# haoy945/DeMF

Hardware: AMD Instinct MI355X
Metric: DeMF fusion fwd+bwd scenes/sec at 20k pts + 530x730 RGB (higher is better)
Workload: dtype f32; 1 GPU; BASELINE configs[2]: full DeMF fusion hot path fwd+loss+bwd+allreduce+AdamW, 8 scenes/GPU x (20000 pts, 800x1120 -> 4-level 256-ch pyramid), 256 queries, H=8 L=4 P=2, fp32; compute_mode=f32, scenes_per_gpu=8, parallelism=dp1, cloud=uniform

## Files before the change

### demf_amd/_ffi.py

```python
import ctypes
import os

_HERE = os.path.dirname(os.path.abspath(__file__))
LIB_PATH = os.environ.get("DEMF_LIB_PATH") or os.path.join(_HERE, "lib", "libdemf_hip.so")

_c_int = ctypes.c_int
_c_float = ctypes.c_float
_ptr = ctypes.c_void_p

SIGNATURES = {
    "demf_stream_create_cu_masked": [_ptr, _c_int, _c_int, _ptr],
    "demf_spin_us": [_c_int, _ptr],
    "demf_conv_nhwc_f32": [_c_int] * 9 + [_ptr, _ptr, _c_int, _ptr, _ptr, _c_int, _c_int, _ptr, _ptr],
    "demf_conv_stem7_nhwc4_f32": [_c_int] * 4 + [_ptr, _ptr, _c_int, _ptr, _c_int, _ptr, _ptr],
    "demf_maxpool3x3s2_nhwc_f32": [_c_int] * 4 + [_ptr, _ptr, _ptr],
    "demf_nchw3_to_nhwc4_f32": [_c_int] * 3 + [_ptr, _ptr, _ptr],
    "demf_groupnorm_nhwc_f32": [_c_int] * 4 + [_c_float, _ptr, _ptr, _ptr, _ptr, _ptr, ctypes.c_longlong, _ptr],
    "demf_fps_f32": [_c_int, _c_int, _c_int, _ptr, _ptr, _ptr, _ptr],
    "demf_fps_ws_f32": [_c_int, _c_int, _c_int, _ptr, _ptr, ctypes.c_longlong, _ptr, _ptr],
    "demf_ball_query_f32": [_c_int, _c_int, _c_int, _c_float, _c_float, _c_int, _ptr, _ptr,
                            _ptr, _ptr],
    "demf_ball_query_grid_ws": [_c_int, _c_int, _ptr, _ptr],
    "demf_ball_query_grid_f32": [_c_int, _c_int, _c_int, _c_float, _c_int] + [_ptr] * 6,
    "demf_group_points_fwd": [_c_int] * 5 + [_ptr] * 4,
    "demf_group_points_bwd": [_c_int] * 5 + [_ptr] * 4,
    "demf_gather_points_fwd": [_c_int] * 4 + [_ptr] * 4,
    "demf_gather_points_bwd": [_c_int] * 4 + [_ptr] * 4,
    "demf_three_nn_f32": [_c_int] * 3 + [_ptr] * 5,
    "demf_three_nn_weights_f32": [_c_int] * 3 + [_ptr] * 6,
    "demf_three_interpolate_fwd": [_c_int] * 4 + [_ptr] * 5,
    "demf_three_interpolate_bwd": [_c_int] * 4 + [_ptr] * 5,
    "demf_group_concat_cl_fwd": [_c_int] * 8 + [_c_float, _c_int] + [_ptr] * 6,
    "demf_group_concat_cl_bwd": [_c_int] * 8 + [_c_float, _c_int] + [_ptr] * 6,
    "demf_gather_rows_cl_fwd": [_c_int] * 4 + [_ptr] * 4,
    "demf_gather_rows_cl_bwd": [_c_int] * 4 + [_ptr] * 4,
    "demf_three_interpolate_cl_fwd": [_c_int] * 6 + [_ptr] * 5,
    "demf_three_interpolate_cl_bwd": [_c_int] * 6 + [_ptr] * 5,
    "demf_three_interpolate_cat_cl_fwd": [_c_int] * 5 + [_ptr] * 6,
    "demf_maxpool_ns_fwd": [_c_int] * 3 + [_ptr] * 4,
    "demf_maxpool_ns_bwd": [_c_int] * 3 + [_ptr] * 4,
    "demf_colsum_f32": [_c_int] * 3 + [_ptr] * 3,
    "demf_nchw_to_tokens": [_c_int] * 5 + [_ptr] * 4,
    "demf_pyramid_to_tokens": [_c_int] * 4 + [_ptr] * 5,
    "demf_pyramid_to_tokens_bf16": [_c_int] * 4 + [_ptr] * 5,
    "demf_vote_targets": [_c_int] * 4 + [_ptr] * 8,
    "demf_box_extent_count": [_c_int] * 4 + [_ptr] * 8,
    "demf_aligned_nms": [_c_int, _c_int, _c_float] + [_ptr] * 6,
    "demf_detect_decode": [_c_int] * 6 + [_ptr] * 7 + [_ptr],
    "demf_detect_pack": [_c_int] * 4 + [_c_float] + [_ptr] * 5 + [_c_int] * 3 + [_ptr] * 5 + [_ptr],
    "demf_box3d_iou": [_c_int, _c_int] + [_ptr] * 4,
    "demf_eval_match": [_c_int, _c_int, _ptr, _c_int, _c_int] + [_ptr] * 7,
    "demf_eval_ap": [_c_int, _c_int] + [_ptr] * 8,
    "demf_points_floor": [_c_int, _c_int, ctypes.c_longlong] + [_ptr] * 4,
    "demf_points_prep": [_c_int] * 3 + [ctypes.c_longlong] + [_ptr] * 8,
    "demf_image_prep": [_c_int] * 3 + [ctypes.c_longlong] + [_ptr] * 6,
    "demf_proposal_targets": [_c_int] * 4 + [_c_float] * 3 + [_ptr] * 18,
    "demf_gt_prep": [_c_int] * 3 + [_ptr] * 10,
    "demf_pad_gt": [_c_int] * 2 + [_ptr] * 8,
    "demf_query_pos_rows": [_c_int] * 2 + [_ptr] * 4,
    "demf_loss_total": [_c_int] + [_ptr] * 4,
    "demf_loss_total_bwd": [_c_int] + [_ptr] * 4,
    "demf_target_weights": [_c_int] + [_ptr] * 5,
    "demf_rows_ln_pos_f32": [_c_int] * 2 + [_ptr] * 4 + [_c_float] + [_ptr] * 4,
    "demf_rows_gemm_f32": [_c_int] * 3 + [_ptr, ctypes.c_longlong, _ptr, _c_int, _c_int, _ptr, _c_int, _ptr, _c_int, _ptr, _c_int,
                           _ptr, ctypes.c_longlong, _ptr, _ptr, _c_float, _ptr, ctypes.c_longlong, _ptr],
    "demf_msda_fwd_raw_f32": [_c_int] * 7 + [_ptr, ctypes.c_longlong, _ptr, _ptr, _ptr, ctypes.c_longlong, _c_int, _c_int,
                              _ptr, _ptr, _ptr],
    "demf_msda_fwd_raw_head_f32": [_c_int] * 4 + [_ptr, ctypes.c_longlong, _ptr, _ptr, _ptr, ctypes.c_longlong, _c_int, _c_int,
                                   _ptr, _ptr, _c_int, _c_int, _ptr],
    "demf_invert_index": [_c_int] * 3 + [_ptr] * 4,
    "demf_invert_index_ws": [_c_int] * 3 + [_ptr] * 5,
    "demf_mlp_gemm_bwd_dw_group": [_c_int, _ptr, _ptr],
    "demf_sa_index_chain": [_c_int] * 3 + [_ptr] * 4,
    "demf_split_points": [ctypes.c_longlong, _c_int] + [_ptr] * 4,
    "demf_group_concat_cl_bwd_gather": [_c_int] * 6 + [_ptr] * 5,
    "demf_group_first_fwd": [_c_int] * 5 + [_c_float, _c_int] + [_ptr] * 5 + [_c_int] + [_ptr] * 4 + [_c_float] * 2 + [_ptr] * 6 + [_ptr],
    "demf_group_first_bwd": [_c_int] * 5 + [_c_float, _c_int] + [_ptr] * 10 + [_c_int, _ptr, _c_int] + [_ptr] * 4,
    "demf_adamw_f32": [ctypes.c_longlong] + [_ptr] * 5 + [_c_float] * 7 + [_c_int, _ptr],
    "demf_multi_copy_sumsq": [_c_int, _ptr, _c_int, _ptr, _ptr],
    "demf_sumsq_f32": [ctypes.c_longlong, _ptr, _ptr, _ptr],
    "demf_adamw_state_f32": [_c_int] + [_ptr] * 9 + [_c_float] * 5 + [_ptr],
    "demf_step_meter": [_c_int, _ptr, _ptr, _c_float, _c_float, _ptr, _c_int, _ptr],
    "demf_mlp_gemm_fwd": [_c_int] * 4 + [_ptr] * 6,
    "demf_mlp_gemm_fwd_pool": [_c_int] * 4 + [_ptr] * 5 + [_c_int] + [_ptr] * 5,
    "demf_mlp_gemm_fwd_bn": [_c_int] * 4 + [_ptr] * 7 + [_c_float, _c_float] + [_ptr] * 7,
    "demf_mlp_gemm_fwd_pool_bn": [_c_int] * 4 + [_ptr] * 5 + [_c_int] + [_ptr] * 6 + [_c_float, _c_float] + [_ptr] * 7,
    "demf_mlp_gemm_fwd_bn_st": [_c_int] * 4 + [_ptr] * 7 + [_c_float, _c_float] + [_ptr] * 6 + [_c_int, _ptr],
    "demf_mlp_gemm_fwd_pool_bn_st": [_c_int] * 4 + [_ptr] * 5 + [_c_int] + [_ptr] * 4 + [_c_float, _c_float] + [_ptr] * 6 + [_c_int, _ptr],
    "demf_pool_select": [_c_int] * 2 + [_ptr] * 9,
    "demf_pool_select_slot0": [_c_int] * 2 + [_ptr] * 7,
    "demf_mlp_first_stats": [_c_int] * 2 + [_ptr] * 5 + [_c_float, _c_float] + [_ptr] * 7,
    "demf_mlp_gemm_fwd_bn_x4": [_c_int] * 2 + [_ptr] * 8 + [_c_float, _c_float] + [_ptr] * 7,
    "demf_mlp_bwd_fused_x4": [_c_int] * 3 + [_ptr] * 11,
    "demf_mlp_bwd_pool": [_c_int] * 4 + [_ptr] * 17,
    "demf_mlp_bwd_pool_ws": [_c_int, _ptr],
    "demf_bn_finalize": [_c_int, ctypes.c_longlong] + [_ptr] * 3 + [_c_float, _c_float] + [_ptr] * 7,
    "demf_l2norm_rows_fwd": [_c_int] * 2 + [_ptr] * 4,
    "demf_l2norm_rows_bwd": [_c_int] * 2 + [_ptr] * 5,
    "demf_vote_combine_fwd": [_c_int] * 2 + [_ptr] * 7,
    "demf_vote_combine_bwd": [_c_int] * 2 + [_ptr] * 7,
    "demf_bnrelu_maxpool_fwd": [_c_int] * 3 + [_ptr] * 5,
    "demf_bn_bwd_reduce": [_c_int] * 3 + [_ptr] * 9,
    "demf_bn_bwd_vectors": [_c_int, ctypes.c_longlong] + [_ptr] * 8,
    "demf_mlp_gemm_bwd_dx": [_c_int] * 4 + [_ptr] * 3 + [_c_int] + [_ptr] * 5,
    "demf_mlp_gemm_bwd_dx_first": [_c_int] * 3 + [_ptr] * 10,
    "demf_mlp_first_finish": [_c_int, ctypes.c_longlong] + [_ptr] * 7,
    "demf_mlp_gemm_bwd_dx_red": [_c_int] * 4 + [_ptr] * 3 + [_c_int] + [_ptr] * 9,
    "demf_mlp_gemm_bwd_dx_w": [_c_int] * 4 + [_ptr] * 3 + [_c_int] + [_ptr] * 5,
    "demf_mlp_bwd_fused": [_c_int] * 3 + [_ptr] * 3 + [_c_int] + [_ptr] * 15 + [_c_int, _ptr],
    "demf_mlp_bwd_fused_cols": [_c_int] * 5 + [_ptr] * 3 + [_c_int] + [_ptr] * 14,
    "demf_mlp_gemm_bwd_dx_red_v": [_c_int] * 4 + [_ptr] * 3 + [_c_int] + [_ptr] * 13,
    "demf_bn_bwd_reduce_vectors": [_c_int] * 3 + [_ptr] * 11 + [_c_int, _ptr],
    "demf_mlp_gemm_bwd_dw": [_c_int] * 4 + [_ptr] * 3 + [_c_int] + [_ptr] * 6,
    "demf_mlp_gemm_bwd_dw_ld": [_c_int] * 4 + [_ptr] * 3 + [_c_int] + [_ptr] * 5 + [_c_int, _ptr],
    "demf_head_loss_fwd": [_c_int] * 3 + [_ptr] * 14,
    "demf_head_loss_bwd": [_c_int] * 3 + [_ptr] * 17,
    "demf_vote_loss": [_c_int] * 4 + [_c_float] + [_ptr] * 10,
    "demf_vote_loss_fwd": [_c_int] * 4 + [_c_float] + [_ptr] * 8,
    "demf_msda_fwd_f32": [_c_int] * 7 + [_ptr] * 7,
    "demf_msda_bwd_f32": [_c_int] * 7 + [_ptr] * 10,
    "demf_msda_fwd_bf16": [_c_int] * 7 + [_ptr] * 7,
    "demf_msda_bwd_bf16": [_c_int] * 7 + [_ptr] * 10,
    "demf_gemm_f32": [_ptr, _ptr],
    "demf_gemm_group_f32": [_ptr, _c_int, _ptr],
    "demf_set_compute_dtype": [_c_int],
    "demf_set_f16_terms": [_c_int],
    "demf_get_compute_dtype": [],
    "demf_ctx_push": [_ptr],
    "demf_ctx_pop": [],
    "demf_gemm_f32_ctx": [_ptr] * 3,
    "demf_gemm_group_f32_ctx": [_ptr, _ptr, _c_int, _ptr],
    "demf_mlp_gemm_fwd_ctx": [_ptr] + [_c_int] * 4 + [_ptr] * 6,
    "demf_multi_copy": [_c_int, _ptr, _c_int, _ptr],
    "demf_zero_f32": [ctypes.c_longlong, _ptr, _ptr],
    "demf_add_dropout_ln_fwd": [_c_int] * 2 + [_ptr] * 4 + [_c_float] * 2 + [_ptr, _c_int] + [_ptr] * 4,
    "demf_add_dropout_ln_bwd": [_c_int] * 2 + [_ptr] * 5 + [_c_float, _ptr, _c_int, _ptr, _c_int] + [_ptr] * 4,
    "demf_attn_core_fwd": [_c_int] * 4 + [_ptr, _c_float, _c_float, _ptr, _c_int] + [_ptr] * 5,
    "demf_attn_core_bwd": [_c_int] * 4 + [_ptr] * 4 + [_c_float, _c_float, _ptr, _c_int] + [_ptr] * 2,
    "demf_softmax_dropout_fwd": [_c_int] * 2 + [_ptr, _c_float, _ptr, _c_int] + [_ptr] * 3,
    "demf_softmax_dropout_bwd": [_c_int] * 2 + [_ptr, _c_float, _ptr, _c_int] + [_ptr] * 2,
    "demf_msda_prep_fwd": [_c_int] * 5 + [_ptr] * 10,
    "demf_msda_prep_bwd": [_c_int] * 5 + [_ptr] * 14,
    "demf_rng_advance": [_ptr, _ptr],
    "demf_rng_next": [_ptr, _ptr, _ptr],
    "demf_dropout_mask": [ctypes.c_longlong, _c_float, _ptr, _c_int, _ptr, _ptr],
}


class DwJob(ctypes.Structure):
    _fields_ = [("R", _c_int), ("N", _c_int), ("K", _c_int), ("ldx", _c_int), ("G", _ptr), ("dP", _ptr), ("arg", _ptr),
                ("ns", _c_int), ("Y", _ptr), ("vec6", _ptr), ("Xprev", _ptr), ("prev_scale_shift", _ptr), ("dW", _ptr),
                ("lddw", _c_int)]


class DetectLayer(ctypes.Structure):
    _fields_ = [("K", _c_int), ("res_scale", _c_float)] + [
        f for name in ("center", "center_base", "size", "dir_class", "dir_res", "obj", "sem")
        for f in ((name, _ptr), ((name if name != "center_base" else "base") + "_sb", _c_int),
                  ((name if name != "center_base" else "base") + "_sk", _c_int))]


class GemmDesc(ctypes.Structure):
    _ll = ctypes.c_longlong
    _fields_ = [
        ("M", _c_int), ("N", _c_int), ("K", _c_int), ("batch", _c_int), ("zdiv", _c_int),
        ("splitk", _c_int),
        ("A", _ptr), ("sam", _ll), ("sak", _ll), ("sab", _ll), ("sab2", _ll),
        ("A2", _ptr), ("a2_cols", _c_int),
        ("B", _ptr), ("sbn", _ll), ("sbk", _ll), ("sbb", _ll), ("sbb2", _ll),
        ("B2", _ptr), ("b2_rows", _c_int),
        ("C", _ptr), ("scm", _ll), ("scb", _ll), ("scb2", _ll),
        ("C2", _ptr),
        ("bias", _ptr), ("sbias_b", _ll),
        ("rowscale", _ptr), ("srs_m", _ll), ("srs_b", _ll),
        ("alpha", _c_float),
        ("flags", _c_int),
        ("gate", _ptr), ("sgm", _ll), ("sgb", _ll),
        ("gate_scale", _c_float),
        ("drop_p", _c_float),
        ("rng", _ptr),
        ("op_id", _c_int),
        ("asum", _ptr),
    ]

_lib = None


def load():
    global _lib
    if _lib is not None:
        return _lib
    if not os.path.exists(LIB_PATH):
        raise RuntimeError(
            f"{LIB_PATH} not found: build it with `python -c 'import __graft_entry__ as g; "
            "g.build()'` (hipcc --offload-arch=gfx950). demf_amd has no CPU fallback.")
    import torch
    lib = ctypes.CDLL(LIB_PATH)
    lib.demf_version.restype = _c_int
    lib.demf_version.argtypes = []
    lib.demf_last_error.restype = ctypes.c_char_p
    lib.demf_last_error.argtypes = []
    for name, argtypes in SIGNATURES.items():
        fn = getattr(lib, name)
        fn.restype = _c_int
        fn.argtypes = argtypes
    _lib = lib
    return lib


def call(name, *args):
    lib = load()
    rc = getattr(lib, name)(*args)
    if rc != 0:
        msg = lib.demf_last_error().decode("utf-8", "replace")
        raise RuntimeError(f"{name} failed (code {rc}): {msg}")
```

### demf_amd/csrc/dense.hip

```cpp
#include "common.h"
#include <stdlib.h>
#include <type_traits>
#include "rng.h"

namespace demf {

using f32x16 = float __attribute__((ext_vector_type(16)));
using bf16x8 = __bf16 __attribute__((ext_vector_type(8)));
using bf16x4 = __bf16 __attribute__((ext_vector_type(4)));

enum {
  GEMM_RELU = DEMF_GEMM_RELU, GEMM_DROPOUT = DEMF_GEMM_DROPOUT, GEMM_GATE = DEMF_GEMM_GATE,
  GEMM_ACCUM = DEMF_GEMM_ACCUM, GEMM_ROWBIAS = DEMF_GEMM_ROWBIAS, GEMM_ACCUM2 = DEMF_GEMM_ACCUM2,
  GEMM_FP32 = DEMF_GEMM_FP32,
};
using GemmArgs = demf_gemm_desc;

constexpr int G_BM = 64, G_BN = 64, G_BK = 64, G_LD = G_BK + 4;

struct GemmRegs {
  float4 v[4], w[4];
};

template <int mode, bool ADD2>
__device__ __forceinline__ void gemm_fetch(GemmRegs& g, float (&sc)[16], const float* __restrict__ P,
                                           const float* __restrict__ P2, long long sr, long long sk,
                                           int r0, int R, int k0, int K1) {
  const int t = threadIdx.x;
  if constexpr (mode == 1) {
#pragma unroll
    for (int i = 0; i < 4; ++i) {
      const int row = (t >> 4) + 16 * i, kq = (t & 15) * 4;
      g.v[i] = make_float4(0.f, 0.f, 0.f, 0.f);
      if constexpr (ADD2) g.w[i] = g.v[i];
      if (r0 + row < R && k0 + kq < K1) {
        const size_t o = (size_t)(r0 + row) * sr + k0 + kq;
        g.v[i] = *reinterpret_cast<const float4*>(P + o);
        if constexpr (ADD2) g.w[i] = *reinterpret_cast<const float4*>(P2 + o);
      }
    }
  } else if constexpr (mode == 2) {
#pragma unroll
    for (int i = 0; i < 4; ++i) {
      const int k = (t >> 4) + 16 * i, rq = (t & 15) * 4;
      g.v[i] = make_float4(0.f, 0.f, 0.f, 0.f);
      if constexpr (ADD2) g.w[i] = g.v[i];
      if (k0 + k < K1 && r0 + rq < R) {
        const size_t o = (size_t)(k0 + k) * sk + r0 + rq;
        g.v[i] = *reinterpret_cast<const float4*>(P + o);
        if constexpr (ADD2) g.w[i] = *reinterpret_cast<const float4*>(P2 + o);
      }
    }
  } else {
#pragma unroll
    for (int i = 0; i < 16; ++i) {
      const int e = t + 256 * i, row = e >> 6, k = e & 63;
      float v = 0.f;
      if (r0 + row < R && k0 + k < K1) {
        const size_t o = (size_t)(r0 + row) * sr + (size_t)(k0 + k) * sk;
        v = P[o];
        if constexpr (ADD2) v += P2[o];
      }
      sc[i] = v;
    }
  }
}

constexpr int G_LDB = 2 * (G_BK + 8);

__device__ __forceinline__ float4 add4(float4 v, const float4& w) {
  v.x += w.x; v.y += w.y; v.z += w.z; v.w += w.w;
  return v;
}

template <int mode, bool ADD2>
__device__ __forceinline__ void gemm_commit_bf16(char* __restrict__ s, const GemmRegs& g, const float (&sc)[16]) {
  const int t = threadIdx.x;
  if constexpr (mode == 1) {
#pragma unroll
    for (int i = 0; i < 4; ++i) {
      const float4 v = ADD2 ? add4(g.v[i], g.w[i]) : g.v[i];
      bf16x4 b;
      b[0] = (__bf16)v.x; b[1] = (__bf16)v.y; b[2] = (__bf16)v.z; b[3] = (__bf16)v.w;
      *reinterpret_cast<bf16x4*>(s + ((t >> 4) + 16 * i) * G_LDB + 2 * (t & 15) * 4) = b;
    }
  } else if constexpr (mode == 2) {
#pragma unroll
    for (int i = 0; i < 4; ++i) {
      const float4 v = ADD2 ? add4(g.v[i], g.w[i]) : g.v[i];
      char* d = s + (t & 15) * 4 * G_LDB + 2 * ((t >> 4) + 16 * i);
      *reinterpret_cast<__bf16*>(d) = (__bf16)v.x;
      *reinterpret_cast<__bf16*>(d + G_LDB) = (__bf16)v.y;
      *reinterpret_cast<__bf16*>(d + 2 * G_LDB) = (__bf16)v.z;
      *reinterpret_cast<__bf16*>(d + 3 * G_LDB) = (__bf16)v.w;
    }
  } else {
#pragma unroll
    for (int i = 0; i < 16; ++i) {
      const int e = t + 256 * i;
      *reinterpret_cast<__bf16*>(s + (e >> 6) * G_LDB + 2 * (e & 63)) = (__bf16)sc[i];
    }
  }
}

template <int mode, bool ADD2>
__device__ __forceinline__ void gemm_commit(float* __restrict__ s, const GemmRegs& g, const float (&sc)[16]) {
  const int t = threadIdx.x;
  if constexpr (mode == 1) {
#pragma unroll
    for (int i = 0; i < 4; ++i) {
      float4 v = g.v[i];
      if constexpr (ADD2) { v.x += g.w[i].x; v.y += g.w[i].y; v.z += g.w[i].z; v.w += g.w[i].w; }
      *reinterpret_cast<float4*>(s + ((t >> 4) + 16 * i) * G_LD + (t & 15) * 4) = v;
    }
  } else if constexpr (mode == 2) {
#pragma unroll
    for (int i = 0; i < 4; ++i) {
      float4 v = g.v[i];
      if constexpr (ADD2) { v.x += g.w[i].x; v.y += g.w[i].y; v.z += g.w[i].z; v.w += g.w[i].w; }
      float* d = s + (t & 15) * 4 * G_LD + (t >> 4) + 16 * i;
      d[0] = v.x; d[G_LD] = v.y; d[2 * G_LD] = v.z; d[3 * G_LD] = v.w;
    }
  } else {
#pragma unroll
    for (int i = 0; i < 16; ++i) {
      const int e = t + 256 * i;
      s[(e >> 6) * G_LD + (e & 63)] = sc[i];
    }
  }
}

__device__ __forceinline__ void gemm_store(const GemmArgs& p, int z, size_t oc, int sp, int m, int n,
                                           float bias, float accv) {
  float v = p.alpha * accv;
  if (p.flags & GEMM_ROWBIAS) {
    if (sp == 0) v = __builtin_fmaf(bias, p.rowscale[(size_t)m * p.srs_m + (size_t)z * p.srs_b], v);
  } else {
    v += bias;
  }
  if (p.flags & GEMM_RELU) v = fmaxf(v, 0.f);
  if (p.flags & GEMM_DROPOUT) {
    const unsigned long long idx = ((unsigned long long)z * p.M + m) * p.N + n;
    v = dropout_keep((const unsigned long long*)p.rng, (unsigned)p.op_id, idx, p.drop_p)
            ? v * (1.0f / (1.0f - p.drop_p)) : 0.f;
  }
  if (p.flags & GEMM_GATE)
    v = p.gate[(size_t)z * p.sgb + (size_t)m * p.sgm + n] != 0.f ? v * p.gate_scale : 0.f;
  float* dst = p.C + oc + (size_t)m * p.scm + n;
  if (p.splitk > 1) atomicAdd(dst, v);
  else if (p.flags & GEMM_ACCUM) *dst += v;
  else *dst = v;
  if (p.C2 != nullptr) {
    float* d2 = p.C2 + oc + (size_t)m * p.scm + n;
    if (p.splitk > 1) atomicAdd(d2, v);
    else if (p.flags & GEMM_ACCUM2) *d2 += v;
    else *d2 = v;
  }
}

__device__ __forceinline__ void xcd_rows(int& bx, int& by, int gx, int gy) {
  if ((gy & 7) == 0) {
    const int L = bx + gx * by;
    by = (L & 7) + 8 * (L / (8 * gx));
    bx = (L >> 3) % gx;
  }
}

template <int MA, int MB, bool ADD, bool BF16>
__global__ __launch_bounds__(256, 2) void gemm_kernel(GemmArgs p) {
  __shared__ __attribute__((aligned(16))) float s_a[G_BM * G_LD];
  __shared__ __attribute__((aligned(16))) float s_b[G_BN * G_LD];
  const int lane = threadIdx.x & 63, wave = threadIdx.x >> 6;
  const int lr = lane & 31, lh = lane >> 5;
  const int wm = wave & 1, wn = wave >> 1;
  int bx = blockIdx.x, by = blockIdx.y;
  xcd_rows(bx, by, gridDim.x, gridDim.y);
  const int m0 = by * G_BM, n0 = bx * G_BN;
  const int z = blockIdx.z / p.splitk, sp = blockIdx.z - z * p.splitk;
  const int kchunk = ((p.K + p.splitk - 1) / p.splitk + G_BK - 1) / G_BK * G_BK;
  const int kbeg = sp * kchunk, kend = min(p.K, kbeg + kchunk);
  const int zo = z / p.zdiv, zi = z - zo * p.zdiv;
  const size_t oa = (size_t)zo * p.sab + (size_t)zi * p.sab2, ob = (size_t)zo * p.sbb + (size_t)zi * p.sbb2;
  const float* A = p.A + oa;
  const float* A2 = (p.A2 != nullptr && n0 < p.a2_cols) ? p.A2 + oa : nullptr;
  const float* B = p.B + ob;
  const float* B2 = (p.B2 != nullptr && m0 < p.b2_rows) ? p.B2 + ob : nullptr;
  f32x16 acc;
#pragma unroll
  for (int r = 0; r < 16; ++r) acc[r] = 0.f;
  constexpr int NS = ADD ? 2 : 3;
  GemmRegs ga[NS], gb[NS];
  float sa16[NS][16], sb16[NS][16];
  auto fetch = [&](auto stage, int k0) {
    constexpr int S = decltype(stage)::value;
    if (ADD && A2 != nullptr) gemm_fetch<MA, ADD>(ga[S], sa16[S], A, A2, p.sam, p.sak, m0, p.M, k0, kend);
    else gemm_fetch<MA, false>(ga[S], sa16[S], A, nullptr, p.sam, p.sak, m0, p.M, k0, kend);
    if (ADD && B2 != nullptr) gemm_fetch<MB, ADD>(gb[S], sb16[S], B, B2, p.sbn, p.sbk, n0, p.N, k0, kend);
    else gemm_fetch<MB, false>(gb[S], sb16[S], B, nullptr, p.sbn, p.sbk, n0, p.N, k0, kend);
  };
  auto step = [&](auto stage, int k0) {
    constexpr int S = decltype(stage)::value;
    lds_barrier();
    if constexpr (BF16) {
      char* ca = reinterpret_cast<char*>(s_a);
      char* cb = reinterpret_cast<char*>(s_b);
      if (ADD && A2 != nullptr) gemm_commit_bf16<MA, ADD>(ca, ga[S], sa16[S]); else gemm_commit_bf16<MA, false>(ca, ga[S], sa16[S]);
      if (ADD && B2 != nullptr) gemm_commit_bf16<MB, ADD>(cb, gb[S], sb16[S]); else gemm_commit_bf16<MB, false>(cb, gb[S], sb16[S]);
      lds_barrier();
      if (k0 + NS * G_BK < kend) fetch(stage, k0 + NS * G_BK);
#pragma unroll
      for (int c16 = 0; c16 < G_BK / 16; ++c16) {
        const bf16x8 a8 = *reinterpret_cast<const bf16x8*>(ca + (wm * 32 + lr) * G_LDB + 2 * (c16 * 16 + 8 * lh));
        const bf16x8 b8 = *reinterpret_cast<const bf16x8*>(cb + (wn * 32 + lr) * G_LDB + 2 * (c16 * 16 + 8 * lh));
        acc = __builtin_amdgcn_mfma_f32_32x32x16_bf16(a8, b8, acc, 0, 0, 0);
      }
    } else {
      if (ADD && A2 != nullptr) gemm_commit<MA, ADD>(s_a, ga[S], sa16[S]); else gemm_commit<MA, false>(s_a, ga[S], sa16[S]);
      if (ADD && B2 != nullptr) gemm_commit<MB, ADD>(s_b, gb[S], sb16[S]); else gemm_commit<MB, false>(s_b, gb[S], sb16[S]);
      lds_barrier();
      if (k0 + NS * G_BK < kend) fetch(stage, k0 + NS * G_BK);
#pragma unroll
      for (int c8 = 0; c8 < G_BK / 8; ++c8) {
        const float4 a4 = *reinterpret_cast<const float4*>(s_a + (wm * 32 + lr) * G_LD + c8 * 8 + 4 * lh);
        const float4 b4 = *reinterpret_cast<const float4*>(s_b + (wn * 32 + lr) * G_LD + c8 * 8 + 4 * lh);
        acc = __builtin_amdgcn_mfma_f32_32x32x2f32(a4.x, b4.x, acc, 0, 0, 0);
        acc = __builtin_amdgcn_mfma_f32_32x32x2f32(a4.y, b4.y, acc, 0, 0, 0);
        acc = __builtin_amdgcn_mfma_f32_32x32x2f32(a4.z, b4.z, acc, 0, 0, 0);
        acc = __builtin_amdgcn_mfma_f32_32x32x2f32(a4.w, b4.w, acc, 0, 0, 0);
      }
    }
  };
  using S0 = std::integral_constant<int, 0>;
  using S1 = std::integral_constant<int, 1>;
  using S2 = std::integral_constant<int, NS - 1>;
  if (kbeg < kend) fetch(S0{}, kbeg);
  if (kbeg + G_BK < kend) fetch(S1{}, kbeg + G_BK);
  if constexpr (NS == 3) {
    if (kbeg + 2 * G_BK < kend) fetch(S2{}, kbeg + 2 * G_BK);
  }
  for (int k0 = kbeg; k0 < kend; k0 += NS * G_BK) {
    step(S0{}, k0);
    if (k0 + G_BK < kend) step(S1{}, k0 + G_BK);
    if constexpr (NS == 3) {
      if (k0 + 2 * G_BK < kend) step(S2{}, k0 + 2 * G_BK);
    }
  }
  const int n = n0 + wn * 32 + lr;
  if (n >= p.N) return;
  float bias = 0.f;
  if (p.bias != nullptr && sp == 0) bias = p.bias[(size_t)z * p.sbias_b + n];
  const size_t oc = (size_t)zo * p.scb + (size_t)zi * p.scb2;
#pragma unroll
  for (int r = 0; r < 16; ++r) {
    const int m = m0 + wm * 32 + (r & 3) + 8 * (r >> 2) + 4 * lh;
    if (m < p.M) gemm_store(p, z, oc, sp, m, n, bias, acc[r]);
  }
}

struct GemmRegsS {
  float4 v[2], w[2];
};

template <int mode, bool ADD2>
__device__ __forceinline__ void gemm_fetch_s(GemmRegsS& g, float (&sc)[8], const float* __restrict__ P,
                                             const float* __restrict__ P2, long long sr, long long sk,
                                             int r0, int R, int k0, int K1) {
  const int t = threadIdx.x;
  if constexpr (mode == 1) {
#pragma unroll
    for (int i = 0; i < 2; ++i) {
      const int row = (t >> 4) + 16 * i, kq = (t & 15) * 4;
      g.v[i] = make_float4(0.f, 0.f, 0.f, 0.f);
      if constexpr (ADD2) g.w[i] = g.v[i];
      if (r0 + row < R && k0 + kq < K1) {
        const size_t o = (size_t)(r0 + row) * sr + k0 + kq;
        g.v[i] = *reinterpret_cast<const float4*>(P + o);
        if constexpr (ADD2) g.w[i] = *reinterpret_cast<const float4*>(P2 + o);
      }
    }
  } else if constexpr (mode == 2) {
#pragma unroll
    for (int i = 0; i < 2; ++i) {
      const int k = (t >> 3) + 32 * i, rq = (t & 7) * 4;
      g.v[i] = make_float4(0.f, 0.f, 0.f, 0.f);
      if constexpr (ADD2) g.w[i] = g.v[i];
      if (k0 + k < K1 && r0 + rq < R) {
        const size_t o = (size_t)(k0 + k) * sk + r0 + rq;
        g.v[i] = *reinterpret_cast<const float4*>(P + o);
        if constexpr (ADD2) g.w[i] = *reinterpret_cast<const float4*>(P2 + o);
      }
    }
  } else {
#pragma unroll
    for (int i = 0; i < 8; ++i) {
      const int e = t + 256 * i, row = e >> 6, k = e & 63;
      float v = 0.f;
      if (r0 + row < R && k0 + k < K1) {
        const size_t o = (size_t)(r0 + row) * sr + (size_t)(k0 + k) * sk;
        v = P[o];
        if constexpr (ADD2) v += P2[o];
      }
      sc[i] = v;
    }
  }
}

template <int mode, bool ADD2, bool BF16>
__device__ __forceinline__ void gemm_commit_s(float* __restrict__ s, const GemmRegsS& g, const float (&sc)[8]) {
  const int t = threadIdx.x;
  char* sb = reinterpret_cast<char*>(s);
  if constexpr (mode == 1) {
#pragma unroll
    for (int i = 0; i < 2; ++i) {
      const float4 v = ADD2 ? add4(g.v[i], g.w[i]) : g.v[i];
      const int row = (t >> 4) + 16 * i, kq = (t & 15) * 4;
      if constexpr (BF16) {
        bf16x4 b;
        b[0] = (__bf16)v.x; b[1] = (__bf16)v.y; b[2] = (__bf16)v.z; b[3] = (__bf16)v.w;
        *reinterpret_cast<bf16x4*>(sb + row * G_LDB + 2 * kq) = b;
      } else {
        *reinterpret_cast<float4*>(s + row * G_LD + kq) = v;
      }
    }
  } else if constexpr (mode == 2) {
#pragma unroll
    for (int i = 0; i < 2; ++i) {
      const float4 v = ADD2 ? add4(g.v[i], g.w[i]) : g.v[i];
      const int k = (t >> 3) + 32 * i, rq = (t & 7) * 4;
      if constexpr (BF16) {
        char* d = sb + rq * G_LDB + 2 * k;
        *reinterpret_cast<__bf16*>(d) = (__bf16)v.x;
        *reinterpret_cast<__bf16*>(d + G_LDB) = (__bf16)v.y;
        *reinterpret_cast<__bf16*>(d + 2 * G_LDB) = (__bf16)v.z;
        *reinterpret_cast<__bf16*>(d + 3 * G_LDB) = (__bf16)v.w;
      } else {
        float* d = s + rq * G_LD + k;
        d[0] = v.x; d[G_LD] = v.y; d[2 * G_LD] = v.z; d[3 * G_LD] = v.w;
      }
    }
  } else {
#pragma unroll
    for (int i = 0; i < 8; ++i) {
      const int e = t + 256 * i;
      if constexpr (BF16) *reinterpret_cast<__bf16*>(sb + (e >> 6) * G_LDB + 2 * (e & 63)) = (__bf16)sc[i];
      else s[(e >> 6) * G_LD + (e & 63)] = sc[i];
    }
  }
}

template <int MA, int MB, bool ADD, bool BF16>
__device__ __forceinline__ void gemm_ks_body(const GemmArgs& p, int bx, int by, int bz, float* __restrict__ s_a,
                                             float* __restrict__ s_b, float (*s_red)[16][64]) {
  const int lane = threadIdx.x & 63, wave = threadIdx.x >> 6;
  const int lr = lane & 31, lh = lane >> 5;
  const int m0 = by * 32, n0 = bx * 32;
  const int z = bz / p.splitk, sp = bz - z * p.splitk;
  const bool do_asum = MA == 2 && p.asum != nullptr && bx == 0;
  float4 rs4 = make_float4(0.f, 0.f, 0.f, 0.f);
  const int kchunk = ((p.K + p.splitk - 1) / p.splitk + G_BK - 1) / G_BK * G_BK;
  const int kbeg = sp * kchunk, kend = min(p.K, kbeg + kchunk);
  const int zo = z / p.zdiv, zi = z - zo * p.zdiv;
  const size_t oa = (size_t)zo * p.sab + (size_t)zi * p.sab2, ob = (size_t)zo * p.sbb + (size_t)zi * p.sbb2;
  const float* A = p.A + oa;
  const float* A2 = (p.A2 != nullptr && n0 < p.a2_cols) ? p.A2 + oa : nullptr;
  const float* B = p.B + ob;
  const float* B2 = (p.B2 != nullptr && m0 < p.b2_rows) ? p.B2 + ob : nullptr;
  f32x16 acc;
#pragma unroll
  for (int r = 0; r < 16; ++r) acc[r] = 0.f;
  constexpr int NS = 3;
  GemmRegsS ga[NS], gb[NS];
  float sa8[NS][8], sb8[NS][8];
// ... 3 lines not shown
    else gemm_fetch_s<MA, false>(ga[S], sa8[S], A, nullptr, p.sam, p.sak, m0, p.M, k0, kend);
    if (ADD && B2 != nullptr) gemm_fetch_s<MB, ADD>(gb[S], sb8[S], B, B2, p.sbn, p.sbk, n0, p.N, k0, kend);
    else gemm_fetch_s<MB, false>(gb[S], sb8[S], B, nullptr, p.sbn, p.sbk, n0, p.N, k0, kend);
  };
  auto step = [&](auto stage, int k0) {
    constexpr int S = decltype(stage)::value;
    lds_barrier();
    if (ADD && A2 != nullptr) gemm_commit_s<MA, ADD, BF16>(s_a, ga[S], sa8[S]); else gemm_commit_s<MA, false, BF16>(s_a, ga[S], sa8[S]);
    if constexpr (MA == 2) {
      if (do_asum) {
        rs4 = add4(rs4, add4(ga[S].v[0], ga[S].v[1]));
      }
    }
    if (ADD && B2 != nullptr) gemm_commit_s<MB, ADD, BF16>(s_b, gb[S], sb8[S]); else gemm_commit_s<MB, false, BF16>(s_b, gb[S], sb8[S]);
    lds_barrier();
    if (k0 + NS * G_BK < kend) fetch(stage, k0 + NS * G_BK);
    if constexpr (BF16) {
      const char* ca = reinterpret_cast<const char*>(s_a);
      const char* cb = reinterpret_cast<const char*>(s_b);
      const bf16x8 a8 = *reinterpret_cast<const bf16x8*>(ca + lr * G_LDB + 2 * (wave * 16 + 8 * lh));
      const bf16x8 b8 = *reinterpret_cast<const bf16x8*>(cb + lr * G_LDB + 2 * (wave * 16 + 8 * lh));
      acc = __builtin_amdgcn_mfma_f32_32x32x16_bf16(a8, b8, acc, 0, 0, 0);
    } else {
#pragma unroll
      for (int c8 = 0; c8 < 2; ++c8) {
        const float4 a4 = *reinterpret_cast<const float4*>(s_a + lr * G_LD + wave * 16 + c8 * 8 + 4 * lh);
        const float4 b4 = *reinterpret_cast<const float4*>(s_b + lr * G_LD + wave * 16 + c8 * 8 + 4 * lh);
        acc = __builtin_amdgcn_mfma_f32_32x32x2f32(a4.x, b4.x, acc, 0, 0, 0);
        acc = __builtin_amdgcn_mfma_f32_32x32x2f32(a4.y, b4.y, acc, 0, 0, 0);
        acc = __builtin_amdgcn_mfma_f32_32x32x2f32(a4.z, b4.z, acc, 0, 0, 0);
        acc = __builtin_amdgcn_mfma_f32_32x32x2f32(a4.w, b4.w, acc, 0, 0, 0);
      }
    }
  };
  using S0 = std::integral_constant<int, 0>;
  using S1 = std::integral_constant<int, 1>;
  using S2 = std::integral_constant<int, 2>;
  if (kbeg < kend) fetch(S0{}, kbeg);
  if (kbeg + G_BK < kend) fetch(S1{}, kbeg + G_BK);
  if (kbeg + 2 * G_BK < kend) fetch(S2{}, kbeg + 2 * G_BK);
  for (int k0 = kbeg; k0 < kend; k0 += NS * G_BK) {
    step(S0{}, k0);
    if (k0 + G_BK < kend) step(S1{}, k0 + G_BK);
    if (k0 + 2 * G_BK < kend) step(S2{}, k0 + 2 * G_BK);
  }
#pragma unroll
  for (int r = 0; r < 16; ++r) s_red[wave][r][lane] = acc[r];
  lds_barrier();
  const int n = n0 + lr;
  if (n < p.N) {
    float bias = 0.f;
    if (p.bias != nullptr && sp == 0) bias = p.bias[(size_t)z * p.sbias_b + n];
    const size_t oc = (size_t)zo * p.scb + (size_t)zi * p.scb2;
#pragma unroll
    for (int q = 0; q < 4; ++q) {
      const int r = 4 * wave + q;
      const int m = m0 + q + 8 * wave + 4 * lh;
      const float v = (s_red[0][r][lane] + s_red[1][r][lane]) + (s_red[2][r][lane] + s_red[3][r][lane]);
      if (m < p.M) gemm_store(p, z, oc, sp, m, n, bias, v);
    }
  }
  if constexpr (MA == 2) {
    if (do_asum) {
      lds_barrier();
      float4* q4 = reinterpret_cast<float4*>(&s_red[0][0][0]);
      q4[threadIdx.x] = rs4;
      lds_barrier();
      if (threadIdx.x < 32 && m0 + (int)threadIdx.x < p.M) {
        const int rq = threadIdx.x >> 2, c = threadIdx.x & 3;
        const float* f = &s_red[0][0][0];
        float t = 0.f;
        for (int j = 0; j < 32; ++j) t += f[(8 * j + rq) * 4 + c];
        atomicAdd(p.asum + (size_t)z * p.M + m0 + threadIdx.x, t);
      }
    }
  }
}

template <int MA, int MB, bool ADD, bool BF16>
__global__ __launch_bounds__(256, ADD ? 2 : 4) void gemm_ks_kernel(GemmArgs p) {
  __shared__ __attribute__((aligned(16))) float s_a[32 * G_LD];
  __shared__ __attribute__((aligned(16))) float s_b[32 * G_LD];
  __shared__ float s_red[4][16][64];
  int bx = blockIdx.x, by = blockIdx.y;
  xcd_rows(bx, by, gridDim.x, gridDim.y);
  gemm_ks_body<MA, MB, ADD, BF16>(p, bx, by, blockIdx.z, s_a, s_b, s_red);
}

constexpr int GEMM_GROUP_MAX = 12;
struct GemmGroup {
  GemmArgs p[GEMM_GROUP_MAX];
  int start[GEMM_GROUP_MAX + 1];
  int n;
  int dbg;
};
template <int MA, int MB, bool ADD, bool BF16>
__global__ __launch_bounds__(256, ADD ? 2 : 4) void gemm_ks_group_kernel(GemmGroup g) {
  __shared__ __attribute__((aligned(16))) float s_a[32 * G_LD];
  __shared__ __attribute__((aligned(16))) float s_b[32 * G_LD];
  __shared__ float s_red[4][16][64];
  const int b = blockIdx.x;
  int i = 0;
  while (i + 1 < g.n && b >= g.start[i + 1]) ++i;
  const GemmArgs& p = g.p[i];
  const int local = b - g.start[i];
  const int gx = (p.N + 31) / 32, gy = (p.M + 31) / 32;
  const int sp = local % p.splitk, rest = local / p.splitk;
  const int bx = rest % gx, by = (rest / gx) % gy, bz = (rest / (gx * gy)) * p.splitk + sp;
  gemm_ks_body<MA, MB, ADD, BF16>(p, bx, by, bz, s_a, s_b, s_red);
}

using f32x2 = float __attribute__((ext_vector_type(2)));
using bf16x2 = __bf16 __attribute__((ext_vector_type(2)));
template <int P>
__device__ __forceinline__ void split_pair(float a, float b, unsigned (&o)[P]) {
  const f32x2 x = {a, b};
  const bf16x2 h = __builtin_convertvector(x, bf16x2);
  o[0] = __builtin_bit_cast(unsigned, h);
  if constexpr (P == 3) {
    const f32x2 r = x - __builtin_convertvector(h, f32x2);
    const bf16x2 m = __builtin_convertvector(r, bf16x2);
    o[1] = __builtin_bit_cast(unsigned, m);
    const f32x2 l = r - __builtin_convertvector(m, f32x2);
    o[2] = __builtin_bit_cast(unsigned, __builtin_convertvector(l, bf16x2));
  }
}
__device__ __forceinline__ int tn_swz(int col, int chunk) { return col * 64 + ((chunk ^ ((col >> 2) & 3)) << 4); }

template <int P>
__global__ __launch_bounds__(256, 3) void gemm_tn_group_kernel(GemmGroup g) {
  __shared__ __attribute__((aligned(16))) char s_pl[2][2][P][4096];
  __shared__ float4 s_rs[128];
  const int b = blockIdx.x;
  const int li = threadIdx.x & 63;
  const int gi = __builtin_amdgcn_readfirstlane(
      __popcll(__ballot(li + 1 < g.n && b >= g.start[li + 1 < GEMM_GROUP_MAX ? li + 1 : GEMM_GROUP_MAX])));
  const GemmArgs& p = g.p[gi];
  const int local = b - g.start[gi];
  const int gx = (p.N + 63) / 64, gy = (p.M + 63) / 64;
  const int sp = local % p.splitk, rest = local / p.splitk;
  const int bx = rest % gx, by = (rest / gx) % gy, z = rest / (gx * gy);
  const int m0 = by * 64, n0 = bx * 64;
  const int t = threadIdx.x, lane = t & 63, wave = t >> 6;
  const int lc = lane & 31, lh = lane >> 5, wm = wave & 1, wn = wave >> 1;
  const int kchunk = ((p.K + p.splitk - 1) / p.splitk + 31) / 32 * 32;
  const int kbeg = sp * kchunk, kend = min(p.K, kbeg + kchunk);
  const int zo = z / p.zdiv, zi = z - zo * p.zdiv;
  const size_t ob = (size_t)zo * p.sbb + (size_t)zi * p.sbb2;
  const int opd = t >> 7, u = t & 127, rg = u >> 4, sc = (u & 15) * 4;
  const float* src = opd == 0 ? p.A + (size_t)zo * p.sab + (size_t)zi * p.sab2 + m0 + sc : p.B + ob + n0 + sc;
  const float* src2 = (opd == 1 && p.B2 != nullptr && m0 < p.b2_rows) ? p.B2 + ob + n0 + sc : nullptr;
  const long long sk = opd == 0 ? p.sak : p.sbk;
  const bool col_ok = opd == 0 ? m0 + sc < p.M : n0 + sc < p.N;
  const bool do_asum = p.asum != nullptr && bx == 0 && opd == 0;
  float4 rv[2][4], rw[2][4], rs4 = make_float4(0.f, 0.f, 0.f, 0.f);
  auto fetch = [&](auto stage, int k0) {
    constexpr int S = decltype(stage)::value;
#pragma unroll
    for (int j = 0; j < 4; ++j) {
      const int k = k0 + 4 * rg + j;
      rv[S][j] = rw[S][j] = make_float4(0.f, 0.f, 0.f, 0.f);
      if (col_ok && k < kend && !(g.dbg & 8)) {
        rv[S][j] = *reinterpret_cast<const float4*>(src + (size_t)k * sk);
        if (src2 != nullptr) rw[S][j] = *reinterpret_cast<const float4*>(src2 + (size_t)k * sk);
      }
    }
// ... 11 lines not shown
      unsigned lo[P], hi[P];
      split_pair<P>(f[c], f[4 + c], lo);
      split_pair<P>(f[8 + c], f[12 + c], hi);
      const int off = tn_swz(sc + c, rg >> 1) + 8 * (rg & 1);
#pragma unroll
      for (int q = 0; q < P; ++q) *reinterpret_cast<uint2*>(&s_pl[buf][opd][q][off]) = make_uint2(lo[q], hi[q]);
    }
  };
  f32x16 acc, acc1;
#pragma unroll
  for (int r = 0; r < 16; ++r) acc[r] = acc1[r] = 0.f;
  auto step = [&](auto stage, int k0, int buf) {
    if (!(g.dbg & 4)) commit(stage, buf);
    lds_barrier();
    if (k0 + 64 < kend) fetch(stage, k0 + 64);
    if (g.dbg & 2) return;
#pragma unroll
    for (int c = 0; c < 2; ++c) {
      bf16x8 pa[P], pb[P];
#pragma unroll
      for (int q = 0; q < P; ++q) {
        pa[q] = *reinterpret_cast<const bf16x8*>(&s_pl[buf][0][q][tn_swz(32 * wm + lc, 2 * c + lh)]);
        pb[q] = *reinterpret_cast<const bf16x8*>(&s_pl[buf][1][q][tn_swz(32 * wn + lc, 2 * c + lh)]);
      }
      f32x16& ac = c == 0 ? acc : acc1;
      if constexpr (P == 3) {
        ac = __builtin_amdgcn_mfma_f32_32x32x16_bf16(pa[2], pb[0], ac, 0, 0, 0);
        ac = __builtin_amdgcn_mfma_f32_32x32x16_bf16(pa[0], pb[2], ac, 0, 0, 0);
        ac = __builtin_amdgcn_mfma_f32_32x32x16_bf16(pa[1], pb[1], ac, 0, 0, 0);
        ac = __builtin_amdgcn_mfma_f32_32x32x16_bf16(pa[1], pb[0], ac, 0, 0, 0);
        ac = __builtin_amdgcn_mfma_f32_32x32x16_bf16(pa[0], pb[1], ac, 0, 0, 0);
      }
      ac = __builtin_amdgcn_mfma_f32_32x32x16_bf16(pa[0], pb[0], ac, 0, 0, 0);
    }
  };
  using S0 = std::integral_constant<int, 0>;
  using S1 = std::integral_constant<int, 1>;
  if (kbeg < kend) fetch(S0{}, kbeg);
  if (kbeg + 32 < kend) fetch(S1{}, kbeg + 32);
  for (int k0 = kbeg; k0 < kend; k0 += 64) {
    step(S0{}, k0, 0);
    if (k0 + 32 < kend) step(S1{}, k0 + 32, 1);
  }
#pragma unroll
  for (int r = 0; r < 16; ++r) acc[r] += acc1[r];
  const int n = n0 + 32 * wn + lc;
  if (n < p.N && !(g.dbg & 16)) {
    float* C = p.C + (size_t)zo * p.scb + (size_t)zi * p.scb2;
#pragma unroll
    for (int r = 0; r < 16; ++r) {
      const int m = m0 + 32 * wm + (r & 3) + 8 * (r >> 2) + 4 * lh;
      if (m < p.M) {
        float* dst = C + (size_t)m * p.scm + n;
        const float v = p.alpha * acc[r];
        if (g.dbg & 1) *dst = v;
        else if (p.splitk > 1) atomicAdd(dst, v);
        else if (p.flags & GEMM_ACCUM) *dst += v;
        else *dst = v;
      }
    }
  }
  if (p.asum != nullptr && bx == 0) {
    if (opd == 0) s_rs[u] = rs4;
    lds_barrier();
    if (t < 64 && m0 + t < p.M) {
      const float* f = reinterpret_cast<const float*>(s_rs);
      float v = 0.f;
      for (int j = 0; j < 8; ++j) v += f[(16 * j + (t >> 2)) * 4 + (t & 3)];
      atomicAdd(p.asum + (size_t)z * p.M + m0 + t, v);
    }
  }
}

static int env_tiles() {
  static const int v = getenv("DEMF_GEMM_SMALL_TILES") ? atoi(getenv("DEMF_GEMM_SMALL_TILES")) : 1024;
  return v;
}

static int stage_mode(long long sr, long long sk, int R, int K) {
  if (sk == 1 && K % 4 == 0) return 1;
  if (sr == 1 && R % 4 == 0) return 2;
  return 0;
}

template <int VPL>
__global__ __launch_bounds__(256) void add_dropout_ln_fwd_k(int R, const float* __restrict__ x,
                                                            const float* __restrict__ identity,
                                                            const float* __restrict__ gamma,
                                                            const float* __restrict__ beta, float eps,
                                                            float p, const unsigned long long* __restrict__ rng,
                                                            unsigned op, float* __restrict__ s_out,
                                                            float* __restrict__ y,
                                                            float* __restrict__ stats) {
  constexpr int C = 64 * VPL;
  const int row = blockIdx.x * 4 + (threadIdx.x >> 6), lane = threadIdx.x & 63;
  if (row >= R) return;
  const float inv_keep = p > 0.f ? 1.0f / (1.0f - p) : 1.0f;
  float v[VPL];
  float sum = 0.f;
#pragma unroll
  for (int i = 0; i < VPL; ++i) {
    const int c = lane + 64 * i;
    float xv = x[(size_t)row * C + c];
    if (p > 0.f) xv = dropout_keep(rng, op, (unsigned long long)row * C + c, p) ? xv * inv_keep : 0.f;
    v[i] = (identity != nullptr ? identity[(size_t)row * C + c] : 0.f) + xv;
    sum += v[i];
  }
  const float mean = group_allsum<64>(sum) * (1.0f / C);
  float sq = 0.f;
#pragma unroll
  for (int i = 0; i < VPL; ++i) sq = __builtin_fmaf(v[i] - mean, v[i] - mean, sq);
  const float rstd = 1.0f / sqrtf(group_allsum<64>(sq) * (1.0f / C) + eps);
#pragma unroll
  for (int i = 0; i < VPL; ++i) {
    const int c = lane + 64 * i;
    if (s_out != nullptr) s_out[(size_t)row * C + c] = v[i];
    y[(size_t)row * C + c] = __builtin_fmaf((v[i] - mean) * rstd, gamma[c], beta[c]);
  }
  if (lane == 0 && stats != nullptr) { stats[2 * row] = mean; stats[2 * row + 1] = rstd; }
}

template <int VPL>
__global__ __launch_bounds__(256) void add_dropout_ln_bwd_k(int R, int rows_per_wave,
                                                            const float* __restrict__ dy,
                                                            const float* __restrict__ dy2,
                                                            const float* __restrict__ s,
                                                            const float* __restrict__ stats,
                                                            const float* __restrict__ gamma, float p,
                                                            const unsigned long long* __restrict__ rng,
                                                            unsigned op, float* __restrict__ ds_out,
                                                            int ds_accum, float* __restrict__ dx_out,
                                                            float* __restrict__ dgamma,
                                                            float* __restrict__ dbeta) {
  constexpr int C = 64 * VPL;
  __shared__ float s_red[4][2][C];
  const int wave = threadIdx.x >> 6, lane = threadIdx.x & 63;
  const float inv_keep = p > 0.f ? 1.0f / (1.0f - p) : 1.0f;
  float ag[VPL], ab[VPL], gm[VPL];
#pragma unroll
  for (int i = 0; i < VPL; ++i) { ag[i] = ab[i] = 0.f; gm[i] = gamma[lane + 64 * i]; }
  const int row0 = (blockIdx.x * 4 + wave) * rows_per_wave;
  for (int row = row0; row < min(R, row0 + rows_per_wave); ++row) {
    const float mean = stats[2 * row], rstd = stats[2 * row + 1];
    float d[VPL], xh[VPL];
    float m1 = 0.f, m2 = 0.f;
#pragma unroll
    for (int i = 0; i < VPL; ++i) {
      const size_t o = (size_t)row * C + lane + 64 * i;
      d[i] = dy[o] + (dy2 != nullptr ? dy2[o] : 0.f);
      xh[i] = (s[o] - mean) * rstd;
      ag[i] = __builtin_fmaf(d[i], xh[i], ag[i]);
      ab[i] += d[i];
      const float g = d[i] * gm[i];
      m1 += g;
      m2 = __builtin_fmaf(g, xh[i], m2);
    }
    m1 = group_allsum<64>(m1) * (1.0f / C);
    m2 = group_allsum<64>(m2) * (1.0f / C);
#pragma unroll
    for (int i = 0; i < VPL; ++i) {
      const int c = lane + 64 * i;
      const size_t o = (size_t)row * C + c;
      const float v = rstd * (d[i] * gm[i] - m1 - xh[i] * m2);
      if (ds_out != nullptr) ds_out[o] = ds_accum ? ds_out[o] + v : v;
      if (dx_out != nullptr) {
        float xv = v;
// ... 154 lines not shown
    if (h != 0) return;
    for (int hh = 0; hh < H; ++hh)
      for (int l = 0; l < L; ++l) {
        const float vx = vr[(b * L + l) * 2], vy = vr[(b * L + l) * 2 + 1];
        for (int q = 0; q < P; ++q) {
          const size_t o = ((size_t)row * H + hh) * LP + l * P + q;
          du = __builtin_fmaf(DL(2 * o), vx, du);
          dv = __builtin_fmaf(DL(2 * o + 1), vy, dv);
        }
      }
  }
  const float u0 = uvw[4 * row], v0 = uvw[4 * row + 1], xw = uvw[4 * row + 2], yw = uvw[4 * row + 3];
  if (!(u0 >= 0.f && u0 <= 1.f)) du = 0.f;
  if (!(v0 >= 0.f && v0 <= 1.f)) dv = 0.f;
  const float x = pts[3 * row], y = pts[3 * row + 1], zc = pts[3 * row + 2];
  const float* m = M + 16 * b;
  const float pw = m[8] * x + m[9] * y + m[10] * zc + m[11];
  const float gx = du * ab[4 * b] / pw, gy = dv * ab[4 * b + 2] / pw;
  const float gw = -(gx * xw + gy * yw);
  dpts[3 * row] = gx * m[0] + gy * m[4] + gw * m[8];
  dpts[3 * row + 1] = gx * m[1] + gy * m[5] + gw * m[9];
  dpts[3 * row + 2] = gx * m[2] + gy * m[6] + gw * m[10];
}

template <int VPL>
__global__ __launch_bounds__(256) void l2norm_fwd_k(int R, const float* __restrict__ x,
                                                    float* __restrict__ y, float* __restrict__ norm) {
  constexpr int C = 64 * VPL;
  const int row = blockIdx.x * 4 + (threadIdx.x >> 6), lane = threadIdx.x & 63;
  if (row >= R) return;
  float v[VPL], sq = 0.f;
#pragma unroll
  for (int i = 0; i < VPL; ++i) { v[i] = x[(size_t)row * C + lane + 64 * i]; sq = __builtin_fmaf(v[i], v[i], sq); }
  const float n = sqrtf(group_allsum<64>(sq));
#pragma unroll
  for (int i = 0; i < VPL; ++i) y[(size_t)row * C + lane + 64 * i] = v[i] / n;
  if (lane == 0) norm[row] = n;
}

template <int VPL>
__global__ __launch_bounds__(256) void l2norm_bwd_k(int R, const float* __restrict__ y,
                                                    const float* __restrict__ norm,
                                                    const float* __restrict__ dy, float* __restrict__ dx) {
  constexpr int C = 64 * VPL;
  const int row = blockIdx.x * 4 + (threadIdx.x >> 6), lane = threadIdx.x & 63;
  if (row >= R) return;
  float yv[VPL], g[VPL], dot = 0.f;
#pragma unroll
  for (int i = 0; i < VPL; ++i) {
    yv[i] = y[(size_t)row * C + lane + 64 * i];
    g[i] = dy[(size_t)row * C + lane + 64 * i];
    dot = __builtin_fmaf(yv[i], g[i], dot);
  }
  dot = group_allsum<64>(dot);
  const float inv = 1.0f / norm[row];
#pragma unroll
  for (int i = 0; i < VPL; ++i) dx[(size_t)row * C + lane + 64 * i] = (g[i] - yv[i] * dot) * inv;
}

template <int VPL>
__global__ __launch_bounds__(256) void vote_combine_fwd_k(int R, const float* __restrict__ rows,
                                                          const float* __restrict__ votes,
                                                          const float* __restrict__ seed_xyz,
                                                          float* __restrict__ vote_xyz,
                                                          float* __restrict__ y, float* __restrict__ norm) {
  constexpr int C = 64 * VPL;
  const int row = blockIdx.x * 4 + (threadIdx.x >> 6), lane = threadIdx.x & 63;
  if (row >= R) return;
  const float* vr = votes + (size_t)row * (C + 3);
  float v[VPL], sq = 0.f;
#pragma unroll
  for (int i = 0; i < VPL; ++i) {
    v[i] = rows[(size_t)row * C + lane + 64 * i] + vr[3 + lane + 64 * i];
    sq = __builtin_fmaf(v[i], v[i], sq);
  }
  const float n = sqrtf(group_allsum<64>(sq));
#pragma unroll
  for (int i = 0; i < VPL; ++i) y[(size_t)row * C + lane + 64 * i] = v[i] / n;
  if (lane == 0) norm[row] = n;
  if (lane < 3) vote_xyz[(size_t)row * 3 + lane] = seed_xyz[(size_t)row * 3 + lane] + vr[lane];
}

template <int VPL>
__global__ __launch_bounds__(256) void vote_combine_bwd_k(int R, const float* __restrict__ y,
                                                          const float* __restrict__ norm,
                                                          const float* __restrict__ dy,
                                                          const float* __restrict__ dxyz,
                                                          float* __restrict__ dvotes,
                                                          float* __restrict__ drows) {
  constexpr int C = 64 * VPL;
  const int row = blockIdx.x * 4 + (threadIdx.x >> 6), lane = threadIdx.x & 63;
  if (row >= R) return;
  float yv[VPL], g[VPL], dot = 0.f;
#pragma unroll
  for (int i = 0; i < VPL; ++i) {
    yv[i] = y[(size_t)row * C + lane + 64 * i];
    g[i] = dy != nullptr ? dy[(size_t)row * C + lane + 64 * i] : 0.f;
    dot = __builtin_fmaf(yv[i], g[i], dot);
  }
  dot = group_allsum<64>(dot);
  const float inv = 1.0f / norm[row];
  float* dv = dvotes + (size_t)row * (C + 3);
#pragma unroll
  for (int i = 0; i < VPL; ++i) {
    const float d = (g[i] - yv[i] * dot) * inv;
    dv[3 + lane + 64 * i] = d;
    drows[(size_t)row * C + lane + 64 * i] = d;
  }
  if (lane < 3) dv[lane] = dxyz != nullptr ? dxyz[(size_t)row * 3 + lane] : 0.f;
}

__global__ void rng_advance_k(unsigned long long* rng) { rng[1] += 1; }
__global__ void rng_next_k(unsigned long long* rng, unsigned long long* snap) {
  const unsigned long long s = rng[1] + 1;
  rng[1] = s;
  snap[0] = rng[0];
  snap[1] = s;
}

__global__ void dropout_mask_k(long long n, float p, const unsigned long long* __restrict__ rng,
                               unsigned op, float* __restrict__ out) {
  const long long i = (long long)blockIdx.x * blockDim.x + threadIdx.x;
  if (i < n) out[i] = dropout_keep(rng, op, (unsigned long long)i, p) ? 1.0f / (1.0f - p) : 0.f;
}

}

using namespace demf;

static int gemm_validate(const GemmArgs& p) {
  DEMF_REQUIRE(p.M > 0 && p.N > 0 && p.K > 0 && p.batch > 0 && p.splitk > 0 && p.zdiv > 0,
               "gemm: bad sizes %d %d %d %d %d %d", p.M, p.N, p.K, p.batch, p.splitk, p.zdiv);
  DEMF_REQUIRE(p.A && p.B && p.C, "gemm: null operand");
  DEMF_REQUIRE(!(p.flags & GEMM_DROPOUT) || p.rng, "gemm: dropout needs the rng state");
  DEMF_REQUIRE(!(p.flags & GEMM_GATE) || p.gate, "gemm: gate flag without a gate tensor");
  DEMF_REQUIRE(!(p.flags & GEMM_ROWBIAS) || (p.rowscale && p.bias), "gemm: rowbias needs bias and rowscale");
  DEMF_REQUIRE(p.splitk == 1 || !(p.flags & (GEMM_RELU | GEMM_DROPOUT | GEMM_GATE)),
               "gemm: split-K cannot carry a non-linear epilogue");
  DEMF_REQUIRE((long long)p.batch * p.splitk <= 65535, "gemm: batch*splitk too large");
  return DEMF_OK;
}

static bool gemm_is_small(const GemmArgs& p) {
  const long long tiles = (long long)cdiv(p.N, G_BN) * cdiv(p.M, G_BM) * p.batch * p.splitk;
  return tiles <= env_tiles() || p.N <= 32;
}

extern "C" int demf_gemm_f32(const demf_gemm_desc* d, demf_stream_t stream) {
  DEMF_REQUIRE(d != nullptr, "gemm: null descriptor");
  GemmArgs p = *d;
  if (int e = gemm_validate(p)) return e;
  const int modeA = stage_mode(p.sam, p.sak, p.M, p.K);
  const int modeB = stage_mode(p.sbn, p.sbk, p.N, p.K);
  dim3 grid(cdiv(p.N, G_BN), cdiv(p.M, G_BM), p.batch * p.splitk);
  const bool add = p.A2 != nullptr || p.B2 != nullptr;
  const bool bf = compute_bf16() && !(p.flags & GEMM_FP32);
  const bool small = gemm_is_small(p);
  if (p.asum != nullptr && !(small && modeA == 2 && p.A2 == nullptr)) {
    DEMF_REQUIRE(p.sam == 1 && p.A2 == nullptr,
                 "gemm: asum needs A contiguous along M (sam == 1) and no A2");
    float* asum = p.asum;
    p.asum = nullptr;
    if (int e = demf_gemm_f32(&p, stream)) return e;
    for (int z = 0; z < p.batch; ++z) {
      const int zo = z / p.zdiv, zi = z - zo * p.zdiv;
      const float* a = p.A + (size_t)zo * p.sab + (size_t)zi * p.sab2;
      if (int e = demf_colsum_f32(p.K, p.M, (int)p.sak, a, asum + (size_t)z * p.M, stream)) return e;
    }
    return DEMF_OK;
  }
  if (small) {
    grid = dim3(cdiv(p.N, 32), cdiv(p.M, 32), p.batch * p.splitk);
#define GEMM_LAUNCH_S(MA_, MB_)                                                                        \
  do {                                                                                                 \
    if (bf) {                                                                                          \
      if (add) hipLaunchKernelGGL((gemm_ks_kernel<MA_, MB_, true, true>), grid, dim3(256), 0, (hipStream_t)stream, p);   \
      else hipLaunchKernelGGL((gemm_ks_kernel<MA_, MB_, false, true>), grid, dim3(256), 0, (hipStream_t)stream, p);      \
    } else {                                                                                           \
      if (add) hipLaunchKernelGGL((gemm_ks_kernel<MA_, MB_, true, false>), grid, dim3(256), 0, (hipStream_t)stream, p);  \
      else hipLaunchKernelGGL((gemm_ks_kernel<MA_, MB_, false, false>), grid, dim3(256), 0, (hipStream_t)stream, p);     \
    }                                                                                                  \
  } while (0)
    switch (modeA * 3 + modeB) {
      case 0: GEMM_LAUNCH_S(0, 0); break;
      case 1: GEMM_LAUNCH_S(0, 1); break;
      case 2: GEMM_LAUNCH_S(0, 2); break;
      case 3: GEMM_LAUNCH_S(1, 0); break;
      case 4: GEMM_LAUNCH_S(1, 1); break;
      case 5: GEMM_LAUNCH_S(1, 2); break;
      case 6: GEMM_LAUNCH_S(2, 0); break;
      case 7: GEMM_LAUNCH_S(2, 1); break;
      default: GEMM_LAUNCH_S(2, 2); break;
    }
#undef GEMM_LAUNCH_S
    return check_launch("gemm_ks_kernel");
  }
#define GEMM_LAUNCH(MA_, MB_)                                                                          \
  do {                                                                                                 \
    if (bf) {                                                                                          \
      if (add) hipLaunchKernelGGL((gemm_kernel<MA_, MB_, true, true>), grid, dim3(256), 0, (hipStream_t)stream, p);   \
      else hipLaunchKernelGGL((gemm_kernel<MA_, MB_, false, true>), grid, dim3(256), 0, (hipStream_t)stream, p);      \
    } else {                                                                                           \
      if (add) hipLaunchKernelGGL((gemm_kernel<MA_, MB_, true, false>), grid, dim3(256), 0, (hipStream_t)stream, p);  \
      else hipLaunchKernelGGL((gemm_kernel<MA_, MB_, false, false>), grid, dim3(256), 0, (hipStream_t)stream, p);     \
    }                                                                                                  \
  } while (0)
  switch (modeA * 3 + modeB) {
    case 0: GEMM_LAUNCH(0, 0); break;
    case 1: GEMM_LAUNCH(0, 1); break;
    case 2: GEMM_LAUNCH(0, 2); break;
    case 3: GEMM_LAUNCH(1, 0); break;
    case 4: GEMM_LAUNCH(1, 1); break;
    case 5: GEMM_LAUNCH(1, 2); break;
    case 6: GEMM_LAUNCH(2, 0); break;
    case 7: GEMM_LAUNCH(2, 1); break;
    default: GEMM_LAUNCH(2, 2); break;
  }
#undef GEMM_LAUNCH
  return check_launch("gemm_kernel");
}

extern "C" int demf_gemm_group_f32(const demf_gemm_desc* descs, int n, demf_stream_t stream) {
  DEMF_REQUIRE(descs != nullptr && n >= 1, "gemm_group: no descriptors");
  const bool bf = compute_bf16();
  static const bool tn_off = getenv("DEMF_GEMM_TN3") && atoi(getenv("DEMF_GEMM_TN3")) == 0;
  const bool tn3 = compute_mode() != 0 && !tn_off;
  static const int tn_split = getenv("DEMF_GEMM_TN_SPLIT") ? atoi(getenv("DEMF_GEMM_TN_SPLIT")) : 0;
  int i0 = 0;
  while (i0 < n) {
    GemmGroup g{};
    int cnt = 0, tiles = 0;
    while (i0 + cnt < n && cnt < GEMM_GROUP_MAX) {
      const GemmArgs& p = descs[i0 + cnt];
      if (int e = gemm_validate(p)) return e;
      const bool ok = gemm_is_small(p) && stage_mode(p.sam, p.sak, p.M, p.K) == 2 &&
                      stage_mode(p.sbn, p.sbk, p.N, p.K) == 2 && !(p.flags & GEMM_FP32) && p.A2 == nullptr &&
                      (!tn3 || ((p.flags & ~GEMM_ACCUM) == 0 && p.bias == nullptr && p.C2 == nullptr &&
                                (p.B2 == nullptr || p.b2_rows % 64 == 0 || p.b2_rows >= p.M)));
      if (!ok) break;
      g.p[cnt] = p;
      g.start[cnt] = tiles;
      tiles += (tn3 ? cdiv(p.N, 64) * cdiv(p.M, 64) : cdiv(p.N, 32) * cdiv(p.M, 32)) * p.batch * g.p[cnt].splitk;
      ++cnt;
    }
    if (cnt == 0) {
      if (int e = demf_gemm_f32(descs + i0, stream)) return e;
      ++i0;
      continue;
    }
    if (tn3) {
      int base = 0;
      for (int i = 0; i < cnt; ++i) base += cdiv(g.p[i].N, 64) * cdiv(g.p[i].M, 64) * g.p[i].batch;
      const int want = tn_split > 0 ? tn_split : (768 + base / 2) / base;
      tiles = 0;
      for (int i = 0; i < cnt; ++i) {
        GemmArgs& q = g.p[i];
        if (q.splitk > 1) q.splitk = want < 2 ? 2 : (want < q.splitk ? want : q.splitk);
        g.start[i] = tiles;
        tiles += cdiv(q.N, 64) * cdiv(q.M, 64) * q.batch * q.splitk;
      }
    }
    g.start[cnt] = tiles;
    g.n = cnt;
    static const int tn_dbg = getenv("DEMF_TN_DBG") ? atoi(getenv("DEMF_TN_DBG")) : 0;
    g.dbg = tn_dbg;
    if (tn3) {
      if (bf) hipLaunchKernelGGL((gemm_tn_group_kernel<1>), dim3(tiles), dim3(256), 0, (hipStream_t)stream, g);
      else hipLaunchKernelGGL((gemm_tn_group_kernel<3>), dim3(tiles), dim3(256), 0, (hipStream_t)stream, g);
      if (int e = check_launch("gemm_tn_group_kernel")) return e;
      i0 += cnt;
      continue;
    }
    if (bf) hipLaunchKernelGGL((gemm_ks_group_kernel<2, 2, true, true>), dim3(tiles), dim3(256), 0, (hipStream_t)stream, g);
    else hipLaunchKernelGGL((gemm_ks_group_kernel<2, 2, true, false>), dim3(tiles), dim3(256), 0, (hipStream_t)stream, g);
    if (int e = check_launch("gemm_ks_group_kernel")) return e;
    i0 += cnt;
  }
  return DEMF_OK;
}

#define LN_DISPATCH(C, CALL)                       \
  switch ((C) / 64) {                              \
    case 1: CALL(1); break;                        \
    case 2: CALL(2); break;                        \
    case 4: CALL(4); break;                        \
    case 8: CALL(8); break;                        \
    case 16: CALL(16); break;                      \
    default:                                       \
      demf::set_error("row kernel: %d channels unsupported (64/128/256/512/1024)", (C)); \
      return DEMF_EUNSUPPORTED;                    \
  }

#define SM_DISPATCH(S, CALL)                       \
  if ((S) <= 0 || (S) > 1024) {                    \
    demf::set_error("softmax: %d keys unsupported (1..1024)", (S)); \
    return DEMF_EUNSUPPORTED;                      \
  } else if ((S) <= 64) { CALL(1); }               \
  else if ((S) <= 128) { CALL(2); }                \
  else if ((S) <= 256) { CALL(4); }                \
  else if ((S) <= 512) { CALL(8); }                \
  else { CALL(16); }

extern "C" int demf_add_dropout_ln_fwd(int R, int C, const float* x, const float* identity,
                                       const float* gamma, const float* beta, float eps, float p,
                                       const void* rng, int op_id, float* s_out, float* y,
                                       float* stats, demf_stream_t stream) {
  DEMF_REQUIRE(R > 0 && x && gamma && beta && y, "add_dropout_ln_fwd: bad arguments");
  DEMF_REQUIRE(p == 0.f || rng, "add_dropout_ln_fwd: dropout needs the rng state");
#define CALL(V) hipLaunchKernelGGL(add_dropout_ln_fwd_k<V>, dim3(cdiv(R, 4)), dim3(256), 0, (hipStream_t)stream, \
                                   R, x, identity, gamma, beta, eps, p, (const unsigned long long*)rng,        \
                                   (unsigned)op_id, s_out, y, stats)
  LN_DISPATCH(C, CALL)
#undef CALL
  return check_launch("add_dropout_ln_fwd_k");
}

extern "C" int demf_add_dropout_ln_bwd(int R, int C, const float* dy, const float* dy2, const float* s,
                                       const float* stats, const float* gamma, float p, const void* rng,
// ... 10 lines not shown
  LN_DISPATCH(C, CALL)
#undef CALL
  return check_launch("add_dropout_ln_bwd_k");
}

extern "C" int demf_softmax_dropout_fwd(int R, int S, const float* scores, float p, const void* rng,
                                        int op_id, float* prob, float* out, demf_stream_t stream) {
  DEMF_REQUIRE(R > 0 && scores && prob && out, "softmax_dropout_fwd: bad arguments");
  DEMF_REQUIRE(p == 0.f || rng, "softmax_dropout_fwd: dropout needs the rng state");
#define CALL(V) hipLaunchKernelGGL(softmax_dropout_fwd_k<V>, dim3(cdiv(R, 4)), dim3(256), 0, (hipStream_t)stream, \
                                   R, S, scores, p, (const unsigned long long*)rng, (unsigned)op_id, prob, out)
  SM_DISPATCH(S, CALL)
#undef CALL
  return check_launch("softmax_dropout_fwd_k");
}

extern "C" int demf_softmax_dropout_bwd(int R, int S, const float* prob, float p, const void* rng,
                                        int op_id, float* dio, demf_stream_t stream) {
  DEMF_REQUIRE(R > 0 && prob && dio, "softmax_dropout_bwd: bad arguments");
  DEMF_REQUIRE(p == 0.f || rng, "softmax_dropout_bwd: dropout needs the rng state");
#define CALL(V) hipLaunchKernelGGL(softmax_dropout_bwd_k<V>, dim3(cdiv(R, 4)), dim3(256), 0, (hipStream_t)stream, \
                                   R, S, prob, p, (const unsigned long long*)rng, (unsigned)op_id, dio)
  SM_DISPATCH(S, CALL)
#undef CALL
  return check_launch("softmax_dropout_bwd_k");
}

extern "C" int demf_msda_prep_fwd(int R, int Q, int H, int L, int P, const float* pts, const float* M,
                                  const float* ab, const float* valid_ratios, const int64_t* shapes,
                                  const float* raw, float* loc, float* w, float* uvw,
                                  demf_stream_t stream) {
  DEMF_REQUIRE(R > 0 && Q > 0 && R % Q == 0 && H > 0 && L > 0 && P > 0 && L * P <= 16,
               "msda_prep_fwd: bad sizes (L*P <= 16)");
  DEMF_REQUIRE(pts && M && ab && valid_ratios && shapes && raw && loc && w && uvw, "msda_prep_fwd: null pointer");
  hipLaunchKernelGGL(msda_prep_fwd_k, dim3(cdiv(R * H, 256)), dim3(256), 0, (hipStream_t)stream, R, Q, H, L,
                     P, pts, M, ab, valid_ratios, (const long long*)shapes, raw, loc, w, uvw);
  return check_launch("msda_prep_fwd_k");
}

extern "C" int demf_msda_prep_bwd(int R, int Q, int H, int L, int P, const float* pts, const float* M,
                                  const float* ab, const float* valid_ratios, const int64_t* shapes,
                                  const float* w, const float* uvw, const float* dloc, const float* dloc2,
                                  const float* dw, const float* dw2, float* draw, float* dpts,
                                  demf_stream_t stream) {
  DEMF_REQUIRE(R > 0 && Q > 0 && R % Q == 0 && H > 0 && L > 0 && P > 0 && L * P <= 16,
               "msda_prep_bwd: bad sizes (L*P <= 16)");
  DEMF_REQUIRE(pts && M && ab && valid_ratios && shapes && w && uvw && dloc && dw && draw, "msda_prep_bwd: null pointer");
  hipLaunchKernelGGL(msda_prep_bwd_k, dim3(cdiv(R * H, 256)), dim3(256), 0, (hipStream_t)stream, R, Q, H, L,
                     P, pts, M, ab, valid_ratios, (const long long*)shapes, w, uvw, dloc, dloc2, dw, dw2, draw, dpts);
  return check_launch("msda_prep_bwd_k");
}

extern "C" int demf_l2norm_rows_fwd(int R, int C, const float* x, float* y, float* norm,
                                    demf_stream_t stream) {
  DEMF_REQUIRE(R > 0 && x && y && norm, "l2norm_rows_fwd: bad arguments");
#define CALL(V) hipLaunchKernelGGL(l2norm_fwd_k<V>, dim3(cdiv(R, 4)), dim3(256), 0, (hipStream_t)stream, R, x, y, norm)
  LN_DISPATCH(C, CALL)
#undef CALL
  return check_launch("l2norm_fwd_k");
}

extern "C" int demf_l2norm_rows_bwd(int R, int C, const float* y, const float* norm, const float* dy,
                                    float* dx, demf_stream_t stream) {
  DEMF_REQUIRE(R > 0 && y && norm && dy && dx, "l2norm_rows_bwd: bad arguments");
#define CALL(V) hipLaunchKernelGGL(l2norm_bwd_k<V>, dim3(cdiv(R, 4)), dim3(256), 0, (hipStream_t)stream, R, y, norm, dy, dx)
  LN_DISPATCH(C, CALL)
#undef CALL
  return check_launch("l2norm_bwd_k");
}

extern "C" int demf_vote_combine_fwd(int R, int C, const float* rows, const float* votes,
                                     const float* seed_xyz, float* vote_xyz, float* vote_feats,
                                     float* norm, demf_stream_t stream) {
  DEMF_REQUIRE(R > 0 && rows && votes && seed_xyz && vote_xyz && vote_feats && norm,
               "vote_combine_fwd: bad arguments");
#define CALL(V) hipLaunchKernelGGL(vote_combine_fwd_k<V>, dim3(cdiv(R, 4)), dim3(256), 0, (hipStream_t)stream, R, rows, votes, seed_xyz, vote_xyz, vote_feats, norm)
  LN_DISPATCH(C, CALL)
#undef CALL
  return check_launch("vote_combine_fwd_k");
}

extern "C" int demf_vote_combine_bwd(int R, int C, const float* vote_feats, const float* norm,
                                     const float* d_vote_feats, const float* d_vote_xyz,
                                     float* d_votes, float* d_rows, demf_stream_t stream) {
  DEMF_REQUIRE(R > 0 && vote_feats && norm && d_votes && d_rows, "vote_combine_bwd: bad arguments");
#define CALL(V) hipLaunchKernelGGL(vote_combine_bwd_k<V>, dim3(cdiv(R, 4)), dim3(256), 0, (hipStream_t)stream, R, vote_feats, norm, d_vote_feats, d_vote_xyz, d_votes, d_rows)
  LN_DISPATCH(C, CALL)
#undef CALL
  return check_launch("vote_combine_bwd_k");
}

extern "C" int demf_rng_advance(void* rng, demf_stream_t stream) {
  DEMF_REQUIRE(rng, "rng_advance: null state");
  hipLaunchKernelGGL(rng_advance_k, dim3(1), dim3(1), 0, (hipStream_t)stream, (unsigned long long*)rng);
  return check_launch("rng_advance_k");
}

extern "C" int demf_rng_next(void* rng, void* snapshot, demf_stream_t stream) {
  DEMF_REQUIRE(rng && snapshot, "rng_next: null state");
  hipLaunchKernelGGL(rng_next_k, dim3(1), dim3(1), 0, (hipStream_t)stream, (unsigned long long*)rng,
                     (unsigned long long*)snapshot);
  return check_launch("rng_next_k");
}

extern "C" int demf_dropout_mask(long long n, float p, const void* rng, int op_id, float* out,
                                 demf_stream_t stream) {
  DEMF_REQUIRE(n > 0 && rng && out && p >= 0.f && p < 1.f, "dropout_mask: bad arguments");
  hipLaunchKernelGGL(dropout_mask_k, dim3((unsigned)((n + 255) / 256)), dim3(256), 0, (hipStream_t)stream, n, p,
                     (const unsigned long long*)rng, (unsigned)op_id, out);
  return check_launch("dropout_mask_k");
}
```

### demf_amd/csrc/loss.hip

```cpp
#include "common.h"

namespace demf {

struct HeadLossCfg {
  int R, ncls, nreg, nbins, nsem;
  float cw0, cw1;
  float w_obj, w_dircls, w_dirres, w_size, w_center, w_sem, w_iou;
  float beta_dirres, beta_size, beta_center;
};

constexpr int NLOSS = 7;

__device__ __forceinline__ float smooth_l1(float d, float beta) {
  const float a = fabsf(d);
  return a < beta ? 0.5f * a * a / beta : a - 0.5f * beta;
}
__device__ __forceinline__ float smooth_l1_grad(float d, float beta) {
  const float a = fabsf(d);
  return a < beta ? d / beta : (d > 0.f ? 1.f : (d < 0.f ? -1.f : 0.f));
}

template <int MAXN>
__device__ __forceinline__ float ce(const float* p, int n, int t, float* grad , float gscale) {
  float m = p[0];
// ... 347 lines not shown
                          float* __restrict__ dir_res, unsigned char* __restrict__ valid,
                          long long* __restrict__ lab, float* __restrict__ center) {
  const int i = blockIdx.x * blockDim.x + threadIdx.x;
  if (i >= n) return;
  const float* t = gt + (size_t)i * 7;
  const float yaw = t[6];
  cs[i] = cosf(-yaw);
  sn[i] = sinf(-yaw);
  const float two_pi = (float)(2.0 * 3.14159265358979323846);
  const float per = (float)(2.0 * 3.14159265358979323846 / (double)nbins);
  const float half = (float)(2.0 * 3.14159265358979323846 / (double)nbins / 2.0);
  const float ang = torch_remainder(yaw, two_pi);
  const float shifted = torch_remainder(ang + half, two_pi);
  const float c = torch_floor_divide(shifted, per);
  dir_cls[i] = (long long)c;
  dir_res[i] = shifted - (c * per + half);
  const long long l = labels[i];
  valid[i] = l >= 0 ? 1 : 0;
  lab[i] = l < 0 ? 0 : l;
  center[(size_t)i * 3] = t[0];
  center[(size_t)i * 3 + 1] = t[1];
  center[(size_t)i * 3 + 2] = t[2] + t[5] * 0.5f;
}

constexpr int PAD_GT_MAX_B = 32;
struct PadGtArgs {
  const float* boxes[PAD_GT_MAX_B];
  const long long* labels[PAD_GT_MAX_B];
  int count[PAD_GT_MAX_B];
  int box_dim[PAD_GT_MAX_B];
  int B, G;
};
__global__ void pad_gt_k(PadGtArgs a, float* __restrict__ gt, long long* __restrict__ lab,
                         unsigned char* __restrict__ valid) {
  const int i = blockIdx.x * blockDim.x + threadIdx.x;
  if (i >= a.B * a.G) return;
  const int b = i / a.G, g = i - b * a.G;
  const int n = a.count[b];
  float* o = gt + (size_t)i * 7;
  if (g < n) {
    const float* t = a.boxes[b] + (size_t)g * a.box_dim[b];
#pragma unroll
    for (int c = 0; c < 7; ++c) o[c] = t[c];
    lab[i] = a.labels[b][g];
  } else {
#pragma unroll
    for (int c = 0; c < 7; ++c) o[c] = 0.f;
    lab[i] = (n == 0 && g == 0) ? 0 : -1;
  }
  if (valid != nullptr) valid[i] = g < (n > 1 ? n : 1) ? 1 : 0;
}

__global__ void query_pos_rows_k(int R, int nreg, const float* __restrict__ reg, const float* __restrict__ base,
                                 float* __restrict__ out) {
  const int r = blockIdx.x * blockDim.x + threadIdx.x;
  if (r >= R) return;
  const float* g = reg + (size_t)r * nreg;
  const float* b = base + (size_t)r * 3;
  float4* o = reinterpret_cast<float4*>(out + (size_t)r * 8);
  o[0] = make_float4(b[0] + g[0], b[1] + g[1], b[2] + g[2], g[3]);
  o[1] = make_float4(g[4], g[5], 0.f, 0.f);
}

__global__ __launch_bounds__(1024) void target_weights_k(int R, const float* __restrict__ obj_mask,
                                                         const long long* __restrict__ obj_t,
                                                         float* __restrict__ obj_w,
                                                         float* __restrict__ box_w) {
  __shared__ float s_m[16], s_o[16];
  float m = 0.f, o = 0.f;
  for (int i = threadIdx.x; i < R; i += 1024) { m += obj_mask[i]; o += (float)obj_t[i]; }
  for (int d = 32; d >= 1; d >>= 1) { m += __shfl_xor(m, d); o += __shfl_xor(o, d); }
  if ((threadIdx.x & 63) == 0) { s_m[threadIdx.x >> 6] = m; s_o[threadIdx.x >> 6] = o; }
  __syncthreads();
  m = 0.f; o = 0.f;
  for (int w = 0; w < 16; ++w) { m += s_m[w]; o += s_o[w]; }
  const float im = m + 1e-6f, io = o + 1e-6f;
  for (int i = threadIdx.x; i < R; i += 1024) {
    obj_w[i] = obj_mask[i] / im;
    box_w[i] = (float)obj_t[i] / io;
  }
}

struct LossTotalArgs { const float* v[4]; };
__global__ void loss_total_k(int n, LossTotalArgs a, const float* __restrict__ vote, float* __restrict__ out8) {
  if (threadIdx.x != 0 || blockIdx.x != 0) return;
  float tot = 0.f;
  for (int i = 0; i < 7; ++i) {
    float m = a.v[0][i];
    for (int j = 1; j < n; ++j) m = m + a.v[j][i];
    m = m / (float)n;
    out8[i] = m;
    tot = i == 0 ? m : tot + m;
  }
  out8[7] = tot + (vote ? vote[0] : 0.f);
}
__global__ void loss_total_bwd_k(int n, const float* __restrict__ g8, float* __restrict__ gv, float* __restrict__ gvote) {
  const int t = threadIdx.x;
  if (t < 7) {
    const float g = (g8[t] + g8[7]) / (float)n;
    for (int j = 0; j < n; ++j) gv[7 * j + t] = g;
  }
  if (t == 7 && gvote) gvote[0] = g8[7];
}

}


using namespace demf;

static HeadLossCfg make_cfg(int R, const float* hp) {
  HeadLossCfg c;
  c.R = R; c.ncls = 12; c.nreg = 30; c.nbins = 12; c.nsem = 10;
  c.cw0 = hp[0]; c.cw1 = hp[1];
  c.w_obj = hp[2]; c.w_dircls = hp[3]; c.w_dirres = hp[4]; c.w_size = hp[5]; c.w_center = hp[6];
  c.w_sem = hp[7]; c.w_iou = hp[8];
  c.beta_dirres = hp[9]; c.beta_size = hp[10]; c.beta_center = hp[11];
  return c;
}

extern "C" int demf_head_loss_fwd(int R, int num_dir_bins, int num_classes, const float* hyper12,
                                  const float* cls, const float* reg, const float* base_xyz,
                                  const float* center_t, const float* size_t_,
                                  const int64_t* dir_class_t, const float* dir_res_t,
                                  const int64_t* sem_t, const int64_t* obj_t, const float* obj_w,
                                  const float* box_w, float* out7, demf_stream_t stream) {
  DEMF_REQUIRE(R >= 0 && num_dir_bins == 12 && num_classes == 10,
               "head_loss: only the reference layout (12 direction bins, 10 classes) is built");
  if (R == 0) return DEMF_OK;
  DEMF_REQUIRE(hyper12 && cls && reg && base_xyz && center_t && size_t_ && dir_class_t && dir_res_t &&
                   sem_t && obj_t && obj_w && box_w && out7, "head_loss_fwd: null pointer");
  hipLaunchKernelGGL(head_loss_fwd_k, dim3(cdiv(R, 256)), dim3(256), 0, (hipStream_t)stream,
                     make_cfg(R, hyper12), cls, reg, base_xyz, center_t, size_t_,
                     (const long long*)dir_class_t, dir_res_t, (const long long*)sem_t,
                     (const long long*)obj_t, obj_w, box_w, out7);
  return check_launch("head_loss_fwd");
}

extern "C" int demf_head_loss_bwd(int R, int num_dir_bins, int num_classes, const float* hyper12,
                                  const float* cls, const float* reg, const float* base_xyz,
                                  const float* center_t, const float* size_t_,
                                  const int64_t* dir_class_t, const float* dir_res_t,
                                  const int64_t* sem_t, const int64_t* obj_t, const float* obj_w,
                                  const float* box_w, const float* grad_out7, float* grad_cls,
                                  float* grad_reg, float* grad_base, demf_stream_t stream) {
  DEMF_REQUIRE(R >= 0 && num_dir_bins == 12 && num_classes == 10,
               "head_loss: only the reference layout (12 direction bins, 10 classes) is built");
  if (R == 0) return DEMF_OK;
  DEMF_REQUIRE(hyper12 && cls && reg && base_xyz && center_t && size_t_ && dir_class_t && dir_res_t &&
                   sem_t && obj_t && obj_w && box_w && grad_out7 && grad_cls && grad_reg && grad_base,
               "head_loss_bwd: null pointer");
  hipLaunchKernelGGL(head_loss_bwd_k, dim3(cdiv(R, 256)), dim3(256), 0, (hipStream_t)stream,
                     make_cfg(R, hyper12), cls, reg, base_xyz, center_t, size_t_,
                     (const long long*)dir_class_t, dir_res_t, (const long long*)sem_t,
                     (const long long*)obj_t, obj_w, box_w, grad_out7, grad_cls, grad_reg, grad_base);
  return check_launch("head_loss_bwd");
}

extern "C" int demf_vote_loss(int B, int S, int N, int gt_per_seed, float dst_weight,
                              const float* seed_points, const float* vote_points,
                              const int64_t* seed_indices, const int64_t* vote_target_masks,
                              const float* vote_targets, const float* mask_sum,
                              const float* grad_out, float* out, float* grad_vote,
                              demf_stream_t stream) {
  DEMF_REQUIRE(B >= 0 && S >= 0 && N >= 1 && gt_per_seed >= 1, "vote_loss: bad sizes");
  if (B * S == 0) return DEMF_OK;
  DEMF_REQUIRE(seed_points && vote_points && seed_indices && vote_target_masks && vote_targets &&
                   mask_sum && (grad_out ? grad_vote != nullptr : out != nullptr),
               "vote_loss: null pointer");
  hipLaunchKernelGGL(vote_loss_k<false>, dim3(cdiv(B * S, 256)), dim3(256), 0, (hipStream_t)stream, B, S, N,
                     3 * gt_per_seed, dst_weight, seed_points, vote_points,
                     (const long long*)seed_indices, (const long long*)vote_target_masks,
                     vote_targets, mask_sum, grad_out, out, grad_vote, (float*)nullptr);
  return check_launch("vote_loss");
}

extern "C" int demf_vote_loss_fwd(int B, int S, int N, int gt_per_seed, float dst_weight,
                                  const float* seed_points, const float* vote_points,
                                  const int64_t* seed_indices, const int64_t* vote_target_masks,
                                  const float* vote_targets, float* mask_sum_out, float* out,
                                  demf_stream_t stream) {
  DEMF_REQUIRE(B >= 0 && S >= 0 && N >= 1 && gt_per_seed >= 1, "vote_loss_fwd: bad sizes");
  DEMF_REQUIRE(mask_sum_out && out, "vote_loss_fwd: null pointer");
  if (B * S == 0) return DEMF_OK;
  DEMF_REQUIRE(seed_points && vote_points && seed_indices && vote_target_masks && vote_targets,
               "vote_loss_fwd: null pointer");
// ... 32 lines not shown
                                     int64_t* mask_targets, float* distance_targets,
                                     int64_t* objectness_targets, float* objectness_masks,
                                     demf_stream_t stream) {
  DEMF_REQUIRE(B >= 0 && Q >= 0 && G >= 1 && res_scale > 0.f, "proposal_targets: bad sizes");
  if (B * Q == 0) return DEMF_OK;
  DEMF_REQUIRE(aggregated_points && gt_boxes && cos_neg_yaw && sin_neg_yaw && gt_dir_class &&
                   gt_dir_res && gt_labels && valid && center_targets && size_targets &&
                   dir_class_targets && dir_res_targets && dir_targets && mask_targets &&
                   distance_targets && objectness_targets && objectness_masks,
               "proposal_targets: null pointer");
  PropTargetArgs a;
  a.Q = Q; a.G = G; a.with_rot = with_rot; a.pos_thr = pos_thr; a.neg_thr = neg_thr;
  a.res_scale = res_scale; a.agg = aggregated_points; a.gt = gt_boxes; a.cs = cos_neg_yaw;
  a.sn = sin_neg_yaw; a.dir_res = gt_dir_res; a.dir_cls = (const long long*)gt_dir_class;
  a.lab = (const long long*)gt_labels; a.valid = valid; a.center_t = center_targets;
  a.size_t_ = size_targets; a.dir_res_t = dir_res_targets; a.dir_t = dir_targets;
  a.dist_t = distance_targets; a.obj_mask = objectness_masks;
  a.dir_cls_t = (long long*)dir_class_targets; a.mask_t = (long long*)mask_targets;
  a.obj_t = (long long*)objectness_targets;
  hipLaunchKernelGGL(proposal_targets_k, dim3(cdiv(Q, 256), B), dim3(256), 0, (hipStream_t)stream, a);
  return check_launch("proposal_targets");
}

extern "C" int demf_gt_prep(int B, int G, int num_dir_bins, const float* gt_boxes,
                            const int64_t* labels_padded, float* cos_neg_yaw, float* sin_neg_yaw,
                            int64_t* gt_dir_class, float* gt_dir_res, unsigned char* valid,
                            int64_t* labels_clamped, float* gravity_center, demf_stream_t stream) {
  DEMF_REQUIRE(B >= 0 && G >= 1 && num_dir_bins >= 1, "gt_prep: bad sizes B=%d G=%d", B, G);
  if (B == 0) return DEMF_OK;
  DEMF_REQUIRE(gt_boxes && labels_padded && cos_neg_yaw && sin_neg_yaw && gt_dir_class && gt_dir_res &&
                   valid && labels_clamped && gravity_center, "gt_prep: null pointer");
  const int n = B * G;
  hipLaunchKernelGGL(gt_prep_k, dim3(cdiv(n, 256)), dim3(256), 0, (hipStream_t)stream, n, num_dir_bins,
                     gt_boxes, (const long long*)labels_padded, cos_neg_yaw, sin_neg_yaw,
                     (long long*)gt_dir_class, gt_dir_res, valid, (long long*)labels_clamped,
                     gravity_center);
  return check_launch("gt_prep");
}

extern "C" int demf_pad_gt(int B, int G, const int* counts, const int* box_dims, const void* const* boxes,
                           const void* const* labels, float* gt_padded, int64_t* labels_padded,
                           unsigned char* valid, demf_stream_t stream) {
  DEMF_REQUIRE(B >= 0 && B <= PAD_GT_MAX_B && G >= 1, "pad_gt: bad sizes B=%d (max %d) G=%d", B, PAD_GT_MAX_B, G);
  if (B == 0) return DEMF_OK;
  DEMF_REQUIRE(counts && box_dims && boxes && labels && gt_padded && labels_padded, "pad_gt: null pointer");
  PadGtArgs a{};
  a.B = B; a.G = G;
  for (int b = 0; b < B; ++b) {
    DEMF_REQUIRE(counts[b] >= 0 && counts[b] <= G, "pad_gt: scene %d has %d boxes, the padded form holds %d", b, counts[b], G);
    DEMF_REQUIRE(counts[b] == 0 || (boxes[b] && labels[b] && box_dims[b] >= 7), "pad_gt: scene %d: null list / box_dim < 7", b);
    a.boxes[b] = (const float*)boxes[b];
    a.labels[b] = (const long long*)labels[b];
    a.count[b] = counts[b];
    a.box_dim[b] = box_dims[b];
  }
  const int n = B * G;
  hipLaunchKernelGGL(pad_gt_k, dim3(cdiv(n, 256)), dim3(256), 0, (hipStream_t)stream, a, gt_padded,
                     (long long*)labels_padded, valid);
  return check_launch("pad_gt");
}

extern "C" int demf_query_pos_rows(int R, int nreg, const float* reg_rows, const float* base_xyz,
                                   float* out8, demf_stream_t stream) {
  DEMF_REQUIRE(R >= 0 && nreg >= 6, "query_pos_rows: bad sizes R=%d nreg=%d", R, nreg);
  if (R == 0) return DEMF_OK;
  DEMF_REQUIRE(reg_rows && base_xyz && out8, "query_pos_rows: null pointer");
  hipLaunchKernelGGL(query_pos_rows_k, dim3(cdiv(R, 256)), dim3(256), 0, (hipStream_t)stream, R, nreg, reg_rows,
                     base_xyz, out8);
  return check_launch("query_pos_rows");
}

extern "C" int demf_target_weights(int R, const float* objectness_masks,
                                   const int64_t* objectness_targets, float* objectness_weights,
                                   float* box_loss_weights, demf_stream_t stream) {
  DEMF_REQUIRE(R >= 0, "target_weights: bad size");
  if (R == 0) return DEMF_OK;
  DEMF_REQUIRE(objectness_masks && objectness_targets && objectness_weights && box_loss_weights,
               "target_weights: null pointer");
  hipLaunchKernelGGL(target_weights_k, dim3(1), dim3(1024), 0, (hipStream_t)stream, R, objectness_masks,
                     (const long long*)objectness_targets, objectness_weights, box_loss_weights);
  return check_launch("target_weights");
}

extern "C" int demf_loss_total(int n, const float* const* vecs, const float* vote, float* out8, demf_stream_t stream) {
  DEMF_REQUIRE(n >= 1 && n <= 4 && vecs && out8, "loss_total: 1..4 seven-vectors");
  LossTotalArgs a{};
  for (int i = 0; i < n; ++i) {
    DEMF_REQUIRE(vecs[i], "loss_total: null vector %d", i);
    a.v[i] = vecs[i];
  }
  hipLaunchKernelGGL(loss_total_k, dim3(1), dim3(64), 0, (hipStream_t)stream, n, a, vote, out8);
  return check_launch("loss_total");
}

extern "C" int demf_loss_total_bwd(int n, const float* g8, float* gvecs, float* gvote, demf_stream_t stream) {
  DEMF_REQUIRE(n >= 1 && n <= 4 && g8 && gvecs, "loss_total_bwd: 1..4 seven-vectors");
  hipLaunchKernelGGL(loss_total_bwd_k, dim3(1), dim3(64), 0, (hipStream_t)stream, n, g8, gvecs, gvote);
  return check_launch("loss_total_bwd");
}
```

### demf_amd/engine.py

```python
import contextlib
import os

import torch
import torch.distributed as dist


def init_distributed():
    world = int(os.environ.get("WORLD_SIZE", "1"))
    rank = int(os.environ.get("RANK", "0"))
    local = int(os.environ.get("LOCAL_RANK", "0"))
    if os.environ.get("DEMF_SHARE_DEVICE"):
        local = 0
    if world > 1 and not dist.is_initialized():
        os.environ.setdefault("MASTER_ADDR", "127.0.0.1")
        os.environ.setdefault("MASTER_PORT", "29500")
        backend = os.environ.get("DEMF_DIST_BACKEND") or \
            ("nccl" if torch.cuda.is_available() else "gloo")
        if torch.cuda.is_available():
            torch.cuda.set_device(local)
        dist.init_process_group(backend=backend, rank=rank, world_size=world)
    elif torch.cuda.is_available():
        torch.cuda.set_device(local)
    return rank, local, world


def cu_masked_streams(side_cus):
    import ctypes
    from . import _ffi
    arr = (ctypes.c_int * len(side_cus))(*side_cus)
    out = []
    for invert in (1, 0):
        h = ctypes.c_void_p()
        _ffi.call("demf_stream_create_cu_masked", ctypes.cast(arr, ctypes.c_void_p), len(side_cus),
                  invert, ctypes.cast(ctypes.byref(h), ctypes.c_void_p))
        out.append(torch.cuda.ExternalStream(h.value))
    return out[0], out[1]


_REJECTED_STREAMS = []


def concurrent_stream(main=None, tries=8, spin_us=300):
    from . import _ffi
    main = main if main is not None else torch.cuda.current_stream()
    if torch.cuda.is_current_stream_capturing():
        return torch.cuda.Stream()
    last = None
    for _ in range(tries):
        cand = torch.cuda.Stream()
        last = cand
        cand.wait_stream(main)
        e0, e1 = torch.cuda.Event(enable_timing=True), torch.cuda.Event(enable_timing=True)
        e0.record(main)
        _ffi.call("demf_spin_us", spin_us, main.cuda_stream)
        with torch.cuda.stream(cand):
            _ffi.call("demf_spin_us", spin_us, cand.cuda_stream)
        main.wait_stream(cand)
        e1.record(main)
        e1.synchronize()
        if e0.elapsed_time(e1) * 1e3 < 1.5 * spin_us:
            return cand
        _REJECTED_STREAMS.append(cand)
    return last


class FlatGrads:

    def __init__(self, params):
        self.params = [p for p in params if p.requires_grad]
        n = sum(p.numel() for p in self.params)
        dev, dt = self.params[0].device, self.params[0].dtype
        self.flat = torch.zeros(n, dtype=dt, device=dev)
        self.views = []
        self._pending_tables, self._tables = [], []
        self.captured_pack = False
        self.sumsq_state = None
        self._reserved_table = None
        off = 0
        for p in self.params:
            k = p.numel()
            p.grad = self.flat[off:off + k].view_as(p)
            self.views.append(p.grad)
            off += k

    def backward_into(self, loss):
        if self.flat.is_cuda:
            from . import ops
            with ops.deferred_weight_grads():
                grads = torch.autograd.grad(loss, self.params, allow_unused=True)
        else:
            grads = torch.autograd.grad(loss, self.params, allow_unused=True)
        dst = [v for v, g in zip(self.views, grads) if g is not None]
        src = [g for g in grads if g is not None]
        if len(src) != len(grads):
            self.flat.zero_()
        if self.captured_pack and self.flat.is_cuda and torch.cuda.is_current_stream_capturing() and src:
            from . import _ffi
            src = [g if g.is_contiguous() else g.contiguous() for g in src]
            tab = [[g.data_ptr() for g in src], [d.data_ptr() for d in dst],
                   [d.numel() for d in dst]]
            table = self._reserved_table.view(-1)[:3 * len(src)].view(3, len(src))
            blocks = max(1, min(64, max(tab[2]) // 4096))
            if self.sumsq_state is not None:
                _ffi.call("demf_multi_copy_sumsq", len(src), table.data_ptr(), blocks,
                          self.sumsq_state.data_ptr(), torch.cuda.current_stream().cuda_stream)
            else:
                _ffi.call("demf_multi_copy", len(src), table.data_ptr(), blocks,
                          torch.cuda.current_stream().cuda_stream)
            self._pending_tables.append((table, tab))
            return
        torch._foreach_copy_(dst, src)

    def reserve_table(self):
        self._reserved_table = torch.empty((3, len(self.params)), dtype=torch.int64,
                                           device=self.flat.device)

    def finish_capture(self):
        for table, tab in self._pending_tables:
            table.copy_(torch.tensor(tab, dtype=torch.int64))
            self._tables.append(table)
        self._reserved_table = None
        self._pending_tables = []

    def zero_(self):
        self.flat.zero_()

    def all_reduce_mean(self):
        if dist.is_initialized() and dist.get_world_size() > 1:
            dist.all_reduce(self.flat, op=dist.ReduceOp.SUM)
            self.flat.div_(dist.get_world_size())

    def clip_(self, max_norm):
        norm = torch.linalg.vector_norm(self.flat)
        self.flat.mul_(torch.clamp(max_norm / (norm + 1e-6), max=1.0))
        return norm


class FlatAdamW:

    def __init__(self, groups, flat_grads, betas=(0.9, 0.999), eps=1e-8):
        import ctypes
        params = flat_grads.params
        assert [id(p) for g in groups for p in g["params"] if p.requires_grad] == [id(p) for p in params]
        self.grads = flat_grads.flat
        self.flat = torch.empty_like(self.grads)
        off, self.segments = 0, []
        for g in groups:
            start = off
            for p in g["params"]:
                if not p.requires_grad:
                    continue
                k = p.numel()
                self.flat[off:off + k].copy_(p.data.reshape(-1))
                p.data = self.flat[off:off + k].view_as(p)
                off += k
            if off > start:
                self.segments.append((start, off - start, float(g["lr"]), float(g["weight_decay"])))
        if not 1 <= len(self.segments) <= 4:
            raise ValueError("FlatAdamW: %d parameter groups (demf_adamw_state_f32 takes 1..4)" % len(self.segments))
        n = len(self.segments)
        self._seg = ((ctypes.c_longlong * n)(*[s[0] for s in self.segments]),
                     (ctypes.c_longlong * n)(*[s[1] for s in self.segments]),
                     (ctypes.c_float * n)(*[s[2] for s in self.segments]),
                     (ctypes.c_float * n)(*[s[3] for s in self.segments]))
        self.params = params
        self.exp_avg = torch.zeros_like(self.flat)
        self.exp_avg_sq = torch.zeros_like(self.flat)
        self.betas, self.eps = betas, eps
        self.state = torch.zeros(64, dtype=torch.uint8, device=self.flat.device)
        self._lr_factor = 1.0
        self.state.view(torch.float32)[5] = 1.0

# ... 689 lines not shown
```

### demf_amd/fused.py

```python
import ctypes
import math

import torch
from torch.autograd import Function
from torch.autograd.function import once_differentiable

from . import _ffi

RELU, DROPOUT, GATE, ACCUM, ROWBIAS, ACCUM2 = 1, 2, 4, 8, 16, 32

OP_ATTN, OP_LN1, OP_LN2, OP_FFN, OP_LN3 = 1, 2, 3, 4, 5

_RNG = {}
ATTN_CORE = True
_DEBUG = None


def rng_state(device, seed=None):
    device = torch.device(device)
    if device.index is None:
        device = torch.device(device.type, torch.cuda.current_device())
    key = str(device)
    if key not in _RNG or seed is not None:
        s = torch.initial_seed() if seed is None else int(seed)
        t = torch.tensor([s & 0x7FFFFFFFFFFFFFFF, 0], dtype=torch.int64, device=device)
        if key in _RNG:
            _RNG[key].copy_(t)
        else:
            _RNG[key] = t
    return _RNG[key]


def advance_rng(device):
    _ffi.call("demf_rng_advance", rng_state(device).data_ptr(), torch.cuda.current_stream().cuda_stream)


def next_rng(device):
    state = rng_state(device)
    snap = torch.empty_like(state)
    _ffi.call("demf_rng_next", state.data_ptr(), snap.data_ptr(), torch.cuda.current_stream().cuda_stream)
    return snap


def peek_next_rng(device):
    snap = rng_state(device).clone()
    snap[1] += 1
    return snap


def get_rng_state(device):
    return [int(v) for v in rng_state(device).tolist()]


def set_rng_state(device, seed_step):
    rng_state(device).copy_(torch.tensor([int(seed_step[0]), int(seed_step[1])], dtype=torch.int64))


def dropout_mask(numel, p, op_id, device, state=None):
    out = torch.empty(numel, dtype=torch.float32, device=device)
    st = rng_state(device) if state is None else state
    _ffi.call("demf_dropout_mask", numel, float(p), st.data_ptr(), int(op_id),
              out.data_ptr(), torch.cuda.current_stream().cuda_stream)
    return out


def _st():
    return torch.cuda.current_stream().cuda_stream


def _p(t, off=0):
    return None if t is None else t.data_ptr() + 4 * off


def gemm(M, N, K, A, sa, B, sb, C, scm, *, batch=1, zdiv=1, sab=(0, 0), sbb=(0, 0), scb=(0, 0),
         A2=None, a2_cols=0, B2=None, b2_rows=0, C2=None, bias=None, sbias_b=0, rowscale=None,
         srs=(0, 0), alpha=1.0, flags=0, gate=None, sg=(0, 0), gate_scale=1.0, drop_p=0.0, rng=None,
         op_id=0, splitk=1, asum=None, group=None):
    d = _ffi.GemmDesc()
    d.M, d.N, d.K, d.batch, d.zdiv, d.splitk = M, N, K, batch, zdiv, splitk
    d.A, d.sam, d.sak, d.sab, d.sab2 = A, sa[0], sa[1], sab[0], sab[1]
    d.A2, d.a2_cols = A2, a2_cols
    d.B, d.sbn, d.sbk, d.sbb, d.sbb2 = B, sb[0], sb[1], sbb[0], sbb[1]
    d.B2, d.b2_rows = B2, b2_rows
    d.C, d.scm, d.scb, d.scb2 = C, scm, scb[0], scb[1]
    d.C2 = C2
    d.bias, d.sbias_b = bias, sbias_b
    d.rowscale, d.srs_m, d.srs_b = rowscale, srs[0], srs[1]
    d.alpha, d.flags = alpha, flags
    d.gate, d.sgm, d.sgb, d.gate_scale = gate, sg[0], sg[1], gate_scale
    d.drop_p, d.rng, d.op_id = drop_p, rng, op_id
    d.asum = asum
    if group is not None:
        group.append(d)
        return
    _ffi.call("demf_gemm_f32", ctypes.addressof(d), _st())


def gemm_group(descs):
    if not descs:
        return
    arr = (_ffi.GemmDesc * len(descs))(*descs)
    _ffi.call("demf_gemm_group_f32", ctypes.addressof(arr), len(descs), _st())


def _splitk(K):
    return max(1, min(16, K // 256))


def linear_fwd(x, w, b, out=None, **kw):
    R, K = x.shape
    N = w.shape[0]
    if out is None:
        out = torch.empty((R, N), dtype=torch.float32, device=x.device)
    gemm(R, N, K, _p(x), (K, 1), _p(w), (K, 1), _p(out), N, bias=_p(b), **kw)
    return out


def weight_grad(dy, x, dw, db=None, x2=None, dy_cols=None, dy_off=0, x2_rows=0, group=None):
    R = dy.shape[0]
    N, K = dw.shape
    ldy = dy.shape[1]
    fused_bias = db is not None and N % 4 == 0
    gemm(N, K, R, _p(dy, dy_off), (1, ldy), _p(x), (1, x.shape[1]), _p(dw), K,
         B2=_p(x2), b2_rows=x2_rows if x2 is not None else 0, splitk=_splitk(R),
         asum=_p(db) if fused_bias else None, group=group)
    if db is not None and not fused_bias:
        _ffi.call("demf_colsum_f32", R, N, ldy, _p(dy, dy_off), _p(db), _st())


class FusedDecoderLayer(Function):

    @staticmethod
    def forward(ctx, x, pos, pts, tokens, keep4, shapes, lsi, M, ab, vr, dims, training,
                in_w, in_b, out_w, out_b, g1, b1, off_w, off_b, aw_w, aw_b, vp_w, vp_b, op_w, op_b,
                g2, b2, f0_w, f0_b, f1_w, f1_b, g3, b3):
        B, Q, H, L, P, p_attn, p_ffn, eps = dims[:8]
        salt = 8 * (int(dims[8]) if len(dims) > 8 else 0)
        if not training:
            p_attn = p_ffn = 0.0
        dev = x.device
        R, E = x.shape
        Dh, F, Ct, S = E // H, f0_w.shape[0], tokens.shape[2], tokens.shape[1]
        HLP = H * L * P
        assert R == B * Q and x.is_contiguous() and pos.is_contiguous() and pts.is_contiguous()
        snap = next_rng(dev) if (p_attn > 0.0 or p_ffn > 0.0) else rng_state(dev)
        rng = snap.data_ptr()
        OP_ATTN, OP_LN1, OP_LN2, OP_FFN, OP_LN3 = (salt + o for o in (1, 2, 3, 4, 5))
        new = lambda *s: torch.empty(s, dtype=torch.float32, device=dev)
        st = _st()
        qkv = new(R, 3 * E)
        gemm(R, 3 * E, E, _p(x), (E, 1), _p(in_w), (E, 1), _p(qkv), 3 * E, A2=_p(pos), a2_cols=2 * E,
             bias=_p(in_b))
        att = new(R, E)
        core = ATTN_CORE and Q == 256 and Dh == 32
        if core:
            prob = pd = new(0)
            ast = new(B * H * Q, 2)
            dbg = _DEBUG is not None
            if dbg:
                prob, pd = new(B * H, Q, Q), new(B * H, Q, Q)
            _ffi.call("demf_attn_core_fwd", B, H, Q, Dh, _p(qkv), 1.0 / math.sqrt(Dh), p_attn, rng, OP_ATTN,
                      _p(att), _p(ast), _p(prob) if dbg else None, _p(pd) if dbg else None, st)
        else:
            ast = new(0)
            sc = new(B * H, Q, Q)
            zb = (Q * 3 * E, Dh)
            gemm(Q, Q, Dh, _p(qkv), (3 * E, 1), _p(qkv, E), (3 * E, 1), _p(sc), Q, batch=B * H, zdiv=H,
                 sab=zb, sbb=zb, scb=(H * Q * Q, Q * Q), alpha=1.0 / math.sqrt(Dh))
            prob, pd = new(B * H, Q, Q), sc
            _ffi.call("demf_softmax_dropout_fwd", B * H * Q, Q, _p(sc), p_attn, rng, OP_ATTN, _p(prob),
                      _p(pd), st)
            gemm(Q, Dh, Q, _p(pd), (Q, 1), _p(qkv, 2 * E), (1, 3 * E), _p(att), E, batch=B * H, zdiv=H,
                 sab=(H * Q * Q, Q * Q), sbb=zb, scb=(Q * E, Dh))
        s1 = linear_fwd(att, out_w, out_b)
        x1, st1 = new(R, E), new(R, 2)
        _ffi.call("demf_add_dropout_ln_fwd", R, E, _p(s1), _p(x), _p(g1), _p(b1), eps, p_attn, rng,
                  OP_LN1, _p(s1), _p(x1), _p(st1), st)
        raw = new(R, 3 * HLP)
        gemm(R, 2 * HLP, E, _p(x1), (E, 1), _p(off_w), (E, 1), _p(raw), 3 * HLP, A2=_p(pos),
             a2_cols=2 * HLP, bias=_p(off_b))
        gemm(R, HLP, E, _p(x1), (E, 1), _p(aw_w), (E, 1), _p(raw, 2 * HLP), 3 * HLP, A2=_p(pos),
             a2_cols=HLP, bias=_p(aw_b))
        loc, w, uvw = new(R, H, L, P, 2), new(R, H, L, P), new(R, 4)
        _ffi.call("demf_msda_prep_fwd", R, Q, H, L, P, _p(pts), _p(M), _p(ab), _p(vr), shapes.data_ptr(),
                  _p(raw), _p(loc), _p(w), _p(uvw), st)
        z, ks4 = new(R * H, Ct), new(R * H, 4)
        _ffi.call("demf_msda_fwd_bf16" if tokens.dtype == torch.bfloat16 else "demf_msda_fwd_f32", B, S, 1, Ct, L,
                  Q * H, P, _p(tokens), shapes.data_ptr(), lsi.data_ptr(), _p(loc), _p(w), _p(z), st)
        _ffi.call("demf_msda_fwd_f32", B, S, 1, 4, L, Q * H, P, _p(keep4), shapes.data_ptr(),
                  lsi.data_ptr(), _p(loc), _p(w), _p(ks4), st)
        mo = new(R, E)
        gemm(R, Dh, Ct, _p(z), (H * Ct, 1), _p(vp_w), (Ct, 1), _p(mo), E, batch=H, sab=(Ct, 0),
             sbb=(Dh * Ct, 0), scb=(Dh, 0), bias=_p(vp_b), sbias_b=Dh, rowscale=_p(ks4), srs=(4 * H, 4),
             flags=ROWBIAS)
        s2 = linear_fwd(mo, op_w, op_b)
        x2, st2 = new(R, E), new(R, 2)
        _ffi.call("demf_add_dropout_ln_fwd", R, E, _p(s2), _p(x1), _p(g2), _p(b2), eps, p_attn, rng,
                  OP_LN2, _p(s2), _p(x2), _p(st2), st)
        hid = new(R, F)
        gemm(R, F, E, _p(x2), (E, 1), _p(f0_w), (E, 1), _p(hid), F, bias=_p(f0_b),
             flags=RELU | (DROPOUT if p_ffn > 0 else 0), drop_p=p_ffn, rng=rng, op_id=OP_FFN)
        s3 = linear_fwd(hid, f1_w, f1_b)
        x3, st3 = new(R, E), new(R, 2)
        _ffi.call("demf_add_dropout_ln_fwd", R, E, _p(s3), _p(x2), _p(g3), _p(b3), eps, p_ffn, rng,
                  OP_LN3, _p(s3), _p(x3), _p(st3), st)
        ctx.dims = (B, Q, H, L, P, p_attn, p_ffn, eps, salt)
        ctx.core = core
        ctx.save_for_backward(snap, x, pos, pts, tokens, keep4, shapes, lsi, M, ab, vr, qkv, prob, pd, att, ast,
                              s1, st1, x1, w, loc, uvw, z, ks4, mo, s2, st2, x2, hid, s3, st3,
                              in_w, out_w, g1, off_w, aw_w, vp_w, vp_b, op_w, g2, f0_w, f1_w, g3)
        return x3

    @staticmethod
    @once_differentiable
    def backward(ctx, dx3):
        (snap, x, pos, pts, tokens, keep4, shapes, lsi, M, ab, vr, qkv, prob, pd, att, ast, s1, st1, x1, w, loc,
         uvw, z, ks4, mo, s2, st2, x2, hid, s3, st3, in_w, out_w, g1, off_w, aw_w, vp_w, vp_b, op_w,
         g2, f0_w, f1_w, g3) = ctx.saved_tensors
        B, Q, H, L, P, p_attn, p_ffn, eps, salt = ctx.dims
        OP_ATTN, OP_LN1, OP_LN2, OP_FFN, OP_LN3 = (salt + o for o in (1, 2, 3, 4, 5))
        dev = x.device
        R, E = x.shape
        Dh, F, Ct, S = E // H, f0_w.shape[0], tokens.shape[2], tokens.shape[1]
        HLP = H * L * P
        rng = snap.data_ptr()
        st = _st()
        new = lambda *s: torch.empty(s, dtype=torch.float32, device=dev)
        dx3 = dx3.contiguous()
        wg = []
        shp = [(3 * E, E), (3 * E,), (E, E), (E,), (E,), (E,), (2 * HLP, E), (2 * HLP,), (HLP, E), (HLP,),
               (E, Ct), (E,), (E, E), (E,), (E,), (E,), (F, E), (F,), (E, F), (E,), (E,), (E,)]
        sizes = [math.prod(s) for s in shp]
        from . import ops
        ws = ops.zeros(sum(sizes), dev)
        gr, o = [], 0
# ... 82 lines not shown
```

### demf_amd/modules/head.py

```python
import numpy as np
import torch
import torch.nn as nn
import torch.nn.functional as F

from .. import ops
from ..geometry import DepthBoxes, level_masks, rotation_3d_in_axis_z
from . import losses as L
from .coder import DeMFClassAgnosticBBoxCoder
from .pointnet2 import build_sa_module
from .transformer import DeMFTransformerDecoderLayer
from .vote import BaseConvBboxHead, VoteModule


BF16_TOKENS = True


def compose_projection(img_meta):
    A = np.eye(3)
    t = np.zeros(3)
    rot = np.asarray(img_meta.get("pcd_rotation", np.eye(3)), np.float64)
    scale = float(img_meta.get("pcd_scale_factor", 1.0))
    trans = np.asarray(img_meta.get("pcd_trans", np.zeros(3)), np.float64)
    for op in list(img_meta.get("transformation_3d_flow", []))[::-1]:
        if op == "T":
# ... 277 lines not shown
        p = torch.cat([seeds_3d_batch, ones], dim=-1) @ M.transpose(1, 2)
        uv = p[..., :2] / p[..., 2:3]
        uv = uv * ab[:, None, 0::2] + ab[:, None, 1::2]
        return torch.clamp(uv, 0, 1)

    def _sample_first(self, on_gpu, C0, S):
        att = self.decoder[0].layer.attentions[1]
        samples = self.num_proposal * att.num_levels * att.num_points * 4
        return bool(on_gpu and samples < S and C0 % 4 == 0 and C0 <= 256)

    def pyramid_tokens(self, mlvl_feats, img_metas, out=None):
        feats = list(mlvl_feats)
        on_gpu = feats[0].is_cuda and not any(f.requires_grad for f in feats) and all(f.is_contiguous() for f in feats)
        spatial = [tuple(f.shape[-2:]) for f in feats]
        S = sum(h * w for h, w in spatial)
        if not self._sample_first(on_gpu, feats[0].shape[1], S) or feats[0].dtype != torch.float32:
            return None
        mt = self._meta_tensors(img_metas, spatial, feats[0].device, feats[0].dtype)
        bf16 = BF16_TOKENS and ops.get_compute_dtype() == "bf16"
        if out is not None and list(out["spatial"]) != spatial:
            raise ValueError("pyramid_tokens: `out` holds levels %s, the pyramid has %s" % (out["spatial"], spatial))
        tokens = ops.pyramid_to_tokens(feats, mt["mask_u8"], bf16=bf16, out=None if out is None else out["tokens"])
        return out if out is not None else dict(tokens=tokens, spatial=spatial, padding_zeroed=True)

    def prepare_image_inputs(self, mlvl_feats, img_metas):
        prepared = False
        if isinstance(mlvl_feats, dict):
            spatial, feat_flatten = list(mlvl_feats["spatial"]), mlvl_feats["tokens"]
            on_gpu, C0 = feat_flatten.is_cuda and not feat_flatten.requires_grad, feat_flatten.shape[2]
            prepared = bool(mlvl_feats.get("padding_zeroed"))
        else:
            spatial = [tuple(f.shape[-2:]) for f in mlvl_feats]
            feat_flatten = None
            on_gpu = mlvl_feats[0].is_cuda and not any(f.requires_grad for f in mlvl_feats) and \
                all(f.is_contiguous() for f in mlvl_feats)
            C0 = mlvl_feats[0].shape[1]
        dev = mlvl_feats["tokens"].device if isinstance(mlvl_feats, dict) else mlvl_feats[0].device
        dt = mlvl_feats["tokens"].dtype if isinstance(mlvl_feats, dict) else mlvl_feats[0].dtype
        if dt == torch.bfloat16:
            dt = torch.float32
        mt = self._meta_tensors(img_metas, spatial, dev, dt)
        mask_flatten, valid_ratios = mt["mask_flatten"], mt["valid_ratios"]
        S = mask_flatten.shape[1]
        sample_first = self._sample_first(on_gpu, C0, S)
        if prepared and not sample_first:
            raise ValueError("tokens with zeroed padding rows serve the sample-then-project attention only")
        if feat_flatten is None:
            if on_gpu:
                feat_flatten = ops.pyramid_to_tokens(mlvl_feats, mt["mask_u8"] if sample_first else None,
                                                     bf16=sample_first and BF16_TOKENS and
                                                     ops.get_compute_dtype() == "bf16")
            else:
                feat_flatten = torch.cat([f.flatten(2).transpose(1, 2) for f in mlvl_feats], 1)
        elif sample_first and not prepared:
            feat_flatten = feat_flatten.masked_fill(mask_flatten.unsqueeze(-1), 0.0)
        value_tokens = (feat_flatten, mt["keep4"]) if sample_first else None
        value_projected = None
        feat_flatten = feat_flatten.permute(1, 0, 2)
        if value_tokens is None:
            value_projected = [layer.layer.attentions[1].project_value(feat_flatten, mask_flatten)
                               for layer in self.decoder]
        return dict(feat_flatten=feat_flatten, mask_flatten=mask_flatten, spatial=spatial,
                    spatial_shapes=mt["spatial_shapes"], level_start_index=mt["level_start_index"],
                    valid_ratios=valid_ratios, value_projected=value_projected,
                    value_tokens=value_tokens)

    def prepare_decoder_inputs(self, seeds_3d, mlvl_feats, img_metas):
        ii = self.prepare_image_inputs(mlvl_feats, img_metas)
        reference_points = self.get_reference_points(seeds_3d, img_metas, ii["spatial"])
        return ii["feat_flatten"], ii["mask_flatten"], reference_points, ii["spatial_shapes"], \
            ii["level_start_index"], ii["valid_ratios"]

    def loss(self, bbox_preds, points, gt_bboxes_3d, gt_labels_3d, pts_semantic_mask=None,
             pts_instance_mask=None, img_metas=None, gt_bboxes_ignore=None, vote_pack=None):
        bbox_preds = dict(bbox_preds)
        decode_res_all = bbox_preds.pop("decode_res_all")
        targets = self.get_targets(points, gt_bboxes_3d, gt_labels_3d, bbox_preds, vote_pack)
        assert self.num_fusion_layers + 1 == len(decode_res_all)
        if all(self._fusable(d) for d in decode_res_all):
            vecs, vote = zip(*[self._loss_fused(bbox_preds, targets, d["_rows"],
                                                 with_vote=(i == 0))
                               for i, d in enumerate(decode_res_all)])
            if vecs[0].is_cuda and len(vecs) <= 4:
                out8 = ops.loss_total(list(vecs), vote[0])
                mean7, total = out8[:7], out8[7]
            else:
                mean7 = vecs[0]
                for v in vecs[1:]:
                    mean7 = mean7 + v
                mean7 = mean7 / len(vecs)
                total = mean7.sum() + vote[0]
            losses = dict(vote_loss=vote[0])
            for i, name in enumerate(ops.HEAD_LOSS_NAMES):
                losses[name] = mean7[i]
            losses["_total"] = total
            return losses
        losses_all = [self._loss({**bbox_preds, **d}, targets) for d in decode_res_all]
        return {k: sum(l[k] for l in losses_all) / (self.num_fusion_layers + 1)
                for k in losses_all[0]}

    def _fusable(self, decode_res):
        rows = decode_res.get("_rows")
        c = self.loss_cfg
        return rows is not None and rows[0].is_cuda and rows[0].shape[-1] == 12 and \
            rows[1].shape[-1] == 30 and c["semantic"] is not None and bool(c["iou"])

    def _loss(self, bbox_preds, targets):
        (vote_targets, vote_target_masks, dir_class_targets, dir_res_targets, mask_targets,
         objectness_targets, objectness_weights, box_loss_weights, distance_targets,
         dir_targets, size_targets, center_targets) = targets
        c = self.loss_cfg
        if self._fusable(bbox_preds):
            seven, vote = self._loss_fused(bbox_preds, targets, bbox_preds["_rows"])
            losses = dict(vote_loss=vote)
            for i, name in enumerate(ops.HEAD_LOSS_NAMES):
                losses[name] = seven[i]
            return losses
        vote_loss = self.vote_module.get_loss(bbox_preds["seed_points"], bbox_preds["vote_points"],
                                              bbox_preds["seed_indices"], vote_target_masks,
                                              vote_targets)
        ocw = c["objectness"].get("class_weight")
        if ocw is not None:
            dev = bbox_preds["obj_scores"].device
            cw = self.__dict__.setdefault("_ocw", {})
            if str(dev) not in cw:
                cw[str(dev)] = torch.tensor(ocw, dtype=torch.float32, device=dev)
            ocw = cw[str(dev)]
        objectness_loss = L.cross_entropy_sum(bbox_preds["obj_scores"].transpose(2, 1),
                                              objectness_targets, objectness_weights, ocw,
                                              c["objectness"].get("loss_weight", 1.0))
        w3 = box_loss_weights.unsqueeze(-1).repeat(1, 1, 3)
        size_reg_loss = L.smooth_l1_sum(bbox_preds["size"], size_targets, w3,
                                        c["size_res"].get("beta", 1.0),
                                        c["size_res"].get("loss_weight", 1.0))
        center_loss = L.smooth_l1_sum(bbox_preds["center"], center_targets, w3,
                                      c["center"].get("beta", 1.0),
                                      c["center"].get("loss_weight", 1.0))
        dir_class_loss = L.cross_entropy_sum(bbox_preds["dir_class"].transpose(2, 1),
                                             dir_class_targets, box_loss_weights, None,
                                             c["dir_class"].get("loss_weight", 1.0))
        one_hot = F.one_hot(dir_class_targets, self.num_dir_bins).to(vote_targets.dtype)
        dir_res_norm = torch.sum(bbox_preds["dir_res_norm"] * one_hot, -1)
        dir_res_loss = L.smooth_l1_sum(dir_res_norm, dir_res_targets, box_loss_weights,
                                       c["dir_res"].get("beta", 1.0),
                                       c["dir_res"].get("loss_weight", 1.0))
        losses = dict(vote_loss=vote_loss, objectness_loss=objectness_loss,
                      dir_class_loss=dir_class_loss, dir_res_loss=dir_res_loss,
                      size_res_loss=size_reg_loss, center_loss=center_loss)
        if c["semantic"] is not None:
            losses["semantic_loss"] = L.cross_entropy_sum(
                bbox_preds["sem_scores"].transpose(2, 1), mask_targets, box_loss_weights, None,
                c["semantic"].get("loss_weight", 1.0))
        if c["iou"]:
            corners_pred = self.bbox_coder.decode_corners(bbox_preds["center"], bbox_preds["size"])
            corners_target = self.bbox_coder.decode_corners(center_targets, size_targets)
            losses["iou_loss"] = L.axis_aligned_iou_loss_sum(corners_pred, corners_target,
                                                             box_loss_weights,
                                                             c["iou"].get("loss_weight", 1.0))
        return losses

    def _loss_fused(self, bbox_preds, targets, rows, with_vote=True):
        (vote_targets, vote_target_masks, dir_class_targets, dir_res_targets, mask_targets,
         objectness_targets, objectness_weights, box_loss_weights, distance_targets,
         dir_targets, size_targets, center_targets) = targets
        c = self.loss_cfg
        cw = c["objectness"].get("class_weight") or [1.0, 1.0]
        hyper = (cw[0], cw[1], c["objectness"].get("loss_weight", 1.0),
                 c["dir_class"].get("loss_weight", 1.0), c["dir_res"].get("loss_weight", 1.0),
# ... 219 lines not shown
```

### demf_amd/ops.py

```python
import ctypes
import os

import torch
from torch.autograd import Function
from torch.autograd.function import once_differentiable

from . import _ffi

__all__ = [
    "set_compute_dtype", "get_compute_dtype", "gt_prep", "target_weights", "vote_combine", "furthest_point_sample", "ball_query", "grouping_operation", "gather_points",
    "three_nn", "three_nn_weights", "three_interpolate", "three_interpolate_cat_cl", "MultiScaleDeformableAttnFunction",
    "group_concat_cl", "gather_rows_cl", "three_interpolate_cl", "maxpool_ns", "shared_mlp_pool",
]


def _stream():
    return torch.cuda.current_stream().cuda_stream


LIBRARY_FALLBACK = bool(int(os.environ.get("DEMF_ALLOW_LIBRARY_FALLBACK", "0") or 0))


def library_fallback(what):
    if not LIBRARY_FALLBACK:
# ... 586 lines not shown
    return _ThreeInterpolateCatCL.apply(feat, idx, weight, skip)


def three_interpolate_cl(feat, idx, weight):
    return _ThreeInterpolateCL.apply(feat, idx, weight)


class _MaxPoolNS(Function):
    @staticmethod
    def forward(ctx, x):
        _chk(x, "x")
        R, ns, C = x.shape
        out = torch.empty((R, C), dtype=x.dtype, device=x.device)
        arg = torch.empty((R, C), dtype=torch.int32, device=x.device)
        _ffi.call("demf_maxpool_ns_fwd", R, ns, C, _p(x), _p(out), _p(arg), _stream())
        ctx.save_for_backward(arg)
        ctx.ns = ns
        return out

    @staticmethod
    @once_differentiable
    def backward(ctx, grad_out):
        (arg,) = ctx.saved_tensors
        grad_out = grad_out.contiguous()
        R, C = grad_out.shape
        gx = torch.empty((R, ctx.ns, C), dtype=grad_out.dtype, device=grad_out.device)
        _ffi.call("demf_maxpool_ns_bwd", R, ctx.ns, C, _p(grad_out), _p(arg), _p(gx), _stream())
        return gx


def maxpool_ns(x):
    return _MaxPoolNS.apply(x)


_IDENTITY_DY = {}


def _identity_dy_vectors(n, device):
    key = (n, str(device))
    if key not in _IDENTITY_DY:
        v = torch.zeros(5, n, dtype=torch.float32, device=device)
        v[1] = 1.0
        v[2] = 1.0
        _IDENTITY_DY[key] = v.reshape(-1).contiguous()
    return _IDENTITY_DY[key]


class _LinearRows(Function):

    @staticmethod
    def _rows_ok(R, K, N, x):
        return R > _OWN_GEMM_ROWS and K % 32 == 0 and N % 128 == 0 and x.stride(1) == 1 and x.stride(0) % 4 == 0

    @staticmethod
    def forward(ctx, x, weight, bias, row_mask):
        from . import fused
        ctx.has_bias = bias is not None
        R, K = x.shape
        N = weight.shape[0]
        if x.stride(1) != 1:
            x = x.contiguous()
        if bias is not None and not bias.is_contiguous():
            bias = bias.contiguous()
        y = torch.empty((R, N), dtype=torch.float32, device=x.device)
        planes = 1 if get_compute_dtype() == "bf16" else 3
        if _LinearRows._rows_ok(R, K, N, x):
            rows_gemm(x, split_planes(weight, planes), bias.detach() if bias is not None else None, y,
                      row_mask=row_mask, mask_col0=0)
        else:
            fused.gemm(R, N, K, _p(x), (x.stride(0), 1), _p(weight), weight.stride(), _p(y), N, bias=_p(bias))
            if row_mask is not None:
                y.masked_fill_(row_mask.unsqueeze(-1), 0.0)
        if row_mask is not None:
            ctx.save_for_backward(x, weight, row_mask)
        else:
            ctx.save_for_backward(x, weight)
        return y

    @staticmethod
    @once_differentiable
    def backward(ctx, g):
        from . import fused
        x, weight = ctx.saved_tensors[:2]
        g = g.contiguous()
        R, K = x.shape
        N = weight.shape[0]
        if len(ctx.saved_tensors) == 3:
            g.masked_fill_(ctx.saved_tensors[2].unsqueeze(-1), 0.0)
        gx = gw = gb = None
        Np, gq, wq = N, g, weight
        if N % 4 != 0 and R >= 4096 and len(ctx.saved_tensors) == 2:
            Np = (N + 3) // 4 * 4
            gq = zeros((R, Np), g.device)
            gq[:, :N].copy_(g)
            wq = zeros((Np, K), g.device)
            wq[:N].copy_(weight)
        if ctx.needs_input_grad[0]:
            gx = torch.empty((R, K), dtype=torch.float32, device=g.device)
            if Np != N:
                fused.gemm(R, K, Np, _p(gq), (Np, 1), _p(wq), (1, K), _p(gx), K)
            elif _LinearRows._rows_ok(R, N, K, g):
                planes = 1 if get_compute_dtype() == "bf16" else 3
                rows_gemm(g, split_planes(weight.detach().t().contiguous(), planes), None, gx)
            else:
                fused.gemm(R, K, N, _p(g), (N, 1), _p(weight), (weight.stride(1), weight.stride(0)), _p(gx), K)
        want_b = ctx.has_bias and ctx.needs_input_grad[2]
        if ctx.needs_input_grad[1] or want_b:
            ws = zeros(Np * K + Np, g.device)
            gw = ws[:Np * K].view(Np, K)
            gb = ws[Np * K:] if ctx.has_bias else None
            in_gemm = False
            if Np != N:
                in_gemm = gb is not None
                fused.gemm(Np, K, R, _p(gq), (1, Np), _p(x), (1, x.stride(0)), _p(gw), K,
                           splitk=fused._splitk(R), asum=_p(gb) if in_gemm else None)
                if gb is not None and not in_gemm:
                    _ffi.call("demf_colsum_f32", R, Np, Np, _p(gq), _p(gb), _stream())
                return gx, gw[:N], (gb[:N] if gb is not None else None), None
            if R >= 32768 and N % 4 == 0 and K % 4 == 0 and x.is_contiguous():
                _ffi.call("demf_mlp_gemm_bwd_dw", R, N, K, K, _p(g), None, None, 1, _p(g),
                          _p(_identity_dy_vectors(N, g.device)), _p(x), None, _p(gw), _stream())
            else:
                in_gemm = gb is not None and N % 4 == 0 and N >= 4
                fused.gemm(N, K, R, _p(g), (1, N), _p(x), (1, x.stride(0)), _p(gw), K,
                           splitk=fused._splitk(R), asum=_p(gb) if in_gemm else None)
            if gb is not None and not in_gemm:
                _ffi.call("demf_colsum_f32", R, N, N, _p(g), _p(gb), _stream())
        return gx, gw, gb, None


def linear(x, weight, bias=None, row_mask=None):
    if not x.is_cuda:
        raise RuntimeError("x must be a GPU (HIP) tensor: demf_amd operators have no CPU path")
    lead = x.shape[:-1]
    y = _LinearRows.apply(x.reshape(-1, x.shape[-1]), weight, bias,
                          None if row_mask is None else row_mask.reshape(-1))
    return y.view(*lead, weight.shape[0])


def split_planes(w, planes=3):
    w = w.detach().float().contiguous()
    h = w.to(torch.bfloat16)
    if planes == 1:
        return h.unsqueeze(0).contiguous()
    r = w - h.float()
    m = r.to(torch.bfloat16)
    low = (r - m.float()).to(torch.bfloat16)
    return torch.stack([h, m, low]).contiguous()


def rows_gemm(x, w_planes, bias, out, a2=None, a2_cols=0, relu=False, ln=None, row_mask=None, mask_col0=0,
              a2_replace=False):
    R, K = x.shape
    planes, N, Kw = w_planes.shape
    if not (x.is_cuda and out.is_cuda and w_planes.is_cuda):
        raise RuntimeError("rows_gemm: operands must be GPU (HIP) tensors: demf_amd operators have no CPU path")
    assert x.dtype == torch.float32 and out.dtype == torch.float32, "rows_gemm: fp32 rows in, fp32 rows out"
    assert Kw == K and out.shape == (R, N) and x.stride(1) == 1 and out.stride(1) == 1
    assert w_planes.dtype == torch.bfloat16 and w_planes.is_contiguous()
    mode = 2 if ln is not None else (1 if relu else 0)
    res, g, b, eps = ln if ln is not None else (None, None, None, 0.0)
    if a2 is not None:
        assert a2.shape == x.shape and a2.stride() == x.stride() and a2.is_cuda and a2.dtype == torch.float32
    if row_mask is not None:
        assert row_mask.dtype == torch.bool and row_mask.numel() == R and row_mask.is_contiguous() and row_mask.is_cuda
    for name, v, n in (("bias", bias, N), ("gamma", g, N), ("beta", b, N)):
        assert v is None or (v.is_cuda and v.dtype == torch.float32 and v.is_contiguous() and v.numel() == n), \
            "rows_gemm: %s must be a contiguous fp32 GPU vector of %d elements" % (name, n)
    if res is not None:
        assert res.is_cuda and res.dtype == torch.float32 and tuple(res.shape) == (R, N) and res.stride(1) == 1 and \
            res.stride(0) % 4 == 0 and out.stride(0) % 4 == 0, "rows_gemm: residual must be fp32 (R,N) rows"
    _ffi.call("demf_rows_gemm_f32", R, N, K, _p(x), x.stride(0), _p(a2), int(a2_cols), int(bool(a2_replace)),
              _p(w_planes), planes,
              _p(bias), mode, _p(row_mask), int(mask_col0), _p(res), res.stride(0) if res is not None else 0,
              _p(g), _p(b), float(eps), _p(out), out.stride(0), _stream())
    return out


def _gpu_f32(name, *ts):
    for t in ts:
        if t is None:
            continue
        if not t.is_cuda:
            raise RuntimeError(name + ": operands must be GPU (HIP) tensors: demf_amd operators have no CPU path")
        if t.dtype != torch.float32 or not t.is_contiguous():
            raise ValueError(name + ": contiguous fp32 tensors required")


def conv_weight_planes(weight, planes=3, scale=None):
    w = weight.detach().float()
    if scale is not None:
        w = w * scale.detach().float().view(-1, 1, 1, 1)
    return split_planes(w.permute(0, 2, 3, 1).reshape(w.shape[0], -1), planes)


def stem_weight_planes(weight, planes=3, scale=None):
    w = weight.detach().float()
    assert tuple(w.shape[1:]) == (3, 7, 7)
    if scale is not None:
        w = w * scale.detach().float().view(-1, 1, 1, 1)
    full = w.new_zeros(w.shape[0], 7, 8, 4)
    full[:, :, :7, :3] = w.permute(0, 2, 3, 1)
    return split_planes(full.reshape(w.shape[0], 224), planes)


def conv_nhwc(x, w_planes, bias, KH, KW, stride=1, pad=0, resid=None, relu=False, out=None, ksplit=None):
    B, H, W, Cin = x.shape
    planes, Cout, K = w_planes.shape
    _gpu_f32("conv_nhwc", x, bias, resid, out)
    assert K == KH * KW * Cin and w_planes.dtype == torch.bfloat16 and w_planes.is_contiguous() and w_planes.is_cuda
# ... 518 lines not shown
                                  _p(Ys[l - 1]), _p(sss[l - 1]), _p(mis[l - 1]), _p(g12p), st)
                        g12_pending = g12p
                elif K % 4 == 0:
                    _ffi.call("demf_mlp_gemm_bwd_dx_w", R, N, K, K, _p(G), _p(dP if sparse else None),
                              _p(arg if sparse else None), ns, _p(Ys[l]), _p(vec6), _p(W), _p(dX), st)
                else:
                    Wtt = W.t().contiguous()
                    _ffi.call("demf_mlp_gemm_bwd_dx", R, N, K, K, _p(G), _p(dP if sparse else None),
                              _p(arg if sparse else None), ns, _p(Ys[l]), _p(vec6), _p(Wtt), _p(dX),
                              st)
                if l > 0:
                    G = dX
                else:
                    dx = dX
        return (dx, None, None, None, None, None,
                dxyz if ctx.needs_input_grad[6] else None,
                dcenter if ctx.needs_input_grad[7] else None, *grads)


def shared_mlp_pool(x, ns, layers, training=True, eps=1e-5, momentum=0.1, geo=None):
    flat = []
    for layer in layers:
        W, gamma, beta, rmean, rvar = layer[:5]
        bias = layer[5] if len(layer) > 5 else None
        nbt = layer[6] if len(layer) > 6 and training else None
        if not training and bias is not None:
            rmean = rmean - bias.detach()
        flat += [W, gamma, beta, rmean, rvar, bias, nbt]
    gx = gc = None
    if geo is not None and torch.is_grad_enabled():
        gx = geo[0] if geo[0].requires_grad else None
        gc = geo[1] if geo[1].requires_grad else None
    return _SharedMLPPool.apply(x, ns, training, eps, momentum, geo, gx, gc, *flat)


class _L2NormRows(Function):
    @staticmethod
    def forward(ctx, x):
        _chk(x, "x")
        R, C = x.shape
        y = torch.empty_like(x)
        norm = torch.empty(R, dtype=torch.float32, device=x.device)
        _ffi.call("demf_l2norm_rows_fwd", R, C, _p(x), _p(y), _p(norm), _stream())
        ctx.save_for_backward(y, norm)
        return y

    @staticmethod
    @once_differentiable
    def backward(ctx, dy):
        y, norm = ctx.saved_tensors
        dy = dy.contiguous()
        dx = torch.empty_like(y)
        _ffi.call("demf_l2norm_rows_bwd", y.shape[0], y.shape[1], _p(y), _p(norm), _p(dy), _p(dx), _stream())
        return dx


def l2norm_rows(x):
    return _L2NormRows.apply(x)


class _VoteCombine(Function):
    @staticmethod
    def forward(ctx, rows, votes, seed_xyz):
        _chk(rows, "rows")
        _chk(votes, "votes")
        _chk(seed_xyz, "seed_xyz")
        R, C = rows.shape
        assert votes.shape == (R, C + 3) and seed_xyz.numel() == 3 * R
        vote_xyz = torch.empty_like(seed_xyz)
        y = torch.empty_like(rows)
        norm = torch.empty(R, dtype=torch.float32, device=rows.device)
        _ffi.call("demf_vote_combine_fwd", R, C, _p(rows), _p(votes), _p(seed_xyz), _p(vote_xyz), _p(y),
                  _p(norm), _stream())
        ctx.save_for_backward(y, norm)
        return vote_xyz, y

    @staticmethod
    @once_differentiable
    def backward(ctx, dxyz, dy):
        y, norm = ctx.saved_tensors
        R, C = y.shape
        dxyz = None if dxyz is None else dxyz.contiguous()
        dy = None if dy is None else dy.contiguous()
        dvotes = torch.empty((R, C + 3), dtype=torch.float32, device=y.device)
        drows = torch.empty_like(y)
        _ffi.call("demf_vote_combine_bwd", R, C, _p(y), _p(norm), _p(dy), _p(dxyz), _p(dvotes),
                  _p(drows), _stream())
        return drows, dvotes, (dxyz if ctx.needs_input_grad[2] else None)


def vote_combine(rows, votes, seed_xyz):
    return _VoteCombine.apply(rows.contiguous(), votes.contiguous(), seed_xyz.contiguous())


import ctypes as _ct

HEAD_LOSS_NAMES = ("objectness_loss", "dir_class_loss", "dir_res_loss", "size_res_loss",
                   "center_loss", "semantic_loss", "iou_loss")


class _HeadLoss(Function):
    @staticmethod
    def forward(ctx, cls_rows, reg_rows, base, hyper, center_t, size_t, dir_class_t, dir_res_t,
                sem_t, obj_t, obj_w, box_w):
        for t, n in ((cls_rows, "cls"), (reg_rows, "reg"), (base, "base"), (center_t, "center_t"),
                     (size_t, "size_t"), (dir_res_t, "dir_res_t"), (obj_w, "obj_w"), (box_w, "box_w")):
            _chk(t, n)
        for t, n in ((dir_class_t, "dir_class_t"), (sem_t, "sem_t"), (obj_t, "obj_t")):
            _chk(t, n, torch.int64)
        R = cls_rows.shape[0]
        assert cls_rows.shape[1] == 12 and reg_rows.shape[1] == 30
        hp = (_ct.c_float * 12)(*hyper)
        out = zeros(7, cls_rows.device)
        _ffi.call("demf_head_loss_fwd", R, 12, 10, hp, _p(cls_rows), _p(reg_rows), _p(base),
                  _p(center_t), _p(size_t), _p(dir_class_t), _p(dir_res_t), _p(sem_t), _p(obj_t),
                  _p(obj_w), _p(box_w), _p(out), _stream())
        ctx.save_for_backward(cls_rows, reg_rows, base, center_t, size_t, dir_class_t, dir_res_t,
                              sem_t, obj_t, obj_w, box_w)
        ctx.hyper = tuple(hyper)
        return out

    @staticmethod
    @once_differentiable
    def backward(ctx, grad_out):
        cls_rows, reg_rows, base = ctx.saved_tensors[:3]
        rest = ctx.saved_tensors[3:]
        R = cls_rows.shape[0]
        hp = (_ct.c_float * 12)(*ctx.hyper)
        gout = grad_out.contiguous()
        gc, gr, gb = torch.empty_like(cls_rows), torch.empty_like(reg_rows), torch.empty_like(base)
        _ffi.call("demf_head_loss_bwd", R, 12, 10, hp, _p(cls_rows), _p(reg_rows), _p(base),
                  *[_p(t) for t in rest], _p(gout), _p(gc), _p(gr), _p(gb), _stream())
        return (gc, gr, gb) + (None,) * 9


def head_loss(cls_rows, reg_rows, base_xyz, hyper12, center_t, size_t, dir_class_t, dir_res_t,
              sem_t, obj_t, obj_w, box_w):
    return _HeadLoss.apply(cls_rows, reg_rows, base_xyz, hyper12, center_t, size_t, dir_class_t,
                           dir_res_t, sem_t, obj_t, obj_w, box_w)


class _VoteLoss(Function):
    @staticmethod
    def forward(ctx, vote_points, seed_points, seed_indices, masks, vote_targets, gt_per_seed,
                dst_weight):
        _chk(vote_points, "vote_points")
        _chk(seed_points, "seed_points")
        _chk(seed_indices, "seed_indices", torch.int64)
        _chk(masks, "vote_target_masks", torch.int64)
        _chk(vote_targets, "vote_targets")
        B, S, _ = seed_points.shape
        N = masks.shape[1]
        msum = torch.empty(1, dtype=torch.float32, device=vote_points.device)
        out = zeros(1, vote_points.device)
        _ffi.call("demf_vote_loss_fwd", B, S, N, int(gt_per_seed), float(dst_weight), _p(seed_points),
                  _p(vote_points), _p(seed_indices), _p(masks), _p(vote_targets), _p(msum),
                  _p(out), _stream())
        ctx.save_for_backward(vote_points, seed_points, seed_indices, masks, vote_targets, msum)
        ctx.meta = (B, S, N, int(gt_per_seed), float(dst_weight))
        return out[0]

    @staticmethod
    @once_differentiable
    def backward(ctx, grad_out):
        vote_points, seed_points, seed_indices, masks, vote_targets, msum = ctx.saved_tensors
        B, S, N, gps, w = ctx.meta
        g = grad_out.reshape(1).contiguous()
        gv = torch.empty_like(vote_points)
        _ffi.call("demf_vote_loss", B, S, N, gps, w, _p(seed_points), _p(vote_points),
                  _p(seed_indices), _p(masks), _p(vote_targets), _p(msum), _p(g), None, _p(gv),
                  _stream())
        return gv, None, None, None, None, None, None


def vote_loss(vote_points, seed_points, seed_indices, vote_target_masks, vote_targets, gt_per_seed,
              dst_weight):
    return _VoteLoss.apply(vote_points.contiguous(), seed_points.contiguous(), seed_indices.contiguous(),
                           vote_target_masks.contiguous(), vote_targets.contiguous(), gt_per_seed,
                           dst_weight)


def gt_prep(gt, labels_padded, num_dir_bins):
    _chk(gt, "gt")
    _chk(labels_padded, "labels", torch.int64)
    B, G = gt.shape[:2]
    dev = gt.device
    f = lambda *sh: torch.empty(sh, dtype=torch.float32, device=dev)
    out = dict(cs=f(B, G), sn=f(B, G), dir_class=torch.empty((B, G), dtype=torch.int64, device=dev),
               dir_res=f(B, G), valid_u8=torch.empty((B, G), dtype=torch.uint8, device=dev),
               lab=torch.empty((B, G), dtype=torch.int64, device=dev), center=f(B, G, 3))
    _ffi.call("demf_gt_prep", B, G, int(num_dir_bins), _p(gt), _p(labels_padded), _p(out["cs"]),
              _p(out["sn"]), _p(out["dir_class"]), _p(out["dir_res"]), _p(out["valid_u8"]),
              _p(out["lab"]), _p(out["center"]), _stream())
    out["valid"] = out["valid_u8"].view(torch.bool)
    return out


def pad_gt_lists(boxes, labels, G, out=None):
    B = len(boxes)
    dev = boxes[0].device
    keep = []
    for i in range(B):
        b, l = boxes[i], labels[i]
        if b.dtype != torch.float32 or not b.is_contiguous():
            b = b.float().contiguous()
        if l.dtype != torch.int64 or not l.is_contiguous():
            l = l.long().contiguous()
        keep.append((b, l))
    counts = (ctypes.c_int * B)(*[int(b.shape[0]) for b, _ in keep])
    dims = (ctypes.c_int * B)(*[int(b.shape[1]) if b.dim() == 2 else 7 for b, _ in keep])
    bp = (ctypes.c_void_p * B)(*[b.data_ptr() if b.numel() else None for b, _ in keep])
    lp = (ctypes.c_void_p * B)(*[l.data_ptr() if l.numel() else None for _, l in keep])
    if out is not None:
        gt, lab = out
        assert tuple(gt.shape) == (B, G, 7) and tuple(lab.shape) == (B, G) and gt.is_contiguous() and \
            lab.is_contiguous() and gt.dtype == torch.float32 and lab.dtype == torch.int64
    else:
        gt = torch.empty((B, G, 7), dtype=torch.float32, device=dev)
        lab = torch.empty((B, G), dtype=torch.int64, device=dev)
    valid = torch.empty((B, G), dtype=torch.uint8, device=dev)
    _ffi.call("demf_pad_gt", B, int(G), ctypes.addressof(counts), ctypes.addressof(dims), ctypes.addressof(bp),
              ctypes.addressof(lp), _p(gt), _p(lab), _p(valid), _stream())
    return gt, lab, valid.view(torch.bool)


@torch.no_grad()
def query_pos_rows(reg_rows, base_xyz):
    _chk(base_xyz, "base_xyz")
    B, Q, nreg = reg_rows.shape
    reg = reg_rows if reg_rows.is_contiguous() else reg_rows.contiguous()
    _chk(reg, "reg_rows")
    out = torch.empty((B * Q, 8), dtype=torch.float32, device=reg.device)
    _ffi.call("demf_query_pos_rows", B * Q, nreg, _p(reg), _p(base_xyz), _p(out), _stream())
    return out


class _LossTotal(Function):
    @staticmethod
    def forward(ctx, vote, *vecs):
        n = len(vecs)
        vecs = [v.contiguous() for v in vecs]
        out = torch.empty(8, dtype=torch.float32, device=vecs[0].device)
        tab = (ctypes.c_void_p * n)(*[v.data_ptr() for v in vecs])
        _ffi.call("demf_loss_total", n, ctypes.addressof(tab), _p(vote), _p(out), _stream())
        ctx.n, ctx.has_vote = n, vote is not None
        return out

    @staticmethod
    def backward(ctx, g8):
        g8 = g8.contiguous()
        gv = torch.empty((ctx.n, 7), dtype=torch.float32, device=g8.device)
        gvote = torch.empty(1, dtype=torch.float32, device=g8.device) if ctx.has_vote else None
        _ffi.call("demf_loss_total_bwd", ctx.n, _p(g8), _p(gv), _p(gvote), _stream())
        return (gvote,) + tuple(gv[i] for i in range(ctx.n))


def loss_total(vecs, vote=None):
    assert 1 <= len(vecs) <= 4
    for v in vecs:
        _chk(v, "loss vector")
    return _LossTotal.apply(None if vote is None else vote.reshape(1), *vecs)


def target_weights(objectness_masks, objectness_targets):
    _chk(objectness_masks, "objectness_masks")
    _chk(objectness_targets, "objectness_targets", torch.int64)
    ow = torch.empty_like(objectness_masks)
    bw = torch.empty_like(objectness_masks)
    _ffi.call("demf_target_weights", objectness_masks.numel(), _p(objectness_masks),
              _p(objectness_targets), _p(ow), _p(bw), _stream())
    return ow, bw


def vote_targets(points, gt, valid, prep=None):
    _chk(points, "points")
    _chk(gt, "gt")
    B, N, stride = points.shape
    G = gt.shape[1]
    if prep is not None:
        cs, sn, v = prep["cs"], prep["sn"], prep["valid_u8"]
    else:
        yaw = gt[..., 6]
        cs, sn = torch.cos(-yaw).contiguous(), torch.sin(-yaw).contiguous()
        v = valid.to(torch.uint8).contiguous()
    vt = torch.empty((B, N, 9), dtype=torch.float32, device=points.device)
    mask = torch.empty((B, N), dtype=torch.int64, device=points.device)
    _ffi.call("demf_vote_targets", B, N, stride, G, _p(points), _p(gt), _p(cs), _p(sn), _p(v),
              _p(vt), _p(mask), _stream())
    return vt, mask


def proposal_targets(agg, gt, lab, valid, dir_class, dir_res, with_rot, pos_thr, neg_thr, res_scale,
                     prep=None):
    _chk(agg, "agg")
    _chk(gt, "gt")
    B, Q, _ = agg.shape
    G = gt.shape[1]
    dev = agg.device
    if prep is not None:
        cs, sn, valid_u8 = prep["cs"], prep["sn"], prep["valid_u8"]
    else:
        yaw = gt[..., 6]
        cs, sn = torch.cos(-yaw).contiguous(), torch.sin(-yaw).contiguous()
        valid_u8 = valid.to(torch.uint8).contiguous()
    f = lambda *s: torch.empty(s, dtype=torch.float32, device=dev)
    l = lambda *s: torch.empty(s, dtype=torch.int64, device=dev)
    out = dict(center=f(B, Q, 3), size=f(B, Q, 3), dir_class=l(B, Q), dir_res=f(B, Q), dir=f(B, Q),
               mask=l(B, Q), distance=f(B, Q, 6), objectness=l(B, Q), objectness_masks=f(B, Q))
    _ffi.call("demf_proposal_targets", B, Q, G, int(bool(with_rot)), float(pos_thr), float(neg_thr),
              float(res_scale), _p(agg), _p(gt), _p(cs), _p(sn), _p(dir_class.contiguous()),
              _p(dir_res.contiguous()), _p(lab.contiguous()), _p(valid_u8),
              _p(out["center"]), _p(out["size"]), _p(out["dir_class"]), _p(out["dir_res"]),
              _p(out["dir"]), _p(out["mask"]), _p(out["distance"]), _p(out["objectness"]),
              _p(out["objectness_masks"]), _stream())
    return out


def box_extent_count(points, boxes7, cos_sin=None):
    _chk(points, "points")
    _chk(boxes7, "boxes7")
    B, N, stride = points.shape
    K = boxes7.shape[1]
    if cos_sin is not None:
        c, s = _chk(cos_sin[0], "cos"), _chk(cos_sin[1], "sin")
    else:
        yaw = boxes7[..., 6]
        c, s = torch.cos(yaw).contiguous(), torch.sin(yaw).contiguous()
    out = torch.empty_like(boxes7)
    ext = torch.empty((B, K, 6), dtype=torch.float32, device=points.device)
    cnt = torch.empty((B, K), dtype=torch.int32, device=points.device)
    _ffi.call("demf_box_extent_count", B, N, stride, K, _p(points), _p(boxes7), _p(c), _p(s),
              _p(out), _p(ext), _p(cnt), _stream())
    return out, ext, cnt


def aligned_nms(extent, scores, classes, valid, iou_thr, as_bytes=False):
    _chk(extent, "extent")
    _chk(scores, "scores")
    _chk(classes, "classes", torch.int64)
    B, K = scores.shape
    keep = torch.empty((B, K), dtype=torch.uint8, device=scores.device)
    valid = valid.contiguous().view(torch.uint8) if valid.dtype == torch.bool else valid.to(torch.uint8).contiguous()
    _ffi.call("demf_aligned_nms", B, K, float(iou_thr), _p(extent), _p(scores), _p(classes),
              _p(valid), _p(keep), _stream())
# ... 269 lines not shown
```

### include/demf_hip.h

```cpp
#ifndef DEMF_HIP_H_
#define DEMF_HIP_H_

#include <stdint.h>

#ifdef __cplusplus
extern "C" {
#endif

typedef void* demf_stream_t;

#define DEMF_OK 0
#define DEMF_EINVAL (-1)
#define DEMF_ELAUNCH (-2)
#define DEMF_EUNSUPPORTED (-3)

#define DEMF_ABI_VERSION 2

#define DEMF_INTERNAL

int demf_version(void);
const char* demf_last_error(void);

DEMF_INTERNAL int demf_stream_create_cu_masked(const int* cus, int n, int invert, void** out);

// ... 71 lines not shown
                        demf_stream_t stream);

DEMF_INTERNAL int demf_invert_index(int B, int N, int E, const int* idx, int* off, int* rows, demf_stream_t stream);
DEMF_INTERNAL int demf_invert_index_ws(int B, int N, int E, const int* idx, int* off, int* rows, int* workspace,
                         demf_stream_t stream);

DEMF_INTERNAL int demf_sa_index_chain(int B, int N, int nlev, const int* const* idx, const int* samples, int64_t* const* out,
                        demf_stream_t stream);
DEMF_INTERNAL int demf_split_points(long long rows, int C, const float* points, float* xyz, float* feat, demf_stream_t stream);

DEMF_INTERNAL int demf_group_concat_cl_bwd_gather(int B, int N, int E, int C, int ldo, int feat_col,
                                    const float* grad_out, const int* off, const int* rows,
                                    float* grad_feat, demf_stream_t stream);

DEMF_INTERNAL int demf_group_first_fwd(int B, int N, int M, int ns, int C1, float radius, int normalize_xyz,
                         const float* xyz, const float* center, const int* idx, const float* U,
                         const float* Wx, int w_ld ,
                         float* Y, double* stats,
                         const float* gamma, const float* beta, float eps, float momentum, float* running_mean,
                         float* running_var, long long* num_batches_tracked, float* scale_shift, float* mean_invstd,
                         const float* conv_bias, demf_stream_t stream);
DEMF_INTERNAL int demf_group_first_bwd(int B, int N, int M, int ns, int C1, float radius, int normalize_xyz,
                         const float* xyz, const float* center, const float* G, const float* Y,
                         const float* U ,
                         const float* vec6, const int* inv_off, const int* inv_rows, float* dU,
                         float* dWx, int dw_ld ,
                         const float* Wx , int w_ld ,
                         float* dxyz ,
                         float* dcenter ,
                         double* wacc ,
                         demf_stream_t stream);

DEMF_INTERNAL int demf_nchw_to_tokens(int B, int C, int HW, int S, int row0, const float* src,
                        const unsigned char* mask, float* dst, demf_stream_t stream);
DEMF_INTERNAL int demf_pyramid_to_tokens(int B, int C, int S, int nlev, const float* const* srcs, const int* hws,
                           const unsigned char* mask, float* dst, demf_stream_t stream);
DEMF_INTERNAL int demf_pyramid_to_tokens_bf16(int B, int C, int S, int nlev, const float* const* srcs, const int* hws,
                                const unsigned char* mask, uint16_t* dst, demf_stream_t stream);

DEMF_INTERNAL int demf_colsum_f32(int R, int N, int ld, const float* x, float* out, demf_stream_t stream);


DEMF_INTERNAL int demf_mlp_gemm_fwd(int R, int K, int N, int ldx, const float* X,
                      const float* pro_scale_shift, const float* Wt, float* Y,
                      double* stats, demf_stream_t stream);

DEMF_INTERNAL int demf_mlp_gemm_fwd_pool(int R, int K, int N, int ldx, const float* X,
                           const float* pro_scale_shift, const float* Wt, float* Y, double* stats,
                           int ns, float* pmax, float* pmin, int* amax, int* amin,
                           demf_stream_t stream);

DEMF_INTERNAL int demf_mlp_gemm_fwd_bn(int R, int K, int N, int ldx, const float* X, const float* pro_scale_shift,
                         const float* Wt, float* Y, double* stats, const float* gamma,
                         const float* beta, float eps, float momentum, float* running_mean,
                         float* running_var, long long* num_batches_tracked, float* scale_shift,
                         float* mean_invstd, const float* conv_bias, demf_stream_t stream);
DEMF_INTERNAL int demf_mlp_gemm_fwd_pool_bn(int R, int K, int N, int ldx, const float* X,
                              const float* pro_scale_shift, const float* Wt, float* Y, double* stats,
                              int ns, float* pmax, float* pmin, int* amax, int* amin,
                              const float* gamma, const float* beta, float eps, float momentum,
                              float* running_mean, float* running_var,
                              long long* num_batches_tracked, float* scale_shift,
                              float* mean_invstd, const float* conv_bias, demf_stream_t stream);

DEMF_INTERNAL int demf_pool_select(int Rp, int C, const float* pmax, const float* pmin, const int* amax,
                     const int* amin, const float* scale_shift, float* out, int* arg, float* yraw,
                     demf_stream_t stream);

DEMF_INTERNAL int demf_pool_select_slot0(int Rp, int C, const float* pmax, const int* amax, const float* scale_shift,
                           float* out, int* arg, float* yraw, demf_stream_t stream);

DEMF_INTERNAL int demf_bn_finalize(int N, long long count, double* stats, const float* gamma,
                     const float* beta, float eps, float momentum, float* running_mean,
                     float* running_var, long long* num_batches_tracked, float* scale_shift,
                     float* mean_invstd, const float* conv_bias, demf_stream_t stream);

DEMF_INTERNAL int demf_l2norm_rows_fwd(int R, int C, const float* x, float* y, float* norm, demf_stream_t stream);
DEMF_INTERNAL int demf_l2norm_rows_bwd(int R, int C, const float* y, const float* norm, const float* dy, float* dx,
                         demf_stream_t stream);

DEMF_INTERNAL int demf_vote_combine_fwd(int R, int C, const float* rows, const float* votes, const float* seed_xyz,
                          float* vote_xyz, float* vote_feats, float* norm, demf_stream_t stream);
DEMF_INTERNAL int demf_vote_combine_bwd(int R, int C, const float* vote_feats, const float* norm,
                          const float* d_vote_feats, const float* d_vote_xyz, float* d_votes,
                          float* d_rows, demf_stream_t stream);

DEMF_INTERNAL int demf_bnrelu_maxpool_fwd(int R, int ns, int C, const float* Y, const float* scale_shift,
                            float* out, int* arg, demf_stream_t stream);

DEMF_INTERNAL int demf_bn_bwd_reduce(int R, int N, int ns, const float* G, const float* dP, const int* arg,
                       const float* Y, const float* yraw, const float* scale_shift,
                       const float* mean_invstd, double* g12, demf_stream_t stream);

DEMF_INTERNAL int demf_bn_bwd_vectors(int N, long long count, double* g12, const float* gamma,
                        const float* scale_shift, const float* mean_invstd, float* vec6,
                        float* dgamma, float* dbeta, demf_stream_t stream);

DEMF_INTERNAL int demf_mlp_gemm_bwd_dx(int R, int N, int K, int ldo, const float* G, const float* dP,
                         const int* arg, int ns, const float* Y, const float* vec6,
                         const float* Wtt, float* dX, demf_stream_t stream);
DEMF_INTERNAL int demf_mlp_gemm_bwd_dx_w(int R, int N, int K, int ldo, const float* G, const float* dP,
                         const int* arg, int ns, const float* Y, const float* vec6,
                         const float* W, float* dX, demf_stream_t stream);
DEMF_INTERNAL int demf_mlp_gemm_bwd_dx_red(int R, int N, int K, int ldo, const float* G, const float* dP,
                             const int* arg, int ns, const float* Y, const float* vec6,
                             const float* W, float* dX, const float* Yprev,
                             const float* scale_shift_prev, const float* mean_invstd_prev,
                             double* g12_prev, demf_stream_t stream);

DEMF_INTERNAL int demf_mlp_gemm_bwd_dx_first(int R, int N, int K0, const float* G, const float* Y1,
                               const float* vec6, const float* W1, const float* X0,
                               const float* Y0, const float* scale_shift0,
                               const float* mean_invstd0, double* sums, demf_stream_t stream);
DEMF_INTERNAL int demf_mlp_first_finish(int N0, long long count, double* sums, const float* gamma0,
                          const float* mean_invstd0, float* dW0, float* dgamma0, float* dbeta0,
                          demf_stream_t stream);

DEMF_INTERNAL int demf_mlp_gemm_bwd_dx_red_v(int R, int N, int K, int ldo, const float* G, const float* dP,
                               const int* arg, int ns, const float* Y, const float* vec6,
                               const float* W, float* dX, const float* Yprev,
                               const float* scale_shift_prev, const float* mean_invstd_prev,
                               double* g12_prev, const float* gamma_prev, float* vec6_prev,
                               float* dgamma_prev, float* dbeta_prev, demf_stream_t stream);
DEMF_INTERNAL int demf_bn_bwd_reduce_vectors(int R, int N, int ns, const float* dP, const int* arg, const float* Y,
                               const float* yraw, const float* scale_shift, const float* mean_invstd,
                               double* g12, const float* gamma, float* vec6, float* dgamma, float* dbeta,
                               int y_bf16, demf_stream_t stream);

DEMF_INTERNAL int demf_mlp_gemm_fwd_bn_st(int R, int K, int N, int ldx, const void* X, const float* pro_scale_shift,
                            const float* Wt, void* Y, double* stats, const float* gamma,
                            const float* beta, float eps, float momentum, float* running_mean,
                            float* running_var, long long* num_batches_tracked, float* scale_shift,
                            float* mean_invstd, const float* conv_bias, int store_flags,
                            demf_stream_t stream);
DEMF_INTERNAL int demf_mlp_gemm_fwd_pool_bn_st(int R, int K, int N, int ldx, const void* X,
                                 const float* pro_scale_shift, const float* Wt, void* Y, double* stats,
                                 int ns, float* pmax, int* amax, const float* gamma, const float* beta,
                                 float eps, float momentum, float* running_mean, float* running_var,
                                 long long* num_batches_tracked, float* scale_shift, float* mean_invstd,
                                 const float* conv_bias, int store_flags, demf_stream_t stream);

DEMF_INTERNAL int demf_mlp_bwd_fused(int R, int N, int K, const float* G, const float* dP, const int* arg, int ns,
                       const float* Y, const float* vec6, const float* W, const float* Yprev,
                       const float* scale_shift_prev, const float* mean_invstd_prev, float* dX,
                       float* dW, double* g12_prev, const float* X0, double* first_sums,
                       const float* gamma_prev, float* vec6_prev, float* dgamma_prev, float* dbeta_prev,
                       int store_flags, demf_stream_t stream);
DEMF_INTERNAL int demf_mlp_bwd_fused_cols(int R, int N, int Ktot, int c0, int Kc, const float* G, const float* dP,
                            const int* arg, int ns, const float* Y, const float* vec6, const float* W,
                            const float* Yprev, const float* scale_shift_prev,
                            const float* mean_invstd_prev, float* dX, float* dW, double* g12_prev,
                            const float* gamma_prev, float* vec6_prev, float* dgamma_prev,
                            float* dbeta_prev, demf_stream_t stream);

DEMF_INTERNAL int demf_mlp_first_stats(int R, int N0, const float* X, const float* W0, double* moments, const float* gamma,
                         const float* beta, float eps, float momentum, float* running_mean,
                         float* running_var, long long* num_batches_tracked, float* scale_shift,
                         float* mean_invstd, const float* conv_bias, demf_stream_t stream);
DEMF_INTERNAL int demf_mlp_gemm_fwd_bn_x4(int R, int N, const float* X4, const float* W0, const float* prev_scale_shift,
                            const float* Wt, float* Y, double* stats, const float* gamma, const float* beta,
                            float eps, float momentum, float* running_mean, float* running_var,
                            long long* num_batches_tracked, float* scale_shift, float* mean_invstd,
                            const float* conv_bias, demf_stream_t stream);
DEMF_INTERNAL int demf_mlp_bwd_fused_x4(int R, int N, int K, const float* G, const float* Y, const float* vec6,
                          const float* W, const float* X0, const float* W0, const float* scale_shift_prev,
                          const float* mean_invstd_prev, float* dW, double* first_sums, demf_stream_t stream);

// ... 32 lines not shown
                       const float* cls, const float* reg, const float* base_xyz,
                       const float* center_t, const float* size_t_, const int64_t* dir_class_t,
                       const float* dir_res_t, const int64_t* sem_t, const int64_t* obj_t,
                       const float* obj_w, const float* box_w, float* out7,
                       demf_stream_t stream);
DEMF_INTERNAL int demf_head_loss_bwd(int R, int num_dir_bins, int num_classes, const float* hyper12,
                       const float* cls, const float* reg, const float* base_xyz,
                       const float* center_t, const float* size_t_, const int64_t* dir_class_t,
                       const float* dir_res_t, const int64_t* sem_t, const int64_t* obj_t,
                       const float* obj_w, const float* box_w, const float* grad_out7,
                       float* grad_cls, float* grad_reg, float* grad_base,
                       demf_stream_t stream);

DEMF_INTERNAL int demf_vote_loss(int B, int S, int N, int gt_per_seed, float dst_weight,
                   const float* seed_points, const float* vote_points,
                   const int64_t* seed_indices, const int64_t* vote_target_masks,
                   const float* vote_targets, const float* mask_sum, const float* grad_out,
                   float* out, float* grad_vote, demf_stream_t stream);
DEMF_INTERNAL int demf_vote_loss_fwd(int B, int S, int N, int gt_per_seed, float dst_weight,
                       const float* seed_points, const float* vote_points,
                       const int64_t* seed_indices, const int64_t* vote_target_masks,
                       const float* vote_targets, float* mask_sum_out, float* out,
                       demf_stream_t stream);


int demf_msda_fwd_f32(int B, int S, int H, int Dh, int L, int Q, int P,
                      const float* value, const int64_t* spatial_shapes,
                      const int64_t* level_start_index, const float* sampling_loc,
                      const float* attn_weight, float* out, demf_stream_t stream);

int demf_msda_bwd_f32(int B, int S, int H, int Dh, int L, int Q, int P,
                      const float* value, const int64_t* spatial_shapes,
                      const int64_t* level_start_index, const float* sampling_loc,
                      const float* attn_weight, const float* grad_out,
                      float* grad_value, float* grad_sampling_loc,
                      float* grad_attn_weight, demf_stream_t stream);

DEMF_INTERNAL int demf_msda_fwd_bf16(int B, int S, int H, int Dh, int L, int Q, int P,
                       const uint16_t* value, const int64_t* spatial_shapes,
                       const int64_t* level_start_index, const float* sampling_loc,
                       const float* attn_weight, float* out, demf_stream_t stream);
DEMF_INTERNAL int demf_msda_bwd_bf16(int B, int S, int H, int Dh, int L, int Q, int P,
                       const uint16_t* value, const int64_t* spatial_shapes,
                       const int64_t* level_start_index, const float* sampling_loc,
                       const float* attn_weight, const float* grad_out,
                       float* grad_value, float* grad_sampling_loc,
                       float* grad_attn_weight, demf_stream_t stream);

DEMF_INTERNAL int demf_rows_gemm_f32(int R, int N, int K, const float* A, long long lda, const float* A2, int a2_cols,
                       int a2_op ,
                       const void* w_planes, int planes, const float* bias, int mode,
                       const unsigned char* row_mask, int mask_col0, const float* resid, long long ldr,
                       const float* gamma, const float* beta, float eps, float* C, long long ldc,
                       demf_stream_t stream);
DEMF_INTERNAL int demf_rows_ln_pos_f32(int R, int C, const float* x, const float* resid, const float* gamma, const float* beta,
                         float eps, const float* pos, float* y, float* ypos, demf_stream_t stream);
DEMF_INTERNAL int demf_msda_fwd_raw_f32(int B, int S, int H, int Dh, int L, int Q, int P, const float* value,
                          long long vpitch, const int64_t* spatial_shapes, const int64_t* level_start_index,
                          const float* raw, long long ldraw, int off_col0, int lgt_col0, const float* ref,
                          float* out, demf_stream_t stream);
DEMF_INTERNAL int demf_msda_fwd_raw_head_f32(int B, int S, int Q, int P, const float* value, long long vpitch,
                               const int64_t* spatial_shapes, const int64_t* level_start_index, const float* raw,
                               long long ldraw, int off_col0, int lgt_col0, const float* ref, float* out,
                               int first_staged_level, int staged_tokens, demf_stream_t stream);

DEMF_INTERNAL int demf_vote_targets(int B, int N, int point_stride, int G, const float* points,
                      const float* gt_boxes, const float* cos_neg_yaw, const float* sin_neg_yaw,
                      const unsigned char* valid, float* vote_targets, int64_t* vote_target_masks,
                      demf_stream_t stream);

DEMF_INTERNAL int demf_proposal_targets(int B, int Q, int G, int with_rot, float pos_thr, float neg_thr,
                          float res_scale, const float* aggregated_points, const float* gt_boxes,
                          const float* cos_neg_yaw, const float* sin_neg_yaw,
                          const int64_t* gt_dir_class, const float* gt_dir_res,
                          const int64_t* gt_labels, const unsigned char* valid,
                          float* center_targets, float* size_targets, int64_t* dir_class_targets,
                          float* dir_res_targets, float* dir_targets, int64_t* mask_targets,
                          float* distance_targets, int64_t* objectness_targets,
                          float* objectness_masks, demf_stream_t stream);

DEMF_INTERNAL int demf_query_pos_rows(int R, int nreg, const float* reg_rows, const float* base_xyz, float* out8,
                        demf_stream_t stream);

DEMF_INTERNAL int demf_loss_total(int n, const float* const* vecs, const float* vote, float* out8, demf_stream_t stream);
DEMF_INTERNAL int demf_loss_total_bwd(int n, const float* g8, float* gvecs, float* gvote, demf_stream_t stream);

DEMF_INTERNAL int demf_pad_gt(int B, int G, const int* counts, const int* box_dims, const void* const* boxes,
                const void* const* labels, float* gt_padded, int64_t* labels_padded,
                unsigned char* valid, demf_stream_t stream);

DEMF_INTERNAL int demf_gt_prep(int B, int G, int num_dir_bins, const float* gt_boxes, const int64_t* labels_padded,
                 float* cos_neg_yaw, float* sin_neg_yaw, int64_t* gt_dir_class, float* gt_dir_res,
                 unsigned char* valid, int64_t* labels_clamped, float* gravity_center,
                 demf_stream_t stream);

DEMF_INTERNAL int demf_target_weights(int R, const float* objectness_masks, const int64_t* objectness_targets,
                        float* objectness_weights, float* box_loss_weights, demf_stream_t stream);


DEMF_INTERNAL int demf_box_extent_count(int B, int N, int point_stride, int K, const float* points,
                          const float* boxes7, const float* cos_yaw, const float* sin_yaw,
                          float* boxes_bottom, float* extent6, int* count, demf_stream_t stream);

DEMF_INTERNAL int demf_aligned_nms(int B, int K, float iou_thr, const float* extent6, const float* scores,
                     const int64_t* classes, const unsigned char* valid, unsigned char* keep,
                     demf_stream_t stream);

typedef struct demf_detect_layer {
  int K;
  float res_scale;
  const float* center; int center_sb, center_sk;
  const float* center_base; int base_sb, base_sk;
  const float* size; int size_sb, size_sk;
  const float* dir_class; int dir_class_sb, dir_class_sk;
  const float* dir_res; int dir_res_sb, dir_res_sk;
  const float* obj; int obj_sb, obj_sk;
  const float* sem; int sem_sb, sem_sk;
} demf_detect_layer;

DEMF_INTERNAL int demf_detect_decode(int B, int K, int L, int C, int num_dir_bins, int with_rot,
                       const demf_detect_layer* layers, float* box7, float* cos_yaw, float* sin_yaw,
                       float* obj, float* sem, int64_t* classes, demf_stream_t stream);

DEMF_INTERNAL int demf_detect_pack(int B, int K, int C, int per_class, float score_thr,
                     const unsigned char* keep, const float* obj, const float* sem, const int64_t* classes,
                     const float* boxes_bottom, int first_scene, int max_scenes, int max_rows, float* boxes,
                     float* scores, int* labels, int* scene_off, int* state, demf_stream_t stream);


DEMF_INTERNAL int demf_box3d_iou(int N, int M, const float* boxes1, const float* boxes2, float* iou,
                   demf_stream_t stream);

DEMF_INTERNAL int demf_eval_match(int S, int T, const float* thresholds, int max_pred, int max_gt,
                    const float* pred_boxes, const int* order, const int* pred_off, const float* gt_boxes,
                    const int* gt_off, unsigned char* tp, demf_stream_t stream);

DEMF_INTERNAL int demf_eval_ap(int C, int T, const int* cls_off, const int* npos, const int* ws_off,
                 const unsigned char* tp_sorted, int* workspace, double* ap, double* rec, demf_stream_t stream);


DEMF_INTERNAL int demf_points_floor(int B, int load_dim, long long total, const float* raw, const int64_t* offsets,
                      float* floor_out, demf_stream_t stream);

DEMF_INTERNAL int demf_points_prep(int B, int num_points, int load_dim, long long total, const float* raw,
                     const int64_t* offsets, const float* floor_in, const float* params, const int64_t* seeds,
                     float* out, int* src_index, demf_stream_t stream);

DEMF_INTERNAL int demf_image_prep(int B, int Hp, int Wp, long long src_bytes, const unsigned char* src,
                    const int64_t* offsets, const int* shapes, const float* mean_std, float* out,
                    demf_stream_t stream);

DEMF_INTERNAL int demf_adamw_f32(long long n, float* param, const float* grad, float* exp_avg, float* exp_avg_sq,
                   const float* grad_norm, float max_norm, float grad_scale, float lr, float beta1,
                   float beta2, float eps, float weight_decay, int step, demf_stream_t stream);

DEMF_INTERNAL int demf_multi_copy_sumsq(int n, const void* table, int blocks_per_segment, void* opt_state,
                          demf_stream_t stream);
DEMF_INTERNAL int demf_sumsq_f32(long long n, const float* x, void* opt_state, demf_stream_t stream);
DEMF_INTERNAL int demf_adamw_state_f32(int nseg, const long long* seg_start, const long long* seg_n, const float* seg_lr,
                         const float* seg_weight_decay, float* param, const float* grad, float* exp_avg,
                         float* exp_avg_sq, void* opt_state, float max_norm, float grad_scale, float beta1,
                         float beta2, float eps, demf_stream_t stream);

#define DEMF_METER_ROW_WORDS 16
#define DEMF_METER_HEAD_WORDS 6
#define DEMF_METER_MAX_SCALARS 10
#define DEMF_METER_FLAG_GRAD_NORM (1u << 16)
DEMF_INTERNAL int demf_step_meter(int n, const float* const* scalars, const void* opt_state, float grad_scale,
                    float max_norm, void* ring, int rows, demf_stream_t stream);


#define DEMF_GEMM_RELU 1
#define DEMF_GEMM_DROPOUT 2
#define DEMF_GEMM_GATE 4
#define DEMF_GEMM_ACCUM 8
#define DEMF_GEMM_ROWBIAS 16
#define DEMF_GEMM_ACCUM2 32
#define DEMF_GEMM_FP32 64

typedef struct demf_gemm_desc {
  int M, N, K, batch, zdiv, splitk;
  const float* A; long long sam, sak, sab, sab2;
  const float* A2; int a2_cols;
  const float* B; long long sbn, sbk, sbb, sbb2;
  const float* B2; int b2_rows;
  float* C; long long scm, scb, scb2;
  float* C2;
  const float* bias; long long sbias_b;
  const float* rowscale; long long srs_m, srs_b;
  float alpha;
  int flags;
  const float* gate; long long sgm, sgb;
  float gate_scale;
  float drop_p;
  const void* rng;
  int op_id;
  float* asum;
} demf_gemm_desc;

DEMF_INTERNAL int demf_gemm_f32(const demf_gemm_desc* desc, demf_stream_t stream);
DEMF_INTERNAL int demf_gemm_group_f32(const demf_gemm_desc* descs, int n, demf_stream_t stream);

DEMF_INTERNAL int demf_set_compute_dtype(int mode);
DEMF_INTERNAL int demf_set_f16_terms(int on);
DEMF_INTERNAL int demf_get_compute_dtype(void);

typedef struct demf_ctx {
  int compute_mode;
  int reserved[7];
} demf_ctx;
DEMF_INTERNAL int demf_ctx_push(const demf_ctx* ctx);
DEMF_INTERNAL int demf_ctx_pop(void);
DEMF_INTERNAL int demf_gemm_f32_ctx(const demf_ctx* ctx, const demf_gemm_desc* desc, demf_stream_t stream);
DEMF_INTERNAL int demf_gemm_group_f32_ctx(const demf_ctx* ctx, const demf_gemm_desc* descs, int n, demf_stream_t stream);
DEMF_INTERNAL int demf_mlp_gemm_fwd_ctx(const demf_ctx* ctx, int R, int K, int N, int ldx, const float* X,
                          const float* pro_scale_shift, const float* Wt, float* Y, double* stats,
                          demf_stream_t stream);

DEMF_INTERNAL int demf_attn_core_fwd(int B, int H, int Q, int Dh, const float* qkv, float scale, float p, const void* rng,
                       int op_id, float* out, float* stats, float* prob, float* prob_dropped,
                       demf_stream_t stream);
DEMF_INTERNAL int demf_attn_core_bwd(int B, int H, int Q, int Dh, const float* qkv, const float* out, const float* dout,
                       const float* stats, float scale, float p, const void* rng, int op_id, float* dqkv,
                       demf_stream_t stream);

DEMF_INTERNAL int demf_add_dropout_ln_fwd(int R, int C, const float* x, const float* identity, const float* gamma,
                            const float* beta, float eps, float p, const void* rng, int op_id,
                            float* s_out, float* y, float* stats, demf_stream_t stream);
DEMF_INTERNAL int demf_add_dropout_ln_bwd(int R, int C, const float* dy, const float* dy2, const float* s,
                            const float* stats, const float* gamma, float p, const void* rng, int op_id,
                            float* ds_out, int ds_accum, float* dx_out, float* dgamma, float* dbeta,
                            demf_stream_t stream);
DEMF_INTERNAL int demf_softmax_dropout_fwd(int R, int S, const float* scores, float p, const void* rng, int op_id,
                             float* prob, float* out, demf_stream_t stream);
DEMF_INTERNAL int demf_softmax_dropout_bwd(int R, int S, const float* prob, float p, const void* rng, int op_id,
                             float* dio, demf_stream_t stream);
DEMF_INTERNAL int demf_msda_prep_fwd(int R, int Q, int H, int L, int P, const float* pts, const float* M,
                       const float* ab, const float* valid_ratios, const int64_t* shapes,
                       const float* raw, float* loc, float* w, float* uvw, demf_stream_t stream);
DEMF_INTERNAL int demf_msda_prep_bwd(int R, int Q, int H, int L, int P, const float* pts, const float* M,
                       const float* ab, const float* valid_ratios, const int64_t* shapes,
                       const float* w, const float* uvw, const float* dloc, const float* dloc2,
                       const float* dw, const float* dw2, float* draw, float* dpts,
                       demf_stream_t stream);
DEMF_INTERNAL int demf_rng_advance(void* rng, demf_stream_t stream);
DEMF_INTERNAL int demf_rng_next(void* rng, void* snapshot, demf_stream_t stream);
DEMF_INTERNAL int demf_dropout_mask(long long n, float p, const void* rng, int op_id, float* out,
                      demf_stream_t stream);

DEMF_INTERNAL int demf_multi_copy(int n, const void* table, int blocks_per_segment, demf_stream_t stream);
DEMF_INTERNAL int demf_zero_f32(long long n, float* x, demf_stream_t stream);


DEMF_INTERNAL int demf_conv_nhwc_f32(int B, int H, int W, int Cin, int Cout, int KH, int KW, int stride, int pad,
                       const float* x, const void* w_planes, int planes, const float* bias,
                       const float* resid, int relu, int ksplit, float* y, demf_stream_t stream);
DEMF_INTERNAL int demf_conv_stem7_nhwc4_f32(int B, int H, int W, int Cout, const float* x4, const void* w_planes, int planes,
                              const float* bias, int relu, float* y, demf_stream_t stream);
DEMF_INTERNAL int demf_maxpool3x3s2_nhwc_f32(int B, int H, int W, int C, const float* x, float* y, demf_stream_t stream);
DEMF_INTERNAL int demf_nchw3_to_nhwc4_f32(int B, int H, int W, const float* x, float* y, demf_stream_t stream);
DEMF_INTERNAL int demf_groupnorm_nhwc_f32(int B, int HW, int C, int G, float eps, const float* x, const float* gamma,
                            const float* beta, double* sums, float* y, long long y_batch_stride,
                            demf_stream_t stream);

#ifdef __cplusplus
}
#endif
#endif
```

Baseline: 1813 scenes/s.

## Cut small launches: fold RNG advance into GEMM, emit scalar loss, drop padding copies

Moves the per-layer RNG advance into the first thread of the first GEMM launch, which removes a separate tiny kernel. The loss kernel now also writes the scalar total, and backward can be seeded with a cached unit tensor, so autograd no longer needs a fill or an index-select backward. The GEMM staging loads now handle ragged tails, which lets linear backward pass strided or non-multiple-of-4 gradients directly instead of zero-padding copies. The vote-combine backward writes into a padded leading dimension. The risks are extra branches in the GEMM load path and a race if other blocks read the RNG state while block 0 updates it.

```diff
diff --git a/demf_amd/_ffi.py b/demf_amd/_ffi.py
--- a/demf_amd/_ffi.py
+++ b/demf_amd/_ffi.py
@@ -58,8 +58,8 @@
     "demf_gt_prep": [_c_int] * 3 + [_ptr] * 10,
     "demf_pad_gt": [_c_int] * 2 + [_ptr] * 8,
     "demf_query_pos_rows": [_c_int] * 2 + [_ptr] * 4,
-    "demf_loss_total": [_c_int] + [_ptr] * 4,
-    "demf_loss_total_bwd": [_c_int] + [_ptr] * 4,
+    "demf_loss_total": [_c_int] + [_ptr] * 5,
+    "demf_loss_total_bwd": [_c_int] + [_ptr] * 2 + [_c_int] + [_ptr] * 3,
     "demf_target_weights": [_c_int] + [_ptr] * 5,
     "demf_rows_ln_pos_f32": [_c_int] * 2 + [_ptr] * 4 + [_c_float] + [_ptr] * 4,
     "demf_rows_gemm_f32": [_c_int] * 3 + [_ptr, ctypes.c_longlong, _ptr, _c_int, _c_int, _ptr, _c_int, _ptr, _c_int, _ptr, _c_int,
@@ -98,7 +98,7 @@
     "demf_l2norm_rows_fwd": [_c_int] * 2 + [_ptr] * 4,
     "demf_l2norm_rows_bwd": [_c_int] * 2 + [_ptr] * 5,
     "demf_vote_combine_fwd": [_c_int] * 2 + [_ptr] * 7,
-    "demf_vote_combine_bwd": [_c_int] * 2 + [_ptr] * 7,
+    "demf_vote_combine_bwd": [_c_int] * 2 + [_ptr] * 5 + [_c_int] + [_ptr] * 2,
     "demf_bnrelu_maxpool_fwd": [_c_int] * 3 + [_ptr] * 5,
     "demf_bn_bwd_reduce": [_c_int] * 3 + [_ptr] * 9,
     "demf_bn_bwd_vectors": [_c_int, ctypes.c_longlong] + [_ptr] * 8,
@@ -181,6 +181,7 @@
         ("rng", _ptr),
         ("op_id", _c_int),
         ("asum", _ptr),
+        ("rng_snap", _ptr),
     ]
 
 _lib = None
diff --git a/demf_amd/csrc/dense.hip b/demf_amd/csrc/dense.hip
--- a/demf_amd/csrc/dense.hip
+++ b/demf_amd/csrc/dense.hip
@@ -18,6 +18,25 @@
 
 constexpr int G_BM = 64, G_BN = 64, G_BK = 64, G_LD = G_BK + 4;
 
+__device__ __forceinline__ float4 load_tail4(const float* __restrict__ p, int n) {
+  float4 v = make_float4(p[0], 0.f, 0.f, 0.f);
+  if (n > 1) v.y = p[1];
+  if (n > 2) v.z = p[2];
+  return v;
+}
+
+__device__ __forceinline__ void rng_next(unsigned long long* rng, unsigned long long* snap) {
+  const unsigned long long s = rng[1] + 1;
+  rng[1] = s;
+  snap[0] = rng[0];
+  snap[1] = s;
+}
+__global__ void rng_next_k(unsigned long long* rng, unsigned long long* snap) { rng_next(rng, snap); }
+__device__ __forceinline__ void gemm_rng_next(const demf_gemm_desc& p) {
+  if ((p.flags & DEMF_GEMM_RNG_NEXT) && threadIdx.x == 0 && blockIdx.x == 0 && blockIdx.y == 0 && blockIdx.z == 0)
+    rng_next((unsigned long long*)p.rng, (unsigned long long*)p.rng_snap);
+}
+
 struct GemmRegs {
   float4 v[4], w[4];
 };
@@ -35,8 +54,13 @@
       if constexpr (ADD2) g.w[i] = g.v[i];
       if (r0 + row < R && k0 + kq < K1) {
         const size_t o = (size_t)(r0 + row) * sr + k0 + kq;
-        g.v[i] = *reinterpret_cast<const float4*>(P + o);
-        if constexpr (ADD2) g.w[i] = *reinterpret_cast<const float4*>(P2 + o);
+        if (k0 + kq + 4 <= K1) {
+          g.v[i] = *reinterpret_cast<const float4*>(P + o);
+          if constexpr (ADD2) g.w[i] = *reinterpret_cast<const float4*>(P2 + o);
+        } else {
+          g.v[i] = load_tail4(P + o, K1 - k0 - kq);
+          if constexpr (ADD2) g.w[i] = load_tail4(P2 + o, K1 - k0 - kq);
+        }
       }
     }
   } else if constexpr (mode == 2) {
@@ -47,8 +71,13 @@
       if constexpr (ADD2) g.w[i] = g.v[i];
       if (k0 + k < K1 && r0 + rq < R) {
         const size_t o = (size_t)(k0 + k) * sk + r0 + rq;
-        g.v[i] = *reinterpret_cast<const float4*>(P + o);
-        if constexpr (ADD2) g.w[i] = *reinterpret_cast<const float4*>(P2 + o);
+        if (r0 + rq + 4 <= R) {
+          g.v[i] = *reinterpret_cast<const float4*>(P + o);
+          if constexpr (ADD2) g.w[i] = *reinterpret_cast<const float4*>(P2 + o);
+        } else {
+          g.v[i] = load_tail4(P + o, R - r0 - rq);
+          if constexpr (ADD2) g.w[i] = load_tail4(P2 + o, R - r0 - rq);
+        }
       }
     }
   } else {
@@ -173,6 +202,7 @@
   const int lane = threadIdx.x & 63, wave = threadIdx.x >> 6;
   const int lr = lane & 31, lh = lane >> 5;
   const int wm = wave & 1, wn = wave >> 1;
+  gemm_rng_next(p);
   int bx = blockIdx.x, by = blockIdx.y;
   xcd_rows(bx, by, gridDim.x, gridDim.y);
   const int m0 = by * G_BM, n0 = bx * G_BN;
@@ -274,8 +304,13 @@
       if constexpr (ADD2) g.w[i] = g.v[i];
       if (r0 + row < R && k0 + kq < K1) {
         const size_t o = (size_t)(r0 + row) * sr + k0 + kq;
-        g.v[i] = *reinterpret_cast<const float4*>(P + o);
-        if constexpr (ADD2) g.w[i] = *reinterpret_cast<const float4*>(P2 + o);
+        if (k0 + kq + 4 <= K1) {
+          g.v[i] = *reinterpret_cast<const float4*>(P + o);
+          if constexpr (ADD2) g.w[i] = *reinterpret_cast<const float4*>(P2 + o);
+        } else {
+          g.v[i] = load_tail4(P + o, K1 - k0 - kq);
+          if constexpr (ADD2) g.w[i] = load_tail4(P2 + o, K1 - k0 - kq);
+        }
       }
     }
   } else if constexpr (mode == 2) {
@@ -286,8 +321,13 @@
       if constexpr (ADD2) g.w[i] = g.v[i];
       if (k0 + k < K1 && r0 + rq < R) {
         const size_t o = (size_t)(k0 + k) * sk + r0 + rq;
-        g.v[i] = *reinterpret_cast<const float4*>(P + o);
-        if constexpr (ADD2) g.w[i] = *reinterpret_cast<const float4*>(P2 + o);
+        if (r0 + rq + 4 <= R) {
+          g.v[i] = *reinterpret_cast<const float4*>(P + o);
+          if constexpr (ADD2) g.w[i] = *reinterpret_cast<const float4*>(P2 + o);
+        } else {
+          g.v[i] = load_tail4(P + o, R - r0 - rq);
+          if constexpr (ADD2) g.w[i] = load_tail4(P2 + o, R - r0 - rq);
+        }
       }
     }
   } else {
@@ -457,6 +497,7 @@
   __shared__ __attribute__((aligned(16))) float s_a[32 * G_LD];
   __shared__ __attribute__((aligned(16))) float s_b[32 * G_LD];
   __shared__ float s_red[4][16][64];
+  gemm_rng_next(p);
   int bx = blockIdx.x, by = blockIdx.y;
   xcd_rows(bx, by, gridDim.x, gridDim.y);
   gemm_ks_body<MA, MB, ADD, BF16>(p, bx, by, blockIdx.z, s_a, s_b, s_red);
@@ -634,6 +675,11 @@
   if (sr == 1 && R % 4 == 0) return 2;
   return 0;
 }
+static int stage_mode_any(long long sr, long long sk) {
+  if (sk == 1) return 1;
+  if (sr == 1) return 2;
+  return 0;
+}
 
 template <int VPL>
 __global__ __launch_bounds__(256) void add_dropout_ln_fwd_k(int R, const float* __restrict__ x,
@@ -954,7 +1000,7 @@
 }
 
 template <int VPL>
-__global__ __launch_bounds__(256) void vote_combine_bwd_k(int R, const float* __restrict__ y,
+__global__ __launch_bounds__(256) void vote_combine_bwd_k(int R, int ldv, const float* __restrict__ y,
                                                           const float* __restrict__ norm,
                                                           const float* __restrict__ dy,
                                                           const float* __restrict__ dxyz,
@@ -972,7 +1018,7 @@
   }
   dot = group_allsum<64>(dot);
   const float inv = 1.0f / norm[row];
-  float* dv = dvotes + (size_t)row * (C + 3);
+  float* dv = dvotes + (size_t)row * ldv;
 #pragma unroll
   for (int i = 0; i < VPL; ++i) {
     const float d = (g[i] - yv[i] * dot) * inv;
@@ -980,15 +1026,10 @@
     drows[(size_t)row * C + lane + 64 * i] = d;
   }
   if (lane < 3) dv[lane] = dxyz != nullptr ? dxyz[(size_t)row * 3 + lane] : 0.f;
+  for (int c = C + 3 + lane; c < ldv; c += 64) dv[c] = 0.f;
 }
 
 __global__ void rng_advance_k(unsigned long long* rng) { rng[1] += 1; }
-__global__ void rng_next_k(unsigned long long* rng, unsigned long long* snap) {
-  const unsigned long long s = rng[1] + 1;
-  rng[1] = s;
-  snap[0] = rng[0];
-  snap[1] = s;
-}
 
 __global__ void dropout_mask_k(long long n, float p, const unsigned long long* __restrict__ rng,
                                unsigned op, float* __restrict__ out) {
@@ -1005,6 +1046,8 @@
                "gemm: bad sizes %d %d %d %d %d %d", p.M, p.N, p.K, p.batch, p.splitk, p.zdiv);
   DEMF_REQUIRE(p.A && p.B && p.C, "gemm: null operand");
   DEMF_REQUIRE(!(p.flags & GEMM_DROPOUT) || p.rng, "gemm: dropout needs the rng state");
+  DEMF_REQUIRE(!(p.flags & DEMF_GEMM_RNG_NEXT) || (p.rng && p.rng_snap && !(p.flags & GEMM_DROPOUT)),
+               "gemm: rng_next needs the live state and a snapshot, on a launch that draws no mask");
   DEMF_REQUIRE(!(p.flags & GEMM_GATE) || p.gate, "gemm: gate flag without a gate tensor");
   DEMF_REQUIRE(!(p.flags & GEMM_ROWBIAS) || (p.rowscale && p.bias), "gemm: rowbias needs bias and rowscale");
   DEMF_REQUIRE(p.splitk == 1 || !(p.flags & (GEMM_RELU | GEMM_DROPOUT | GEMM_GATE)),
@@ -1022,8 +1065,8 @@
   DEMF_REQUIRE(d != nullptr, "gemm: null descriptor");
   GemmArgs p = *d;
   if (int e = gemm_validate(p)) return e;
-  const int modeA = stage_mode(p.sam, p.sak, p.M, p.K);
-  const int modeB = stage_mode(p.sbn, p.sbk, p.N, p.K);
+  const int modeA = stage_mode_any(p.sam, p.sak);
+  const int modeB = stage_mode_any(p.sbn, p.sbk);
   dim3 grid(cdiv(p.N, G_BN), cdiv(p.M, G_BM), p.batch * p.splitk);
   const bool add = p.A2 != nullptr || p.B2 != nullptr;
   const bool bf = compute_bf16() && !(p.flags & GEMM_FP32);
@@ -1105,7 +1148,7 @@
     while (i0 + cnt < n && cnt < GEMM_GROUP_MAX) {
       const GemmArgs& p = descs[i0 + cnt];
       if (int e = gemm_validate(p)) return e;
-      const bool ok = gemm_is_small(p) && stage_mode(p.sam, p.sak, p.M, p.K) == 2 &&
+      const bool ok = gemm_is_small(p) && !(p.flags & DEMF_GEMM_RNG_NEXT) && stage_mode(p.sam, p.sak, p.M, p.K) == 2 &&
                       stage_mode(p.sbn, p.sbk, p.N, p.K) == 2 && !(p.flags & GEMM_FP32) && p.A2 == nullptr &&
                       (!tn3 || ((p.flags & ~GEMM_ACCUM) == 0 && p.bias == nullptr && p.C2 == nullptr &&
                                 (p.B2 == nullptr || p.b2_rows % 64 == 0 || p.b2_rows >= p.M)));
@@ -1282,9 +1325,10 @@
 
 extern "C" int demf_vote_combine_bwd(int R, int C, const float* vote_feats, const float* norm,
                                      const float* d_vote_feats, const float* d_vote_xyz,
-                                     float* d_votes, float* d_rows, demf_stream_t stream) {
+                                     float* d_votes, int ld_votes, float* d_rows, demf_stream_t stream) {
   DEMF_REQUIRE(R > 0 && vote_feats && norm && d_votes && d_rows, "vote_combine_bwd: bad arguments");
-#define CALL(V) hipLaunchKernelGGL(vote_combine_bwd_k<V>, dim3(cdiv(R, 4)), dim3(256), 0, (hipStream_t)stream, R, vote_feats, norm, d_vote_feats, d_vote_xyz, d_votes, d_rows)
+  DEMF_REQUIRE(ld_votes >= C + 3, "vote_combine_bwd: d_votes rows of %d floats hold no %d columns", ld_votes, C + 3);
+#define CALL(V) hipLaunchKernelGGL(vote_combine_bwd_k<V>, dim3(cdiv(R, 4)), dim3(256), 0, (hipStream_t)stream, R, ld_votes, vote_feats, norm, d_vote_feats, d_vote_xyz, d_votes, d_rows)
   LN_DISPATCH(C, CALL)
 #undef CALL
   return check_launch("vote_combine_bwd_k");
diff --git a/demf_amd/csrc/loss.hip b/demf_amd/csrc/loss.hip
--- a/demf_amd/csrc/loss.hip
+++ b/demf_amd/csrc/loss.hip
@@ -453,7 +453,8 @@
 }
 
 struct LossTotalArgs { const float* v[4]; };
-__global__ void loss_total_k(int n, LossTotalArgs a, const float* __restrict__ vote, float* __restrict__ out8) {
+__global__ void loss_total_k(int n, LossTotalArgs a, const float* __restrict__ vote, float* __restrict__ out8,
+                             float* __restrict__ tot1) {
   if (threadIdx.x != 0 || blockIdx.x != 0) return;
   float tot = 0.f;
   for (int i = 0; i < 7; ++i) {
@@ -463,15 +464,22 @@
     out8[i] = m;
     tot = i == 0 ? m : tot + m;
   }
-  out8[7] = tot + (vote ? vote[0] : 0.f);
-}
-__global__ void loss_total_bwd_k(int n, const float* __restrict__ g8, float* __restrict__ gv, float* __restrict__ gvote) {
+  tot = tot + (vote ? vote[0] : 0.f);
+  out8[7] = tot;
+  if (tot1) tot1[0] = tot;
+}
+__global__ void loss_total_bwd_k(int n, const float* __restrict__ g8, const float* __restrict__ gtot, int unit,
+                                 float* __restrict__ gv, float* __restrict__ gvote) {
   const int t = threadIdx.x;
+  if (t > 7) return;
+  const bool has_tot = unit || gtot != nullptr;
+  const float gs = unit ? 1.0f : (gtot != nullptr ? gtot[0] : 0.f);
+  const float gt = g8 == nullptr ? gs : (has_tot ? g8[7] + gs : g8[7]);
   if (t < 7) {
-    const float g = (g8[t] + g8[7]) / (float)n;
+    const float g = (g8 == nullptr ? gt : g8[t] + gt) / (float)n;
     for (int j = 0; j < n; ++j) gv[7 * j + t] = g;
   }
-  if (t == 7 && gvote) gvote[0] = g8[7];
+  if (t == 7 && gvote) gvote[0] = gt;
 }
 
 }
@@ -670,19 +678,24 @@
   return check_launch("target_weights");
 }
 
-extern "C" int demf_loss_total(int n, const float* const* vecs, const float* vote, float* out8, demf_stream_t stream) {
+extern "C" int demf_loss_total(int n, const float* const* vecs, const float* vote, float* out8, float* total,
+                               demf_stream_t stream) {
   DEMF_REQUIRE(n >= 1 && n <= 4 && vecs && out8, "loss_total: 1..4 seven-vectors");
   LossTotalArgs a{};
   for (int i = 0; i < n; ++i) {
     DEMF_REQUIRE(vecs[i], "loss_total: null vector %d", i);
     a.v[i] = vecs[i];
   }
-  hipLaunchKernelGGL(loss_total_k, dim3(1), dim3(64), 0, (hipStream_t)stream, n, a, vote, out8);
+  hipLaunchKernelGGL(loss_total_k, dim3(1), dim3(64), 0, (hipStream_t)stream, n, a, vote, out8, total);
   return check_launch("loss_total");
 }
 
-extern "C" int demf_loss_total_bwd(int n, const float* g8, float* gvecs, float* gvote, demf_stream_t stream) {
-  DEMF_REQUIRE(n >= 1 && n <= 4 && g8 && gvecs, "loss_total_bwd: 1..4 seven-vectors");
-  hipLaunchKernelGGL(loss_total_bwd_k, dim3(1), dim3(64), 0, (hipStream_t)stream, n, g8, gvecs, gvote);
+extern "C" int demf_loss_total_bwd(int n, const float* g8, const float* gtotal, int unit_total, float* gvecs,
+                                   float* gvote, demf_stream_t stream) {
+  DEMF_REQUIRE(n >= 1 && n <= 4 && gvecs, "loss_total_bwd: 1..4 seven-vectors");
+  DEMF_REQUIRE(g8 || gtotal || unit_total, "loss_total_bwd: no incoming gradient");
+  DEMF_REQUIRE(!(gtotal && unit_total), "loss_total_bwd: the total's gradient is either a tensor or the unit seed");
+  hipLaunchKernelGGL(loss_total_bwd_k, dim3(1), dim3(64), 0, (hipStream_t)stream, n, g8, gtotal, unit_total, gvecs,
+                     gvote);
   return check_launch("loss_total_bwd");
 }
diff --git a/demf_amd/engine.py b/demf_amd/engine.py
--- a/demf_amd/engine.py
+++ b/demf_amd/engine.py
@@ -76,6 +76,10 @@
         self.captured_pack = False
         self.sumsq_state = None
         self._reserved_table = None
+        self._unit = None
+        if self.flat.is_cuda:
+            from . import ops
+            self._unit = ops.unit_seed(dev)
         off = 0
         for p in self.params:
             k = p.numel()
@@ -86,8 +90,10 @@
     def backward_into(self, loss):
         if self.flat.is_cuda:
             from . import ops
+            seed = self._unit if (self._unit is not None and loss.dim() == 0 and loss.dtype == self._unit.dtype
+                                  and loss.device == self._unit.device) else None
             with ops.deferred_weight_grads():
-                grads = torch.autograd.grad(loss, self.params, allow_unused=True)
+                grads = torch.autograd.grad(loss, self.params, grad_outputs=seed, allow_unused=True)
         else:
             grads = torch.autograd.grad(loss, self.params, allow_unused=True)
         dst = [v for v, g in zip(self.views, grads) if g is not None]
diff --git a/demf_amd/fused.py b/demf_amd/fused.py
--- a/demf_amd/fused.py
+++ b/demf_amd/fused.py
@@ -8,6 +8,7 @@
 from . import _ffi
 
 RELU, DROPOUT, GATE, ACCUM, ROWBIAS, ACCUM2 = 1, 2, 4, 8, 16, 32
+RNG_NEXT = 128
 
 OP_ATTN, OP_LN1, OP_LN2, OP_FFN, OP_LN3 = 1, 2, 3, 4, 5
 
@@ -75,7 +76,7 @@
 def gemm(M, N, K, A, sa, B, sb, C, scm, *, batch=1, zdiv=1, sab=(0, 0), sbb=(0, 0), scb=(0, 0),
          A2=None, a2_cols=0, B2=None, b2_rows=0, C2=None, bias=None, sbias_b=0, rowscale=None,
          srs=(0, 0), alpha=1.0, flags=0, gate=None, sg=(0, 0), gate_scale=1.0, drop_p=0.0, rng=None,
-         op_id=0, splitk=1, asum=None, group=None):
+         op_id=0, splitk=1, asum=None, group=None, rng_next=None):
     d = _ffi.GemmDesc()
     d.M, d.N, d.K, d.batch, d.zdiv, d.splitk = M, N, K, batch, zdiv, splitk
     d.A, d.sam, d.sak, d.sab, d.sab2 = A, sa[0], sa[1], sab[0], sab[1]
@@ -90,6 +91,9 @@
     d.gate, d.sgm, d.sgb, d.gate_scale = gate, sg[0], sg[1], gate_scale
     d.drop_p, d.rng, d.op_id = drop_p, rng, op_id
     d.asum = asum
+    if rng_next is not None:
+        assert not flags & DROPOUT and group is None
+        d.flags, d.rng, d.rng_snap = flags | RNG_NEXT, rng_next[0], rng_next[1]
     if group is not None:
         group.append(d)
         return
@@ -143,14 +147,16 @@
         Dh, F, Ct, S = E // H, f0_w.shape[0], tokens.shape[2], tokens.shape[1]
         HLP = H * L * P
         assert R == B * Q and x.is_contiguous() and pos.is_contiguous() and pts.is_contiguous()
-        snap = next_rng(dev) if (p_attn > 0.0 or p_ffn > 0.0) else rng_state(dev)
+        draws = p_attn > 0.0 or p_ffn > 0.0
+        live = rng_state(dev)
+        snap = torch.empty_like(live) if draws else live
         rng = snap.data_ptr()
         OP_ATTN, OP_LN1, OP_LN2, OP_FFN, OP_LN3 = (salt + o for o in (1, 2, 3, 4, 5))
         new = lambda *s: torch.empty(s, dtype=torch.float32, device=dev)
         st = _st()
         qkv = new(R, 3 * E)
         gemm(R, 3 * E, E, _p(x), (E, 1), _p(in_w), (E, 1), _p(qkv), 3 * E, A2=_p(pos), a2_cols=2 * E,
-             bias=_p(in_b))
+             bias=_p(in_b), rng_next=(live.data_ptr(), rng) if draws else None)
         att = new(R, E)
         core = ATTN_CORE and Q == 256 and Dh == 32
         if core:
diff --git a/demf_amd/modules/head.py b/demf_amd/modules/head.py
--- a/demf_amd/modules/head.py
+++ b/demf_amd/modules/head.py
@@ -383,8 +383,8 @@
                                                  with_vote=(i == 0))
                                for i, d in enumerate(decode_res_all)])
             if vecs[0].is_cuda and len(vecs) <= 4:
-                out8 = ops.loss_total(list(vecs), vote[0])
-                mean7, total = out8[:7], out8[7]
+                out8, total = ops.loss_total_pair(list(vecs), vote[0])
+                mean7 = out8[:7]
             else:
                 mean7 = vecs[0]
                 for v in vecs[1:]:
diff --git a/demf_amd/ops.py b/demf_amd/ops.py
--- a/demf_amd/ops.py
+++ b/demf_amd/ops.py
@@ -692,50 +692,36 @@
     def backward(ctx, g):
         from . import fused
         x, weight = ctx.saved_tensors[:2]
-        g = g.contiguous()
         R, K = x.shape
         N = weight.shape[0]
+        if not (N % 4 != 0 and g.dim() == 2 and g.stride(1) == 1 and g.stride(0) >= N):
+            g = g.contiguous()
+        ldg = g.stride(0)
         if len(ctx.saved_tensors) == 3:
             g.masked_fill_(ctx.saved_tensors[2].unsqueeze(-1), 0.0)
         gx = gw = gb = None
-        Np, gq, wq = N, g, weight
-        if N % 4 != 0 and R >= 4096 and len(ctx.saved_tensors) == 2:
-            Np = (N + 3) // 4 * 4
-            gq = zeros((R, Np), g.device)
-            gq[:, :N].copy_(g)
-            wq = zeros((Np, K), g.device)
-            wq[:N].copy_(weight)
         if ctx.needs_input_grad[0]:
             gx = torch.empty((R, K), dtype=torch.float32, device=g.device)
-            if Np != N:
-                fused.gemm(R, K, Np, _p(gq), (Np, 1), _p(wq), (1, K), _p(gx), K)
-            elif _LinearRows._rows_ok(R, N, K, g):
+            if N % 4 == 0 and _LinearRows._rows_ok(R, N, K, g):
                 planes = 1 if get_compute_dtype() == "bf16" else 3
                 rows_gemm(g, split_planes(weight.detach().t().contiguous(), planes), None, gx)
             else:
-                fused.gemm(R, K, N, _p(g), (N, 1), _p(weight), (weight.stride(1), weight.stride(0)), _p(gx), K)
+                fused.gemm(R, K, N, _p(g), (ldg, 1), _p(weight), (weight.stride(1), weight.stride(0)), _p(gx), K)
         want_b = ctx.has_bias and ctx.needs_input_grad[2]
         if ctx.needs_input_grad[1] or want_b:
-            ws = zeros(Np * K + Np, g.device)
-            gw = ws[:Np * K].view(Np, K)
-            gb = ws[Np * K:] if ctx.has_bias else None
+            ws = zeros(N * K + N, g.device)
+            gw = ws[:N * K].view(N, K)
+            gb = ws[N * K:] if ctx.has_bias else None
             in_gemm = False
-            if Np != N:
-                in_gemm = gb is not None
-                fused.gemm(Np, K, R, _p(gq), (1, Np), _p(x), (1, x.stride(0)), _p(gw), K,
-                           splitk=fused._splitk(R), asum=_p(gb) if in_gemm else None)
-                if gb is not None and not in_gemm:
-                    _ffi.call("demf_colsum_f32", R, Np, Np, _p(gq), _p(gb), _stream())
-                return gx, gw[:N], (gb[:N] if gb is not None else None), None
             if R >= 32768 and N % 4 == 0 and K % 4 == 0 and x.is_contiguous():
                 _ffi.call("demf_mlp_gemm_bwd_dw", R, N, K, K, _p(g), None, None, 1, _p(g),
                           _p(_identity_dy_vectors(N, g.device)), _p(x), None, _p(gw), _stream())
             else:
-                in_gemm = gb is not None and N % 4 == 0 and N >= 4
-                fused.gemm(N, K, R, _p(g), (1, N), _p(x), (1, x.stride(0)), _p(gw), K,
+                in_gemm = gb is not None and (N % 4 == 0 or ldg != N) and N >= 4
+                fused.gemm(N, K, R, _p(g), (1, ldg), _p(x), (1, x.stride(0)), _p(gw), K,
                            splitk=fused._splitk(R), asum=_p(gb) if in_gemm else None)
             if gb is not None and not in_gemm:
-                _ffi.call("demf_colsum_f32", R, N, N, _p(g), _p(gb), _stream())
+                _ffi.call("demf_colsum_f32", R, N, ldg, _p(g), _p(gb), _stream())
         return gx, gw, gb, None
 
 
@@ -1420,11 +1406,12 @@
         R, C = y.shape
         dxyz = None if dxyz is None else dxyz.contiguous()
         dy = None if dy is None else dy.contiguous()
-        dvotes = torch.empty((R, C + 3), dtype=torch.float32, device=y.device)
+        ld = (C + 3 + 3) // 4 * 4
+        dvotes = torch.empty((R, ld), dtype=torch.float32, device=y.device)
         drows = torch.empty_like(y)
-        _ffi.call("demf_vote_combine_bwd", R, C, _p(y), _p(norm), _p(dy), _p(dxyz), _p(dvotes),
+        _ffi.call("demf_vote_combine_bwd", R, C, _p(y), _p(norm), _p(dy), _p(dxyz), _p(dvotes), ld,
                   _p(drows), _stream())
-        return drows, dvotes, (dxyz if ctx.needs_input_grad[2] else None)
+        return drows, dvotes[:, :C + 3], (dxyz if ctx.needs_input_grad[2] else None)
 
 
 def vote_combine(rows, votes, seed_xyz):
@@ -1573,31 +1560,56 @@
     return out
 
 
+_UNIT_SEED = {}
+
+
+def unit_seed(device):
+    device = torch.device(device)
+    if device.index is None and device.type == "cuda":
+        device = torch.device(device.type, torch.cuda.current_device())
+    key = str(device)
+    if key not in _UNIT_SEED:
+        _UNIT_SEED[key] = torch.ones((), dtype=torch.float32, device=device)
+    return _UNIT_SEED[key]
+
+
 class _LossTotal(Function):
     @staticmethod
     def forward(ctx, vote, *vecs):
         n = len(vecs)
         vecs = [v.contiguous() for v in vecs]
         out = torch.empty(8, dtype=torch.float32, device=vecs[0].device)
+        tot = torch.empty((), dtype=torch.float32, device=vecs[0].device)
         tab = (ctypes.c_void_p * n)(*[v.data_ptr() for v in vecs])
-        _ffi.call("demf_loss_total", n, ctypes.addressof(tab), _p(vote), _p(out), _stream())
+        _ffi.call("demf_loss_total", n, ctypes.addressof(tab), _p(vote), _p(out), _p(tot), _stream())
         ctx.n, ctx.has_vote = n, vote is not None
-        return out
-
-    @staticmethod
-    def backward(ctx, g8):
-        g8 = g8.contiguous()
-        gv = torch.empty((ctx.n, 7), dtype=torch.float32, device=g8.device)
-        gvote = torch.empty(1, dtype=torch.float32, device=g8.device) if ctx.has_vote else None
-        _ffi.call("demf_loss_total_bwd", ctx.n, _p(g8), _p(gv), _p(gvote), _stream())
+        ctx.set_materialize_grads(False)
+        return out, tot
+
+    @staticmethod
+    def backward(ctx, g8, gtot):
+        some = g8 if g8 is not None else gtot
+        if some is None:
+            return (None,) * (1 + ctx.n)
+        dev = some.device
+        g8 = None if g8 is None else g8.contiguous()
+        unit = gtot is not None and gtot.data_ptr() == unit_seed(dev).data_ptr()
+        gv = torch.empty((ctx.n, 7), dtype=torch.float32, device=dev)
+        gvote = torch.empty(1, dtype=torch.float32, device=dev) if ctx.has_vote else None
+        _ffi.call("demf_loss_total_bwd", ctx.n, _p(g8), None if unit else _p(gtot), int(unit), _p(gv), _p(gvote),
+                  _stream())
         return (gvote,) + tuple(gv[i] for i in range(ctx.n))
 
 
-def loss_total(vecs, vote=None):
+def loss_total_pair(vecs, vote=None):
     assert 1 <= len(vecs) <= 4
     for v in vecs:
         _chk(v, "loss vector")
     return _LossTotal.apply(None if vote is None else vote.reshape(1), *vecs)
+
+
+def loss_total(vecs, vote=None):
+    return loss_total_pair(vecs, vote)[0]
 
 
 def target_weights(objectness_masks, objectness_targets):
diff --git a/include/demf_hip.h b/include/demf_hip.h
--- a/include/demf_hip.h
+++ b/include/demf_hip.h
@@ -177,7 +177,7 @@
 DEMF_INTERNAL int demf_vote_combine_fwd(int R, int C, const float* rows, const float* votes, const float* seed_xyz,
                           float* vote_xyz, float* vote_feats, float* norm, demf_stream_t stream);
 DEMF_INTERNAL int demf_vote_combine_bwd(int R, int C, const float* vote_feats, const float* norm,
-                          const float* d_vote_feats, const float* d_vote_xyz, float* d_votes,
+                          const float* d_vote_feats, const float* d_vote_xyz, float* d_votes, int ld_votes,
                           float* d_rows, demf_stream_t stream);
 
 DEMF_INTERNAL int demf_bnrelu_maxpool_fwd(int R, int ns, int C, const float* Y, const float* scale_shift,
@@ -376,8 +376,10 @@
 DEMF_INTERNAL int demf_query_pos_rows(int R, int nreg, const float* reg_rows, const float* base_xyz, float* out8,
                         demf_stream_t stream);
 
-DEMF_INTERNAL int demf_loss_total(int n, const float* const* vecs, const float* vote, float* out8, demf_stream_t stream);
-DEMF_INTERNAL int demf_loss_total_bwd(int n, const float* g8, float* gvecs, float* gvote, demf_stream_t stream);
+DEMF_INTERNAL int demf_loss_total(int n, const float* const* vecs, const float* vote, float* out8, float* total,
+                    demf_stream_t stream);
+DEMF_INTERNAL int demf_loss_total_bwd(int n, const float* g8, const float* gtotal, int unit_total, float* gvecs,
+                        float* gvote, demf_stream_t stream);
 
 DEMF_INTERNAL int demf_pad_gt(int B, int G, const int* counts, const int* box_dims, const void* const* boxes,
                 const void* const* labels, float* gt_padded, int64_t* labels_padded,
@@ -471,6 +473,7 @@
 #define DEMF_GEMM_ROWBIAS 16
 #define DEMF_GEMM_ACCUM2 32
 #define DEMF_GEMM_FP32 64
+#define DEMF_GEMM_RNG_NEXT 128
 
 typedef struct demf_gemm_desc {
   int M, N, K, batch, zdiv, splitk;
@@ -490,6 +493,7 @@
   const void* rng;
   int op_id;
   float* asum;
+  void* rng_snap;
 } demf_gemm_desc;
 
 DEMF_INTERNAL int demf_gemm_f32(const demf_gemm_desc* desc, demf_stream_t stream);
```

Measured after the change: 1802 scenes/s. Within noise of the previous version (-0.6%).
